# Gjerman/Orange3-Spark

Hardware: AMD Instinct MI355X
Metric: samples/sec LogisticRegression.fit on 1Bx256 synthetic at 1/2/4/8 MI355X (higher is better)
Workload: dtype bf16; 1 GPU; global_batch=1000000000, seq_len=256, features=256, parallelism=dp1, resident_rows=497795896, lineage_rows=502204104, device=cuda:0

## Files before the change

### orange3_spark_amd/models/glm.py

```python
from __future__ import annotations

import logging
import math
import os
import time
from dataclasses import dataclass, field

import numpy as np
import torch

from ..frame import column as C
from ..ops import _native as N
from ..ops import glm as G
from ..runtime.tracing import traced
from ..synthetic import LineageVectorColumn
from . import optim
from ..runtime import progress

log = logging.getLogger(__name__)

LOSS_ID = {"logistic": G.LOSS_LOGISTIC, "hinge": G.LOSS_HINGE, "squared": G.LOSS_SQUARED}


class GlmData:

    def __init__(self, comm, feat: C.Column, y: torch.Tensor, sw: torch.Tensor | None = None,
                 chunk_rows: int = 1 << 22):
        from ..frame.spill import SpilledVectorColumn
        self.comm = comm
        self.lineage = None
        self.spill = None
        if isinstance(feat, C.SparseVectorColumn):
            feat = C.VectorColumn(feat.to_dense(torch.float32), feat.size)
        if isinstance(feat, LineageVectorColumn):
            X = feat.data
            self.lineage = (feat.spec, feat.row0 + feat.resident_rows, feat.lineage_rows)
        elif isinstance(feat, SpilledVectorColumn):
            X = feat.data
            if feat.spilled_rows:
                self.spill = feat.streamer()
        else:
            X = feat.data
        self.d = int(feat.size)
        self.X = X
        self.device = X.device if X.numel() or X.is_cuda else y.device
        self.kernel = X.is_cuda and X.is_contiguous() and (
            X.dtype == torch.bfloat16 or (G.f32_rows(X) and not isinstance(feat, SpilledVectorColumn)))
        self.ld = int(X.shape[1])
        self.y = y.to(self.device, torch.float32).contiguous() if self.kernel else y.to(self.device)
        self.sw = None if sw is None else (sw.to(self.device, torch.float32).contiguous() if self.kernel else sw.to(self.device))
        self.nres = int(X.shape[0])
        self.n_local = self.nres + (self.lineage[2] if self.lineage else 0) + \
            (int(self.spill.host.shape[0]) if self.spill is not None else 0)
        self.n = int(comm.sum_scalar(self.n_local))
        self.chunk = chunk_rows
        self.ws = G.GlmWorkspace(self.device, self.ld) if self.kernel else None
        self.passes = 0
        self.overlap = None
        self.mixed = self.kernel and os.environ.get("O3S_GLM_MIXED", "1") == "1" \
            and (self.sw is None or self.sw.shape[0] == self.y.shape[0])
        self._row0 = int(feat.row0) if isinstance(feat, LineageVectorColumn) else None
        if self.spill is not None and self.kernel:
            self.mixed = True
        self._setup_workspace()
        self.ws_stream = G.GlmWorkspace(self.device, self.ld) if (self.spill is not None and self.kernel) else None

    def _res(self, t):
        return None if t is None else (t if self.spill is None else t[: self.nres])

    def _chunk_rows(self, t, off, rows):
        return None if t is None else t[self.nres + off: self.nres + off + rows]

    @property
    def mode(self) -> str:
        if self.lineage:
            return "resident+lineage" if self.nres else "lineage"
        if self.spill is not None:
            return "resident+streamed" if self.nres else "streamed"
        return "resident"

    def _setup_workspace(self):
        if self.mixed:
            cus = N.num_cus(self.device)
            tiles = -(-int(self.X.shape[0]) // 16) + -(-int(self.lineage[2] if self.lineage else 0) // 16)
            if self.spill is not None:
                tiles = max(tiles, -(-int(self.spill.chunk_rows) // 16))
            grid = max(1, min(cus * 32, -(-tiles // 4)))
            self.ws = G.GlmWorkspace(self.device, self.ld,
                                     grid=int(os.environ.get("O3S_GLM_GRID_MIX", str(grid))))
        elif self.kernel and self.lineage and self.X.shape[0] and os.environ.get("O3S_GLM_OVERLAP", "1") == "1":
            cus = N.num_cus(self.device)
            res_grid = int(os.environ.get("O3S_GLM_GRID_RES", str(cus * 8)))
            lin_grid = int(os.environ.get("O3S_GLM_GRID_LIN", str(cus)))
            self.ws = G.GlmWorkspace(self.device, self.ld, grid=res_grid)
            self.overlap = (torch.cuda.Stream(self.device), G.GlmWorkspace(self.device, self.ld, grid=lin_grid))

    def global_row0(self) -> int:
        if self._row0 is None:
            counts = self.comm.all_gather_object(int(self.n_local))
            self._row0 = int(sum(counts[: self.comm.rank]))
        return self._row0

    def require_mixed(self) -> None:
        if self.kernel and not self.mixed:
            self.mixed, self.overlap = True, None
            self._setup_workspace()

    def stats(self):
        spec, r0, nl = self.lineage if self.lineage else (None, 0, 0)
        if self.kernel:
            if not self.mixed:
                return None
            st = G.glm_stats_mixed(self.X, self._res(self.y), self._res(self.sw), nl, spec.d if spec else self.d,
                                   spec.seed if spec else 0, r0)
            if st is None:
                return None
            dpad = self.ws.dpad
        else:
            st = G.glm_stats_torch(self.X, self._res(self.y), self._res(self.sw), nl, spec.d if spec else self.d,
                                   spec.seed if spec else 0, r0).to(self.device)
            dpad = G.layout(self.ld)[0]
        if self.spill is not None:
            acc = st

            def chunk(Xc, off):
                yc, wc = self._chunk_rows(self.y, off, Xc.shape[0]), self._chunk_rows(self.sw, off, Xc.shape[0])
                if self.kernel:
                    acc.add_(G.glm_stats_mixed(Xc, yc, wc, 0, self.d, 0, 0))
                else:
                    acc.add_(G.glm_stats_torch(Xc, yc, wc, 0, self.d, 0, 0).to(self.device))
            self.spill.run(chunk)
        self.comm.all_reduce(st)
        h = st.cpu().numpy()
        d = self.d
        self.passes += 1
        return (h[:d], h[dpad:dpad + d], h[2 * dpad:2 * dpad + d], float(h[3 * dpad]), float(h[3 * dpad + 1]),
                float(h[3 * dpad + 2]))

    def moments(self):
        d = self.d
        def torch_stats(Xc, swc):
            Xd = Xc.to(torch.float64)
            w = torch.ones(Xd.shape[0], dtype=torch.float64, device=Xd.device) if swc is None \
                else swc.to(torch.float64)
            return torch.cat([w @ Xd, w @ (Xd * Xd), w.sum().reshape(1)])
        if self.kernel:
            parts = [G.glm_colstats(self.X, self._res(self.sw))] if self.X.shape[0] else []
            if self.lineage:
                spec, r0, nl = self.lineage
                parts.append(G.glm_colstats_synth(nl, self.ld, spec.d, spec.seed, r0, self.device))
            if parts:
                st = torch.stack(parts).sum(0)
            else:
                st = torch.zeros(2 * self.ld + 1, dtype=torch.float64, device=self.device)
        else:
            st = torch_stats(self.X, self._res(self.sw))
        if self.spill is not None:
            def chunk(Xc, off):
                wc = self._chunk_rows(self.sw, off, Xc.shape[0])
                st.add_(G.glm_colstats(Xc, wc) if self.kernel else torch_stats(Xc, wc).to(st.device))
            self.spill.run(chunk)
        ld = self.ld
        yw = self.y.to(torch.float64) * (1.0 if self.sw is None else self.sw.to(torch.float64))
        ystats = torch.stack([yw.sum(), (yw * self.y.to(torch.float64)).sum()]).to(st.device)
        full = torch.cat([st, ystats]).contiguous()
        self.comm.all_reduce(full)
        full = full.cpu().numpy()
        s1, s2, W = full[:ld], full[ld:2 * ld], full[2 * ld]
        ys1, ys2 = full[2 * ld + 1], full[2 * ld + 2]
        if self.lineage:
            pass
        mean = s1 / max(W, 1e-300)
        var = (s2 - W * mean * mean) / max(W - 1.0, 1e-300)
        var = np.maximum(var, 0.0)
        ymean = ys1 / max(W, 1e-300)
        yvar = max((ys2 - W * ymean * ymean) / max(W - 1.0, 1e-300), 0.0)
        return mean[:self.d], var[:self.d], W, ymean, yvar

    def pass_device(self, coef_eff: torch.Tensor, intercept: float | None, loss: int,
                    t_dev: torch.Tensor | None = None, sample: tuple | None = None) -> torch.Tensor:
        ws = self.ws
        if sample is not None and sample[1] < 1.0:
            self.require_mixed()
            ws = self.ws
        if self.mixed:
            spec, r0, nl = self.lineage if self.lineage else (None, 0, 0)
            sseed, frac = sample if sample is not None else (0, 1.0)
            g0 = self.global_row0() if frac < 1.0 else 0
            if self.nres or nl:
                G.glm_grad_mixed(self.X, self._res(self.y), self._res(self.sw), nl, spec.d if spec else self.d,
                                 spec.seed if spec else 0, r0, coef_eff, intercept, loss, ws,
                                 res_row0=g0, t_dev=t_dev, sample_seed=sseed, fraction=frac)
            else:
                ws.out.zero_()
            if self.spill is not None:
                cf = G._coef_buf(coef_eff, ws.dpad, self.device, intercept=intercept)
                wss = self.ws_stream

                def chunk(Xc, off):
                    rows = Xc.shape[0]
                    G.glm_grad_mixed(Xc, self._chunk_rows(self.y, off, rows), self._chunk_rows(self.sw, off, rows),
                                     0, self.d, 0, 0, cf, None, loss, wss, res_row0=g0 + self.nres + off,
                                     t_dev=t_dev, sample_seed=sseed, fraction=frac)
                    ws.out.add_(wss.out)
                self.spill.run(chunk)
            self.passes += 1
            return ws.out
        if self.overlap is not None:
            return self._pass_overlapped(coef_eff, intercept, loss)
        filled = False
        if self.X.shape[0]:
            G.glm_grad(self.X, self.y, self.sw, coef_eff, intercept, loss, ws)
            filled = True
        if self.lineage:
            spec, r0, nl = self.lineage
            G.glm_grad_synth(nl, self.ld, spec.d, spec.seed, r0, spec.wtrue, spec.btrue, coef_eff,
                             intercept, loss, ws, accumulate=filled)
            filled = True
        if not filled:
            ws.out.zero_()
        self.passes += 1
        return ws.out

    def _pass_overlapped(self, coef_eff, intercept, loss):
        side, ws_l = self.overlap
        ws = self.ws
        main = torch.cuda.current_stream(self.device)
        cf = G._coef_buf(coef_eff, ws.dpad, self.device, intercept=intercept)
        side.wait_stream(main)
        spec, r0, nl = self.lineage
        with torch.cuda.stream(side):
            G.glm_grad_synth(nl, self.ld, spec.d, spec.seed, r0, spec.wtrue, spec.btrue, cf, None, loss, ws_l)
        G.glm_grad(self.X, self.y, self.sw, cf, None, loss, ws)
        main.wait_stream(side)
        ws.out += ws_l.out
        self.passes += 1
        return ws.out

    def pass_torch(self, coef_eff: torch.Tensor, intercept: float, loss: int, it: int = 1,
                   sample: tuple | None = None) -> torch.Tensor:
        dpad = self.ld
        acc = torch.zeros(dpad + 3, dtype=torch.float64, device=self.device)
        c = coef_eff.to(self.device, torch.float64)[: self.ld]
        sampled = sample is not None and sample[1] < 1.0
        g0 = self.global_row0() if sampled else 0

        def block(X, base):
            n = X.shape[0]
            for a in range(0, n, self.chunk):
                b = min(n, a + self.chunk)
                Xc = X[a:b].to(self.device, torch.float64)
                yc = self.y[base + a:base + b].to(torch.float64)
                wc = None if self.sw is None else self.sw[base + a:base + b].to(torch.float64)
                if sampled:
                    keep = G.sample_mask(sample[0], it, torch.arange(g0 + base + a, g0 + base + b),
                                         sample[1]).to(self.device)
                    wc = keep.to(torch.float64) if wc is None else wc * keep
                acc.add_(G.glm_grad_torch(Xc, yc, wc, c, intercept, loss))
        block(self.X, 0)
        if self.spill is not None:
            self.spill.run(lambda Xc, off: block(Xc, self.nres + off))
        self.passes += 1
        return acc

    @traced("glm.pass")
    def loss_grad(self, coef_eff: np.ndarray, intercept: float, loss: int):
        ct = torch.from_numpy(np.ascontiguousarray(coef_eff, dtype=np.float64))
        if self.kernel:
            cf = torch.zeros(self.ws.dpad, dtype=torch.float32)
            cf[: self.d] = ct.float()
            out = self.pass_device(cf.to(self.device), intercept, loss)
            dpad = self.ws.dpad
        else:
            cf = torch.zeros(self.ld, dtype=torch.float64)
            cf[: self.d] = ct
            out = self.pass_torch(cf, intercept, loss)
            dpad = self.ld
        self.comm.all_reduce(out)
        o = out.cpu().numpy()
        return float(o[dpad + 1]), o[: self.d].copy(), float(o[dpad]), float(o[dpad + 2])


class SparseGlmData:

    kernel = False
    lineage = None

    def __init__(self, comm, feat: C.SparseVectorColumn, y: torch.Tensor, sw: torch.Tensor | None = None):
        from ..ops.sparse import SparseRows
        self.comm = comm
        self.rows = SparseRows(feat.indptr, feat.indices, feat.values, feat.size)
        self.device = self.rows.device
        self.d = int(feat.size)
        self.y = y.to(self.device)
        self.sw = None if sw is None else sw.to(self.device)
        self.n_local = self.rows.n
        self.n = int(comm.sum_scalar(self.n_local))
        self.passes = 0

    def moments(self):
        w = None if self.sw is None else self.sw.to(torch.float32)
        s1 = self.rows.colsum(w)
        s2 = self.rows.colsum(w, square=True)
        wd = torch.ones(self.n_local, dtype=torch.float64, device=self.device) if self.sw is None \
            else self.sw.to(torch.float64)
        yd = self.y.to(torch.float64)
        full = torch.cat([s1, s2, torch.stack([wd.sum(), (wd * yd).sum(), (wd * yd * yd).sum()])]).contiguous()
        self.comm.all_reduce(full)
        full = full.cpu().numpy()
        d = self.d
        s1, s2, W, ys1, ys2 = full[:d], full[d:2 * d], full[2 * d], full[2 * d + 1], full[2 * d + 2]
        mean = s1 / max(W, 1e-300)
        var = np.maximum((s2 - W * mean * mean) / max(W - 1.0, 1e-300), 0.0)
        ymean = ys1 / max(W, 1e-300)
        yvar = max((ys2 - W * ymean * ymean) / max(W - 1.0, 1e-300), 0.0)
        return mean, var, W, ymean, yvar

    sample_state = None
    _row0 = None

    def global_row0(self) -> int:
        if self._row0 is None:
            counts = self.comm.all_gather_object(int(self.n_local))
            self._row0 = int(sum(counts[: self.comm.rank]))
        return self._row0

    @traced("glm.pass")
    def loss_grad(self, coef_eff: np.ndarray, intercept: float, loss: int):
        ct = torch.from_numpy(np.ascontiguousarray(coef_eff, dtype=np.float64))
        sw = self.sw
        st = self.sample_state
        if st is not None and st[1] < 1.0:
            g0 = self.global_row0()
            keep = G.sample_mask(st[0], st[2], torch.arange(g0, g0 + self.n_local), st[1]).to(self.device)
            sw = keep.to(torch.float64) if sw is None else sw.to(torch.float64) * keep
        out = self.rows.loss_grad(ct, intercept, loss, self.y, sw)
        self.comm.all_reduce(out)
        self.passes += 1
        o = out.cpu().numpy()
        d = self.d
        return float(o[d + 1]), o[:d].copy(), float(o[d]), float(o[d + 2])


def make_glm_data(comm, feat: C.Column, y: torch.Tensor, sw: torch.Tensor | None = None):
    if isinstance(feat, C.SparseVectorColumn):
        return SparseGlmData(comm, feat, y, sw)
    return GlmData(comm, feat, y, sw)


@dataclass
class GlmResult:
    coef: np.ndarray
    intercept: float
    history: list = field(default_factory=list)
    iterations: int = 0
    converged: bool = False
    seconds: float = 0.0
    passes: int = 0
    setup_seconds: float = 0.0


class GlmObjective:

    def __init__(self, data: GlmData, loss: str, reg: float, alpha: float, fit_intercept: bool,
                 standardization: bool, std: np.ndarray):
        self.data, self.loss = data, LOSS_ID[loss]
        self.reg, self.alpha = float(reg), float(alpha)
        self.fi, self.stdz = fit_intercept, standardization
        self.std = std
        self.inv_std = np.where(std > 0, 1.0 / np.where(std > 0, std, 1.0), 0.0)
        self.W = None
        d = data.d
        self.l2 = self.reg * (1.0 - self.alpha)
        if self.stdz:
            self.pen2 = np.full(d, self.l2)
            self.pen1 = np.full(d, self.reg * self.alpha)
        else:
            self.pen2 = self.l2 * self.inv_std ** 2
            self.pen1 = self.reg * self.alpha * self.inv_std

    def split(self, x):
        d = self.data.d
        return x[:d], (x[d] if self.fi else 0.0)

    def smooth(self, x):
        bt, b = self.split(x)
        ls, g, gb, W = self.data.loss_grad(bt * self.inv_std, b, self.loss)
        self.W = W
        f = ls / W + 0.5 * float(np.sum(self.pen2 * bt * bt))
        gx = g * self.inv_std / W + self.pen2 * bt
        if self.fi:
            return f, np.concatenate([gx, [gb / W]])
        return f, gx


def _initial_intercept(loss: str, fit_intercept: bool, ymean: float, init_intercept=None) -> float:
    if not fit_intercept:
        return 0.0
    if init_intercept is not None:
        return float(init_intercept)
    if loss == "logistic" and 0 < ymean < 1:
        return math.log(ymean / (1 - ymean))
    if loss == "squared":
        return float(ymean)
    return 0.0


def _first_step_out(loss: str, b0: float, s1, syx, W: float, wy: float, wyy: float):
    if loss == "logistic":
        p = 1.0 / (1.0 + math.exp(-b0))
        sp = max(b0, 0.0) + math.log1p(math.exp(-abs(b0)))
        return p * s1 - syx, p * W - wy, sp * W - b0 * wy
    if loss == "hinge":
        if abs(b0) >= 1.0:
            return None
        return s1 - 2.0 * syx, W - 2.0 * wy, W - b0 * (2.0 * wy - W)
    return b0 * s1 - syx, b0 * W - wy, 0.5 * (b0 * b0 * W - 2.0 * b0 * wy + wyy)


def fit_sgd(data: GlmData, loss: str, reg=0.0, alpha=0.0, fit_intercept=True, standardization=True,
            max_iter=100, tol=1e-6, step_size=1.0, mini_batch_fraction=1.0, seed=0, init_intercept=None,
            ckpt=None, check_every: int = 10) -> GlmResult:
    t0 = time.time()
    frac = float(mini_batch_fraction)
    G.sample_threshold(frac)
    last = ckpt.latest() if ckpt is not None else None
    st = data.stats() if (frac >= 1.0 and last is None and max_iter > 0) else None
    if st is not None:
        s1, s2, syx, W, wy, wyy = st
        mean = s1 / max(W, 1e-300)
        var = np.maximum((s2 - W * mean * mean) / max(W - 1.0, 1e-300), 0.0)
        ymean = wy / max(W, 1e-300)
    else:
        mean, var, W, ymean, _ = data.moments()
    std = np.sqrt(var)
    b0 = float(init_intercept) if (fit_intercept and init_intercept is not None) else 0.0
    sgd = DeviceSGD(data, loss, reg, fit_intercept, step_size, standardization, std, elastic_net=alpha,
                    mini_batch_fraction=frac, seed=seed, init_intercept=b0)
    setup_s = time.time() - t0
    done = 0
    if last is not None and last[1]["x"].shape[0] == data.d + (1 if fit_intercept else 0):
        done = int(last[0])
        sgd.set_state(last[1]["x"], done)
    elif st is not None:
        first = _first_step_out(loss, b0, s1, syx, W, wy, wyy)
        if first is not None:
            sgd.apply_first_step(*first, W)
    converged = False
    while sgd.t < max_iter:
        progress.iteration(sgd.t, max_iter)
        sgd.step()
        if (tol > 0 or ckpt is not None) and sgd.t % check_every == 0:
            h = sgd.loss_hist[max(0, sgd.t - 2):sgd.t].cpu().numpy()
            if ckpt is not None and ckpt.due(sgd.t):
                ckpt.save(sgd.t, {"x": sgd.state()})
            if tol > 0 and len(h) == 2 and abs(h[0] - h[1]) / max(abs(h[1]), 1e-12) < tol:
                converged = True
                break
    if ckpt is not None:
        ckpt.clear()
    res = sgd.result()
    res.converged = converged
    res.seconds = time.time() - t0
    res.setup_seconds = setup_s
    res.passes = data.passes
    return res


def fit_glm(data: GlmData, loss: str, reg=0.0, alpha=0.0, fit_intercept=True, standardization=True,
            max_iter=100, tol=1e-6, solver="auto", step_size=1.0, mini_batch_fraction=1.0, seed=0,
            init_intercept=None, ckpt=None) -> GlmResult:
    if solver in ("sgd", "gd") and isinstance(data, GlmData):
        return fit_sgd(data, loss, reg, alpha, fit_intercept, standardization, max_iter, tol, step_size,
                       mini_batch_fraction, seed, init_intercept, ckpt)
    t0 = time.time()
    mean, var, W, ymean, yvar = data.moments()
    std = np.sqrt(var)
    obj = GlmObjective(data, loss, reg, alpha, fit_intercept, standardization, std)
    d = data.d
    x0 = np.zeros(d + (1 if fit_intercept else 0))
    if fit_intercept:
        if init_intercept is not None:
            x0[-1] = init_intercept
        elif loss == "logistic" and 0 < ymean < 1:
            x0[-1] = math.log(ymean / (1 - ymean))
        elif loss == "squared":
            x0[-1] = ymean
    done = 0
    last = ckpt.latest() if ckpt is not None else None
    if last is not None and last[1]["x"].shape == x0.shape:
        done, x0 = last[0], last[1]["x"]

    def save(it, x, f):
        if ckpt is not None and ckpt.due(done + it):
            ckpt.save(done + it, {"x": np.asarray(x)})
    left = max(max_iter - done, 0)
    if solver in ("sgd", "gd"):
        res = _sgd(obj, x0, left, step_size, mini_batch_fraction, seed, tol)
    elif reg * alpha > 0:
        l1 = np.concatenate([obj.pen1, [0.0]]) if fit_intercept else obj.pen1
        r = optim.owlqn(obj.smooth, x0, l1, max_iter=left, tol=tol, callback=save)
        res = GlmResult(r.x, 0.0, r.history, done + r.iterations, r.converged)
    else:
        f32 = isinstance(data, GlmData) and data.kernel and data.X.dtype == torch.float32
        r = optim.lbfgs(obj.smooth, x0, max_iter=left, tol=tol, callback=save, f_noise=2.0 ** -24 if f32 else 0.0)
        res = GlmResult(r.x, 0.0, r.history, done + r.iterations, r.converged)
    if ckpt is not None:
        ckpt.clear()
    bt, b = obj.split(res.coef)
    res.coef = bt * obj.inv_std
    res.intercept = float(b)
    res.seconds = time.time() - t0
    res.passes = data.passes
    return res


def _sgd(obj: GlmObjective, x0, max_iter, step, frac, seed, tol) -> GlmResult:
    x = x0.copy()
    hist = []
    for t in range(1, max_iter + 1):
        progress.iteration(t - 1, max_iter)
        obj.data.sample_state = (int(seed), float(frac), t)
        f, g = obj.smooth(x)
        hist.append(f)
        x = x - (step / math.sqrt(t)) * g
        if len(hist) > 1 and abs(hist[-2] - hist[-1]) / max(abs(hist[-1]), 1e-12) < tol * 1e-3:
            break
    obj.data.sample_state = None
    return GlmResult(x, 0.0, hist, len(hist), False)


class DeviceSGD:

    def __init__(self, data: GlmData, loss: str = "logistic", reg: float = 0.0, fit_intercept=True,
                 step_size: float = 1.0, standardization: bool = True, std: np.ndarray | None = None,
                 elastic_net: float = 0.0, mini_batch_fraction: float = 1.0, seed: int = 0,
                 init_intercept: float = 0.0):
        self.data, self.loss = data, LOSS_ID[loss]
        dev = data.device
        dpad = data.ws.dpad if data.kernel else data.ld
        self.dpad = dpad
        inv = np.ones(data.d) if std is None else np.where(std > 0, 1.0 / np.where(std > 0, std, 1.0), 0.0)
        self.inv_std = torch.zeros(dpad, dtype=torch.float64, device=dev)
        self.inv_std[: data.d] = torch.from_numpy(inv).to(dev)
        a = float(elastic_net)
        l2, l1 = float(reg) * (1.0 - a), float(reg) * a
        self.l2 = l2 if standardization else 0.0
        self.l2v = (l2 * self.inv_std ** 2) if not standardization else None
        self.l1 = l1 if standardization else 0.0
        self.l1v = (l1 * self.inv_std) if (not standardization and l1 > 0) else None
        self.bt = torch.zeros(dpad, dtype=torch.float64, device=dev)
        self.b = torch.full((1,), float(init_intercept) if fit_intercept else 0.0, dtype=torch.float64, device=dev)
        self.coef_eff = torch.zeros(dpad + 1, dtype=torch.float32, device=dev)
        self.coef_eff[dpad] = float(self.b[0])
        self.fi = fit_intercept
        self.step_size = float(step_size)
        self.fraction = float(mini_batch_fraction)
        G.sample_threshold(self.fraction)
        self.sample = (int(seed), self.fraction) if self.fraction < 1.0 else None
        self.t = 0
        self.loss_hist = torch.zeros(1024, dtype=torch.float64, device=dev)
        self.t_dev = torch.zeros(1, dtype=torch.int64, device=dev)
        self._graphs = None
        self._graph_failed = False
        self._eager_steps = 0
        self._first_buf = None
        self.passes = 0

    def state(self) -> np.ndarray:
        x = self.bt[: self.data.d].cpu().numpy()
        return np.concatenate([x, self.b.cpu().numpy()]) if self.fi else x

    def set_state(self, x: np.ndarray, t: int) -> None:
        d = self.data.d
        self.bt.zero_()
        self.bt[:d] = torch.from_numpy(np.asarray(x[:d], dtype=np.float64)).to(self.bt.device)
        if self.fi:
            self.b.fill_(float(x[d]))
        self.coef_eff[: self.dpad].copy_((self.bt * self.inv_std).to(torch.float32))
        self.coef_eff[self.dpad:].copy_(self.b.to(torch.float32))
        self.t = int(t)
        self.t_dev.fill_(int(t))
        self._ensure_hist()
        self._graphs = None

    def _ensure_hist(self):
        if self.t > self.loss_hist.shape[0]:
            n = self.loss_hist.shape[0]
            while n < self.t:
                n *= 2
            self.loss_hist = torch.cat([self.loss_hist, torch.zeros(n - self.loss_hist.shape[0],
                                                                     dtype=torch.float64, device=self.loss_hist.device)])
            self._graphs = None

    def apply_first_step(self, grad: np.ndarray, sum_r: float, loss_sum: float, W: float) -> None:
        out = torch.zeros(self.dpad + 3, dtype=torch.float64)
        out[: self.data.d] = torch.from_numpy(np.asarray(grad, dtype=np.float64))
        out[self.dpad:] = torch.tensor([sum_r, loss_sum, W], dtype=torch.float64)
        self._first_buf = out.to(self.bt.device)
        self.t += 1
        self._ensure_hist()
        self._update(self._first_buf)

    @traced("sgd.step")
    def step(self):
        self.t += 1
        self._ensure_hist()
        d = self.data
        self.passes += 1
        if d.kernel and self._graphs is not None:
            gp, gu = self._graphs
            gp.replay()
            if gu is not None:
                d.comm.all_reduce(self.data.ws.out)
                gu.replay()
            d.passes += 1
            return
        out = self._pass()
        d.comm.all_reduce(out)
        self._update(out)
        if d.kernel:
            self._eager_steps += 1
            self._maybe_capture()

    def _pass(self):
        if self.data.kernel:
            return self.data.pass_device(self.coef_eff, None, self.loss, t_dev=self.t_dev, sample=self.sample)
        return self.data.pass_torch(self.coef_eff[: self.dpad], float(self.b.item()), self.loss, it=self.t,
                                    sample=self.sample)

    def _update(self, out: torch.Tensor):
        if self.data.kernel:
            N.check(N.kernels().o3s_glm_sgd_update_dev(
                out.data_ptr(), self.dpad, self.bt.data_ptr(), self.b.data_ptr(), self.inv_std.data_ptr(),
                N.ptr(self.l2v), self.l2, N.ptr(self.l1v), self.l1, self.step_size, int(self.fi),
                self.coef_eff.data_ptr(), self.loss_hist.data_ptr(), int(self.loss_hist.shape[0]),
                self.t_dev.data_ptr(), torch.cuda.current_stream(self.data.device).cuda_stream), "glm_sgd_update")
            return
        eta = self.step_size / math.sqrt(self.t)
        W = out[self.dpad + 2]
        invW = torch.where(W > 0, 1.0 / W, torch.zeros_like(W))
        g = out[: self.dpad] * self.inv_std * invW
        g = g + (self.l2v if self.l2v is not None else self.l2) * self.bt
        v = self.bt - eta * g
        if self.l1v is not None or self.l1 > 0:
            sh = eta * (self.l1v if self.l1v is not None else self.l1)
            v = torch.sign(v) * torch.clamp(v.abs() - sh, min=0.0)
        self.bt.copy_(v)
        if self.fi:
            self.b -= eta * out[self.dpad] * invW
        self.coef_eff[: self.dpad].copy_((self.bt * self.inv_std).to(torch.float32))
        self.coef_eff[self.dpad:].copy_(self.b.to(torch.float32))
        self.loss_hist[self.t - 1:self.t].copy_(out[self.dpad + 1:self.dpad + 2] * invW)
        self.t_dev.fill_(self.t)

    GRAPH_MAX_BYTES = int(os.environ.get("O3S_SGD_GRAPH_MAX_BYTES", str(256 << 20)))

    def _maybe_capture(self):
        from ..runtime import faults
        mode = os.environ.get("O3S_SGD_GRAPH", "1")
        if self._graphs is not None or self._graph_failed or mode == "0" or self._eager_steps < 2:
            return
        if faults.launch_blocking():
            return
        d = self.data
        if d.spill is not None:
            return
        if mode != "force" and d.n_local * d.ld * d.X.element_size() > self.GRAPH_MAX_BYTES:
            return
        if d.comm.world_size > 1 and mode != "all":
            return
        try:
            if d.comm.world_size == 1:
                g = torch.cuda.CUDAGraph()
                with torch.cuda.graph(g):
                    out = self._pass()
                    self._update(out)
                self._graphs = (g, None)
            else:
                gp, gu = torch.cuda.CUDAGraph(), torch.cuda.CUDAGraph()
                with torch.cuda.graph(gp):
                    out = self._pass()
                with torch.cuda.graph(gu):
                    self._update(out)
                self._graphs = (gp, gu)
            d.passes -= 1
        except Exception as e:
            log.warning("SGD step graph capture failed (%s); continuing eagerly", e)
            self._graph_failed = True
            self._graphs = None

    def result(self) -> GlmResult:
        coef = (self.bt * self.inv_std)[: self.data.d].cpu().numpy()
        hist = [float(x) for x in self.loss_hist[: self.t].cpu()]
        return GlmResult(coef, float(self.b.item()), hist, self.t, False, 0.0, self.data.passes)


def _class_weights(yl: torch.Tensor, w: torch.Tensor | None, K: int) -> torch.Tensor:
    if w is None:
        return torch.bincount(yl, minlength=K)[:K].to(torch.float64)
    w64 = w.to(torch.float64)
    if K <= 64:
        return torch.stack([torch.where(yl == k, w64, 0.0).sum() for k in range(K)])
    return torch.zeros(K, dtype=torch.float64, device=yl.device).index_add_(0, yl, w64)


def fit_multinomial(comm, X: torch.Tensor, y: torch.Tensor, sw, num_classes: int, reg=0.0, alpha=0.0,
                    fit_intercept=True, standardization=True, max_iter=100, tol=1e-6, chunk=1 << 21):
    dev = X.device
    n, D = X.shape
    K = num_classes
    Xf_dtype = torch.float32 if X.is_cuda else torch.float64
    yl = y.to(dev).long()
    w = torch.ones(n, dtype=Xf_dtype, device=dev) if sw is None else sw.to(dev, Xf_dtype)
    fused = G.softmax_kernel_ok(X, K) and os.environ.get("O3S_SOFTMAX_KERNEL", "1") == "1"
    f32_kernel = fused and X.dtype == torch.float32
    if X.is_cuda and X.dtype in (torch.bfloat16, torch.float32) and X.stride(1) == 1 and X.stride(0) % 8 == 0:
        base = torch.as_strided(X, (n, X.stride(0)), (X.stride(0), 1))
        cs = G.glm_colstats(base, None if sw is None else w.float().contiguous())
        ldp = X.stride(0)
        s1, s2 = cs[:D], cs[ldp:ldp + D]
    else:
        s1 = torch.zeros(D, dtype=torch.float64, device=dev)
        s2 = torch.zeros(D, dtype=torch.float64, device=dev)
        for a in range(0, n, chunk):
            Xc = X[a:a + chunk].to(torch.float64)
            wc = w[a:a + chunk].to(torch.float64)
            s1 += wc @ Xc
            s2 += wc @ (Xc * Xc)
    cnt = _class_weights(yl, None if sw is None else w, K)
    st = torch.cat([s1, s2, cnt])
    comm.all_reduce(st)
    st = st.cpu().numpy()
    W = st[2 * D:].sum()
    mean = st[:D] / W
    var = np.maximum((st[D:2 * D] - W * mean ** 2) / max(W - 1, 1e-300), 0)
    std = np.sqrt(var)
    inv = np.where(std > 0, 1.0 / np.where(std > 0, std, 1.0), 0.0)
    inv_t = torch.from_numpy(inv).to(dev, Xf_dtype)
    l2 = reg * (1 - alpha)
    pen2 = np.full(D, l2) if standardization else l2 * inv ** 2
    pen1 = np.full(D, reg * alpha) if standardization else reg * alpha * inv
    prior = st[2 * D:] / W

    y32 = yl.to(torch.int32).contiguous() if fused else None
    sw32 = None if (sw is None or not fused) else w.float().contiguous()

    def fg(x):
        Bt = x[: D * K].reshape(K, D)
        b = x[D * K:] if fit_intercept else np.zeros(K)
        if fused:
            Gk, gbk, lk = G.softmax_pass(X, y32, sw32, torch.from_numpy(Bt * inv[None, :]).to(dev, torch.float32),
                                         torch.from_numpy(b).to(dev, torch.float32))
            buf = torch.cat([Gk.T.reshape(-1), gbk, lk.reshape(1)])
            return _mn_finish(buf, Bt)
        Weff = torch.from_numpy(Bt.T * inv[:, None]).to(dev, Xf_dtype)
        bt = torch.from_numpy(b).to(dev, Xf_dtype)
        G_ = torch.zeros((D, K), dtype=torch.float64, device=dev)
        gb = torch.zeros(K, dtype=torch.float64, device=dev)
        loss = torch.zeros(1, dtype=torch.float64, device=dev)
        for a in range(0, n, chunk):
            Xc = X[a:a + chunk].to(Xf_dtype)
            M = Xc @ Weff + bt
            lse = torch.logsumexp(M, dim=1)
            yc = yl[a:a + chunk]
            wc = w[a:a + chunk]
            loss += (wc * (lse - M.gather(1, yc[:, None]).squeeze(1))).to(torch.float64).sum()
            P = torch.softmax(M, dim=1)
            P[torch.arange(P.shape[0], device=dev), yc] -= 1.0
            R = P * wc[:, None]
            G_ += (Xc.T @ R).to(torch.float64)
            gb += R.sum(0).to(torch.float64)
        return _mn_finish(torch.cat([G_.reshape(-1), gb, loss]), Bt)

    def _mn_finish(buf, Bt):
        comm.all_reduce(buf)
        buf = buf.cpu().numpy()
        Gm = buf[: D * K].reshape(D, K).T * inv[None, :] / W
        gbm = buf[D * K:D * K + K] / W
        if f32_kernel:
            Gm = Gm - Gm.mean(0, keepdims=True)
            gbm = gbm - gbm.mean()
        f = buf[-1] / W + 0.5 * float(np.sum(pen2[None, :] * Bt * Bt))
        Gm = Gm + pen2[None, :] * Bt
        g = Gm.reshape(-1)
        if fit_intercept:
            g = np.concatenate([g, gbm])
        return f, g

    f_noise = 2.0 ** -24 if f32_kernel else 0.0
    x0 = np.zeros(D * K + (K if fit_intercept else 0))
    if fit_intercept:
        lp = np.log(np.maximum(prior, 1e-300))
        x0[D * K:] = lp - lp.mean()
    if reg * alpha > 0:
        l1 = np.concatenate([np.tile(pen1, K), np.zeros(K if fit_intercept else 0)])
        r = optim.owlqn(fg, x0, l1, max_iter=max_iter, tol=tol, f_noise=f_noise)
    else:
        r = optim.lbfgs(fg, x0, max_iter=max_iter, tol=tol, f_noise=f_noise)
    Bt = r.x[: D * K].reshape(K, D)
    B = Bt * inv[None, :]
    b = r.x[D * K:] if fit_intercept else np.zeros(K)
    if fit_intercept:
        b = b - b.mean()
    if reg == 0:
        B = B - B.mean(0, keepdims=True)
    return B, b, r
```

### orange3_spark_amd/ops/_native.py

```python
from __future__ import annotations

import ctypes as C
import os
import threading
from pathlib import Path

import torch

from ..runtime.faults import O3SError
from . import build as _build

_LOCK = threading.Lock()
_LIB = None
_HOST = None

c_i64, c_i32, c_u32, c_f32, c_f64 = C.c_int64, C.c_int, C.c_uint32, C.c_float, C.c_double
c_vp = C.c_void_p

_SIGS: dict[str, list] = {
    "o3s_glm_layout": [c_i64, C.POINTER(c_i32), C.POINTER(c_i32)],
    "o3s_glm_grad": [c_i32, c_i32, c_vp, c_i64, c_i64, c_vp, c_vp, c_vp, c_u32, c_i64,
                     c_vp, c_f32, c_vp, c_i32, c_vp, c_i32, c_vp],
    "o3s_glm_grad_mixed": [c_i32, c_vp, c_i64, c_i64, c_vp, c_vp, c_vp, c_u32, c_i64, c_i64,
                           c_vp, c_i32, c_vp, c_i32, c_i64, c_vp, c_u32, c_u32, c_i32, c_i32, c_i32, c_vp],
    "o3s_glm_stats_mixed": [c_vp, c_i64, c_i64, c_vp, c_vp, c_u32, c_i64, c_i64, c_vp, c_i32, c_vp, c_i32, c_i32,
                            c_vp],
    "o3s_glm_grad_f32": [c_i32, c_vp, c_i64, c_i64, c_vp, c_vp, c_vp, c_i64, c_vp, c_i32, c_vp, c_i32, c_i64, c_vp,
                         c_u32, c_u32, c_i32, c_vp],
    "o3s_glm_stats_f32": [c_vp, c_i64, c_i64, c_vp, c_vp, c_i64, c_vp, c_i32, c_vp, c_vp],
    "o3s_glm_margin_f32": [c_vp, c_i64, c_i64, c_vp, c_f32, c_vp, c_i32, c_vp],
    "o3s_glm_colstats_f32": [c_vp, c_i64, c_i64, c_vp, c_vp, c_i32, c_vp, c_vp],
    "o3s_bin_features": [c_vp, c_i64, c_i64, c_i32, c_vp, c_i32, c_vp, c_vp],
    "o3s_u8_transpose": [c_vp, c_i64, c_i32, c_vp, c_vp],
    "o3s_slab_range_sum": [c_vp, c_i32, c_i64, c_vp, c_vp, c_i32, c_vp, c_vp],
    "o3s_tree_leaf_apply": [c_vp, c_vp, c_vp, c_vp, c_i32, c_vp, c_vp],
    "o3s_ftf": [c_vp, c_i64, c_i64, c_i32, c_i64, c_vp, c_vp, c_vp],
    "o3s_als_gram": [c_vp, c_vp, c_vp, c_vp, c_vp, c_i32, c_vp, c_vp, c_i64, c_i64, c_vp, c_vp, c_vp],
    "o3s_csr_glm": [c_i32, c_vp, c_vp, c_vp, c_i64, c_vp, c_f32, c_vp, c_vp, c_vp, c_vp, c_i32, c_vp],
    "o3s_csc_colsum": [c_vp, c_vp, c_i64, c_vp, c_i64, c_vp, c_vp, c_vp, c_i32, c_vp, c_vp, c_vp],
    "o3s_csc_piece": [],
    "o3s_tokenize": [c_i32, c_vp, c_vp, c_i64, c_vp, c_vp, c_vp, c_vp, c_vp, c_vp],
    "o3s_murmur3_spans": [c_vp, c_vp, c_vp, c_i64, c_u32, c_i64, c_vp, c_vp],
    "o3s_tree_partition": [c_vp, c_i64, c_i64, c_vp, c_vp, c_vp, c_vp, c_vp, c_vp, c_vp, c_vp, c_vp, c_vp, c_i32, c_i32,
                           c_vp, c_vp, c_vp, c_vp, c_vp],
    "o3s_glm_sgd_update": [c_vp, c_i32, c_vp, c_vp, c_vp, c_vp, c_f64, c_f64, c_i32, c_vp, c_vp, c_vp],
    "o3s_glm_sgd_update_dev": [c_vp, c_i32, c_vp, c_vp, c_vp, c_vp, c_f64, c_vp, c_f64, c_f64, c_i32, c_vp, c_vp,
                               c_i64, c_vp, c_vp],
    "o3s_synth_glm": [c_vp, c_i64, c_i64, c_vp, c_u32, c_i64, c_vp, c_f32, c_i32, c_vp],
    "o3s_glm_margin": [c_vp, c_i64, c_i64, c_vp, c_f32, c_vp, c_i32, c_vp],
    "o3s_glm_colstats": [c_i32, c_vp, c_i64, c_i64, c_vp, c_u32, c_i64, c_vp, c_i32, c_vp, c_vp],
    "o3s_bin_sums": [c_vp, c_i32, c_i64, c_i64, c_i32, c_vp, c_i64, c_vp, c_i32, c_vp, c_i32, c_vp, c_vp],
    "o3s_glm_softmax": [c_vp, c_i64, c_i64, c_i32, c_vp, c_vp, c_vp, c_vp, c_i32, c_vp, c_i32, c_vp, c_vp],
    "o3s_glm_softmax_f32": [c_vp, c_i64, c_i64, c_i32, c_vp, c_vp, c_vp, c_vp, c_i32, c_vp, c_i32, c_vp, c_vp],
    "o3s_kmeans_assign": [c_vp, c_i64, c_i64, c_i32, c_vp, c_vp, c_vp, c_i32, c_vp, c_vp, c_vp, c_vp],
    "o3s_kmeans_screen2": [c_vp, c_i64, c_i64, c_i32, c_vp, c_vp, c_vp, c_i32, c_i32, C.c_float, C.c_float,
                           C.c_float, C.c_float, C.c_float, c_vp, c_vp, c_vp, c_vp, c_i32, c_i32, c_vp, c_vp, c_vp,
                           c_vp, c_vp],
    "o3s_kmeans_presplit": [c_vp, c_i64, c_i64, c_i32, C.c_float, c_vp, c_vp, c_vp],
    "o3s_kmeans_moments": [c_vp, c_i64, c_i64, c_i32, c_vp, c_i32, c_vp, c_vp],
    "o3s_kmeans_cost": [c_vp, c_i64, c_i64, c_i32, c_vp, c_vp, c_i32, c_i32, c_vp, c_vp],
    "o3s_kmeans_bounds": [c_vp, c_vp, c_i64, c_vp, C.c_float, c_i32, c_vp, c_vp, c_vp, c_i32, c_vp],
    "o3s_kmeans_update_ws": [c_i32, c_i32, c_i32, C.POINTER(c_i64), C.POINTER(c_i64), C.POINTER(c_i32)],
    "o3s_kmeans_screen_lds": [c_i32, c_i32, C.POINTER(c_i32)],
    "o3s_murmur3_terms": [c_vp, c_vp, c_i64, c_u32, c_i64, c_vp, c_vp, c_vp],
    "o3s_als_init": [c_i64, c_i64, c_i32, c_u32, c_i32, c_vp, c_vp],
    "o3s_als_cg": [c_i32, c_i64, c_i32, c_vp, c_vp, c_vp, c_vp, c_vp, c_vp, c_vp, c_vp, c_vp],
    "o3s_als_pass": [c_i32, c_vp, c_vp, c_vp, c_i64, c_vp, c_i32, c_vp, c_vp, c_vp, c_vp, c_vp],
    "o3s_tree_hist_lds": [c_i32, c_i32, c_i32, c_i32],
    "o3s_hash_uniform": [c_vp, c_i64, c_i64, c_u32, c_u32, c_i32, c_f64, c_vp, c_vp, c_vp],
    "o3s_tree_final_level": [c_vp, c_i64, c_i64, c_vp, c_vp, c_vp, c_vp, c_vp, c_vp, c_vp, c_vp, c_vp, c_vp, c_vp,
                             c_i32, c_vp],
    "o3s_forest_weights": [c_vp, c_i64, c_vp, c_i32, c_vp, c_i32, c_f32, c_vp, c_vp, c_vp],
    "o3s_tree_sibling": [c_vp, c_vp, c_vp, c_i64, c_i32, c_i32, c_i32, c_vp, c_vp],
    "o3s_tree_part_dest": [c_vp, c_vp, c_vp, c_vp, c_vp, c_i32, c_vp, c_vp, c_vp, c_vp],
    "o3s_gbt_grad_loss": [c_vp, c_vp, c_vp, c_vp, c_i64, c_i32, c_vp, c_vp, c_i32, c_vp],
    "o3s_gbt_leaf_pass": [c_vp, c_i64, c_i32, c_vp, c_i32, c_vp, c_i32, c_vp, c_vp, c_vp, c_vp, c_vp, c_i32, c_i32,
                          c_vp, c_vp, c_vp, c_i32, c_vp],
    "o3s_tree_split": [c_vp, c_i32, c_i32, c_i32, c_i32, c_i32, c_vp, c_vp, c_f64, c_f64, c_f64, c_vp, c_vp, c_vp],
    "o3s_tree_hist": [c_vp, c_i64, c_i32, c_i32, c_i32, c_i32, c_vp, c_vp, c_vp, c_vp, c_vp, c_i32, c_vp, c_i32,
                      c_vp],
    "o3s_eval_grid": [c_i64],
    "o3s_regression_stats": [c_vp, c_i32, c_vp, c_i32, c_vp, c_i32, c_i64, c_vp, c_vp, c_vp],
    "o3s_confusion": [c_vp, c_i32, c_vp, c_i32, c_vp, c_i32, c_i64, c_i32, c_vp, c_vp, c_vp],
    "o3s_score_hist": [c_vp, c_i32, c_i64, c_vp, c_i32, c_vp, c_i32, c_i64, c_f64, c_f64, c_i32, c_vp, c_vp],
    "o3s_als_wood_kn": [c_i32, c_i32, c_vp, c_vp, c_vp, c_vp, c_vp, c_vp, c_vp, c_vp, c_i64, c_vp, c_vp],
    "o3s_als_wood_timed": [c_i32, c_vp, c_vp, c_vp, c_vp, c_vp, c_vp, c_vp, c_vp, c_i64, c_vp, c_vp, c_vp],
    "o3s_hashing_tf": [c_i32, c_vp, c_vp, c_vp, c_vp, c_vp, c_i64, c_u32, c_i64, c_vp, c_vp, c_vp, c_vp, c_i32,
                       c_vp, c_vp, c_vp],
    "o3s_als_dense_wave_dbg": [c_i32, c_i32, c_vp, c_vp, c_vp, c_vp, c_vp, c_vp, c_i64, c_vp, c_i32, c_vp, c_vp],
    "o3s_bin_features2": [c_vp, c_i32, c_i64, c_i64, c_i32, c_vp, c_i32, c_vp, c_vp, c_i64, c_vp],
    "o3s_kmeanspp": [c_vp, c_vp, c_vp, c_i32, c_i32, c_i32, c_i32, c_vp, c_vp, c_vp, c_vp, c_vp, c_vp, c_vp, c_vp],
    "o3s_als_dense_wave_timed": [c_vp, c_vp, c_vp, c_vp, c_vp, c_vp, c_i64, c_vp, c_i32, c_vp, c_vp],
    "o3s_als_dense_wave": [c_i32, c_i32, c_vp, c_vp, c_vp, c_vp, c_vp, c_vp, c_i64, c_vp, c_i32, c_vp],
    "o3s_als_dense_wave_gd": [c_i32, c_vp, c_vp, c_vp, c_vp, c_vp, c_vp, c_i64, c_vp, c_i32, c_vp],
    "o3s_als_exact_max_small": [],
    "o3s_als_rotate": [c_i32, c_vp, c_vp, c_i64, c_vp, c_i32, c_vp],
    "o3s_als_rotate_to": [c_i32, c_vp, c_vp, c_i64, c_vp, c_vp, c_i32, c_vp],
    "o3s_assemble": [c_vp, c_i32, c_vp, c_i32, c_i32, c_i64, c_vp, c_i32, c_vp, c_vp, c_i32, c_vp],
    "o3s_assemble_src_size": [],
    "o3s_assemble_cols": [c_vp, c_i32, c_i32, c_i32, c_i64, c_vp, c_i32, c_vp, c_vp, c_i32, c_vp],
    "o3s_kmeans_update": [c_vp, c_i64, c_i64, c_i32, c_vp, c_i32, c_vp, c_vp, c_i32, c_vp, c_vp, c_vp],
    "o3s_gather_probe": [c_vp, c_i32, c_vp, c_i64, c_i32, c_vp, c_vp],
    "o3s_gram_layout": [c_i32, C.POINTER(c_i32), C.POINTER(c_i32), C.POINTER(c_i32)],
    "o3s_gram": [c_vp, c_i32, c_i64, c_i64, c_i32, c_vp, c_vp, c_vp, c_vp, c_i32, c_vp, c_vp],
    "o3s_gmm_layout": [c_i32, c_i32, C.POINTER(c_i32), C.POINTER(c_i32), C.POINTER(c_i64), C.POINTER(c_i32)],
    "o3s_gmm_estep": [c_vp, c_i32, c_i64, c_i64, c_i32, c_i32, c_vp, c_vp, c_vp, c_vp, c_vp, c_vp, c_vp, c_i32, c_vp],
}


class NativeError(O3SError):
    """A native kernel launch was rejected (bad shape/arguments) or failed."""


def lib_path() -> Path:
    alt = os.environ.get("O3S_KERNEL_LIB")
    return Path(alt) if alt else _build.KERNEL_LIB


def _load():
    global _LIB
    path = lib_path()
    if not path.exists() and os.environ.get("O3S_AUTOBUILD", "1") == "1":
        _build.build()
    if not path.exists():
        raise NativeError(f"kernel library missing: {path} (run python -m orange3_spark_amd.ops.build)")
    lib = C.CDLL(str(path), mode=C.RTLD_GLOBAL)
    for name, argt in _SIGS.items():
        fn = getattr(lib, name, None)
        if fn is None:
            continue
        fn.argtypes = argt
        fn.restype = C.c_int
    _LIB = lib
    return lib


def kernels():
    if _LIB is not None:
        return _LIB
    with _LOCK:
        if _LIB is not None:
            return _LIB
        return _load()


_HOST_SIGS: dict[str, list] = {
    "o3s_host_murmur3": [c_vp, c_vp, c_i64, c_u32, c_i64, c_vp, c_vp],
    "o3s_host_tokenize": [c_vp, c_vp, c_i64, c_vp, c_vp, c_vp, c_i64, c_vp],
    "o3s_host_pav": [c_vp, c_vp, c_vp, c_vp, c_i64, c_vp, c_vp, c_vp, c_vp],
    "o3s_host_ascii_lengths": [c_vp, c_i64, c_vp, c_vp],
    "o3s_host_ascii_pack": [c_vp, c_i64, c_vp, c_vp, c_i32],
}
_HOST_RET = {"o3s_host_tokenize": C.c_int64, "o3s_host_pav": C.c_int64, "o3s_host_ascii_lengths": C.c_int64}


def host():
    global _HOST
    if _HOST is not None:
        return _HOST
    with _LOCK:
        if _HOST is None:
            path = _build.HOST_LIB
            if not path.exists():
                _build.build()
            lib = C.CDLL(str(path))
            for name, argt in _HOST_SIGS.items():
                fn = getattr(lib, name)
                fn.argtypes = argt
                fn.restype = _HOST_RET.get(name)
            _HOST = lib
    return _HOST


PRELOAD_TAGS = ("glm", "trees", "kmeans", "als", "als_dense", "als_exact", "assemble", "binsum", "eval",
                "sampling", "sparse", "text", "probe", "gram", "gmm")


def preload(tags=PRELOAD_TAGS) -> dict:
    import time
    lib = kernels()
    out = {}
    for tag in tags:
        fn = getattr(lib, f"o3s_preload_{tag}", None)
        if fn is None:
            continue
        fn.restype = C.c_int
        t = time.perf_counter()
        rc = fn()
        if rc != 0:
            raise NativeError(f"o3s_preload_{tag}: hipError {rc}")
        out[tag] = round(time.perf_counter() - t, 5)
    return out


def available() -> bool:
    try:
        kernels()
        return True
    except Exception:
        return False


def ptr(t: torch.Tensor | None) -> int | None:
    if t is None:
        return None
    return t.data_ptr()


def upload(arr, dev) -> torch.Tensor:
    import numpy as np
    t = torch.from_numpy(np.ascontiguousarray(arr))
    dev = torch.device(dev)
    if dev.type != "cuda":
        return t.to(dev)
    p = torch.empty(t.shape, dtype=t.dtype, pin_memory=True)
    p.copy_(t)
    return p.to(dev, non_blocking=True)


def upload_many(dev, *arrays) -> list:
    import numpy as np
    arrs = [np.ascontiguousarray(a) for a in arrays]
    offs, total = [], 0
    for a in arrs:
        offs.append(total)
        total += (a.nbytes + 7) // 8 * 8
    buf = np.zeros(max(total, 8), dtype=np.uint8)
    for a, o in zip(arrs, offs):
        buf[o:o + a.nbytes] = a.view(np.uint8).reshape(-1)
    d = upload(buf, dev)
    out = []
    for a, o in zip(arrs, offs):
        dt = torch.from_numpy(np.zeros(0, dtype=a.dtype)).dtype
        out.append(d[o:o + a.nbytes].view(dt).view(a.shape))
    return out


def stream_of(t: torch.Tensor) -> int:
    return torch.cuda.current_stream(t.device).cuda_stream


def check(rc: int, what: str) -> None:
    from ..runtime import faults
    faults.INJECTOR.hit("kernel")
    if rc != 0:
        raise NativeError(f"{what} failed with code {rc}")
    if faults.launch_blocking() and torch.cuda.is_available():
        try:
            torch.cuda.synchronize()
        except Exception as e:
            raise faults.DeviceError(what, e) from e


def num_cus(device: torch.device) -> int:
    try:
        return torch.cuda.get_device_properties(device).multi_processor_count
    except Exception:
        return 256


def grid_for(device: torch.device, work_items: int, per_block: int, blocks_per_cu: int = 8) -> int:
    need = max(1, (work_items + per_block - 1) // per_block)
    return int(max(1, min(need, num_cus(device) * blocks_per_cu)))
```

### orange3_spark_amd/ops/csrc/glm.hip

```cpp
#include <type_traits>

#include "common.h"

using namespace o3s;

namespace {

enum { LOSS_LOGISTIC = 0, LOSS_HINGE = 1, LOSS_SQUARED = 2 };

constexpr int kBlock = 256;
constexpr int kWavesPerBlock = kBlock / kWave;

__host__ __device__ __forceinline__ uint32_t umad24(uint32_t a, uint32_t c, uint32_t add) {
#if defined(__HIP_DEVICE_COMPILE__)
  return __umul24(a, c) + add;
#else
  return (a & 0xFFFFFFu) * c + add;
#endif
}
__host__ __device__ __forceinline__ uint32_t mix24(uint32_t h) {
  h ^= h >> 16;
  h = umad24(h, 0xED5AD4u, h);
  h ^= h >> 15;
  return umad24(h, 0x2C1B3Cu, h);
}
__device__ __forceinline__ uint32_t feat_key(uint32_t seed, int64_t row) {
  const uint32_t lo = (uint32_t)(row & 0xffffffffll);
  const uint32_t hi = (uint32_t)((uint64_t)row >> 32);
  return mix24(mix24(lo + seed * 0x9E3779B1u) ^ umad24(hi, 0x7FEB35u, 0x165667u));
}
__device__ __forceinline__ uint32_t synth_word(uint32_t fk, int i) {
  return mix24(umad24((uint32_t)i, 0x9E3779u, fk));
}
__device__ __forceinline__ float synth_byte(uint32_t h, int q) {
  return (float)((h >> (8 * q)) & 0xffu);
}
constexpr float kSynthScale = 1.0f / 128.0f, kSynthShift = -255.0f / 256.0f;
__device__ __forceinline__ short8 synth_chunk(uint32_t fk, int ch) {
  short8 v;
#pragma unroll
  for (int p = 0; p < 2; ++p) {
    const uint32_t h = synth_word(fk, 2 * ch + p);
#pragma unroll
    for (int q = 0; q < 4; ++q)
      v[4 * p + q] = (short)f32_to_bf16(fmaf(synth_byte(h, q), kSynthScale, kSynthShift));
  }
  return v;
}
__device__ __forceinline__ float synth_label(uint32_t rk, float margin_true) {
  const float u = (float)(fmix32(rk ^ 0xA511E9B3u) >> 8) * (1.0f / 16777216.0f);
  return u < sigmoidf(margin_true) ? 1.0f : 0.0f;
}

constexpr int ilog2(int x) { return x <= 1 ? 0 : 1 + ilog2(x / 2); }

template <int LPR, int U>
struct RowReduce {
  static constexpr int LL = ilog2(LPR), LU = ilog2(U);
  static constexpr int H = LL < LU ? LL : LU;
  static constexpr int NF = U >> H;
  __device__ static __forceinline__ int base(int c) {
    int b = 0;
#pragma unroll
    for (int s = 0; s < H; ++s) b += ((c >> (LL - 1 - s)) & 1) * (U >> (s + 1));
    return b;
  }
  __host__ __device__ static constexpr int owner(int u) {
    int c = 0;
    for (int s = 0; s < H; ++s) c += (((u - u % NF) >> (LU - 1 - s)) & 1) << (LL - 1 - s);
    return c;
  }
  __device__ static __forceinline__ bool representative(int c) {
    return (c & ((1 << (LL - H)) - 1)) == 0;
  }
  __device__ static __forceinline__ void run(float (&v)[U], int c) {
    int n = U;
#pragma unroll
    for (int s = 0; s < LL; ++s) {
      const int off = LPR >> (s + 1);
      if (s < H) {
        const bool up = (c & off) != 0;
        n >>= 1;
#pragma unroll
        for (int j = 0; j < U / 2; ++j) {
          if (j < n) {
            const float keep = up ? v[j + n] : v[j];
            const float send = up ? v[j] : v[j + n];
            v[j] = keep + __shfl_xor(send, off, kWave);
          }
        }
      } else {
#pragma unroll
        for (int j = 0; j < NF; ++j) v[j] += __shfl_xor(v[j], off, kWave);
      }
    }
  }
};

struct MemoryRows {
  static constexpr bool kLineage = false;
  __device__ static __forceinline__ float dot(float d, float) { return d; }
  __device__ static __forceinline__ float resid(float r, float&) { return r; }
};
struct RowsBf16 : MemoryRows {
  using elem = uint16_t;
  using chunk = short8;
  __device__ static __forceinline__ void load(const elem* __restrict__ X, int64_t ld, int64_t rowc, int chc,
                                              chunk& v) {
    v = __builtin_nontemporal_load(reinterpret_cast<const short8*>(X + rowc * ld + 8 * chc));
  }
  __device__ static __forceinline__ void mask(chunk& v, bool keep) {
    v = keep ? v : short8{0, 0, 0, 0, 0, 0, 0, 0};
  }
  __device__ static __forceinline__ void load_if(const elem* __restrict__ X, int64_t ld, int64_t row, int ch,
                                                 bool ok, chunk& v) {
    v = ok ? *reinterpret_cast<const short8*>(X + row * ld + 8 * ch) : short8{0, 0, 0, 0, 0, 0, 0, 0};
  }
  __device__ static __forceinline__ void unpack(const chunk& v, float (&x)[8]) { unpack8(v, x); }
  __device__ static __forceinline__ void pin(chunk& v) { asm volatile("" : "+v"(v)); }
};
struct RowsF32 : MemoryRows {
  using elem = float;
  struct chunk { float4_ lo, hi; };
  __device__ static __forceinline__ void load(const elem* __restrict__ X, int64_t ld, int64_t rowc, int chc,
                                              chunk& v) {
    const float4_* p = reinterpret_cast<const float4_*>(X + rowc * ld + 8 * chc);
    v.lo = __builtin_nontemporal_load(p);
    v.hi = __builtin_nontemporal_load(p + 1);
  }
  __device__ static __forceinline__ void mask(chunk& v, bool keep) {
    v.lo = keep ? v.lo : float4_{0.f, 0.f, 0.f, 0.f};
    v.hi = keep ? v.hi : float4_{0.f, 0.f, 0.f, 0.f};
  }
  __device__ static __forceinline__ void load_if(const elem* __restrict__ X, int64_t ld, int64_t row, int ch,
                                                 bool ok, chunk& v) {
    const float4_* p = reinterpret_cast<const float4_*>(X + row * ld + 8 * ch);
    v.lo = ok ? p[0] : float4_{0.f, 0.f, 0.f, 0.f};
    v.hi = ok ? p[1] : float4_{0.f, 0.f, 0.f, 0.f};
  }
  __device__ static __forceinline__ void unpack(const chunk& v, float (&x)[8]) {
#pragma unroll
    for (int j = 0; j < 4; ++j) {
      x[j] = v.lo[j];
      x[4 + j] = v.hi[j];
    }
  }
  __device__ static __forceinline__ void pin(chunk&) {}
};
struct RowsLineage {
  using elem = uint16_t;
  static constexpr bool kLineage = true;
  struct chunk { float b[8]; };
  __device__ static __forceinline__ void load(uint32_t fk, int ch, chunk& v) {
    decode(synth_word(fk, 2 * ch), synth_word(fk, 2 * ch + 1), v);
  }
  __device__ static __forceinline__ void decode(uint32_t h0, uint32_t h1, chunk& v) {
#pragma unroll
    for (int j = 0; j < 4; ++j) {
      v.b[j] = synth_byte(h0, j);
      v.b[4 + j] = synth_byte(h1, j);
    }
  }
  __device__ static __forceinline__ void unpack(const chunk& v, float (&x)[8]) {
#pragma unroll
    for (int j = 0; j < 8; ++j) x[j] = v.b[j];
  }
  __device__ static __forceinline__ void values(const chunk& v, float (&x)[8]) {
#pragma unroll
    for (int j = 0; j < 8; ++j) x[j] = fmaf(v.b[j], kSynthScale, kSynthShift);
  }
  __device__ static __forceinline__ void pin(chunk& v) {
#pragma unroll
    for (int j = 0; j < 8; ++j) asm volatile("" : "+v"(v.b[j]));
  }
  __device__ static __forceinline__ float dot(float d, float wshift) { return fmaf(d, kSynthScale, wshift); }
  __device__ static __forceinline__ float resid(float r, float& rs) {
    rs += r;
    return r * kSynthScale;
  }
};

template <int LOSS>
__device__ __forceinline__ void loss_terms(float m, float yv, float wv, float& r, float& l) {
  if (LOSS == LOSS_LOGISTIC) {
    const float e = __expf(-fabsf(m));
    const float inv = __builtin_amdgcn_rcpf(1.0f + e);
    const float p = m >= 0.f ? inv : e * inv;
    r = (p - yv) * wv;
    l = wv * (fmaxf(m, 0.f) + __logf(1.0f + e) - yv * m);
  } else if (LOSS == LOSS_HINGE) {
    const float s = 2.f * yv - 1.f;
    const float mg = 1.f - s * m;
    r = mg > 0.f ? -s * wv : 0.f;
    l = mg > 0.f ? wv * mg : 0.f;
  } else {
    const float e = m - yv;
    r = e * wv;
    l = 0.5f * wv * e * e;
  }
}

template <int LPR, int CPL>
__device__ __forceinline__ void load_coef(const float* __restrict__ coef, int64_t ld, int c, float (&w)[CPL][8]) {
#pragma unroll
  for (int k = 0; k < CPL; ++k)
#pragma unroll
    for (int j = 0; j < 8; ++j) {
      const int col = 8 * (c + k * LPR) + j;
      w[k][j] = col < ld ? coef[col] : 0.f;
    }
}
template <class T, int A, int B>
__device__ __forceinline__ void zero(T (&a)[A][B]) {
#pragma unroll
  for (int k = 0; k < A; ++k)
#pragma unroll
    for (int j = 0; j < B; ++j) a[k][j] = T{};
}

template <int LPR, int CPL>
__device__ __forceinline__ void grad_epilogue(float (&acc)[CPL][8], float acc_r, float acc_loss, float acc_w,
                                              float* __restrict__ partial, int pstride, int pacc, int lane, int wid,
                                              int c) {
  constexpr int DP = LPR * CPL * 8;
#pragma unroll
  for (int k = 0; k < CPL; ++k)
#pragma unroll
    for (int j = 0; j < 8; ++j) {
      float v = acc[k][j];
#pragma unroll
      for (int off = LPR; off < kWave; off <<= 1) v += __shfl_xor(v, off, kWave);
      acc[k][j] = v;
    }
  acc_r = wave_sum(acc_r);
  acc_loss = wave_sum(acc_loss);
  acc_w = wave_sum(acc_w);
  __shared__ float red[kWavesPerBlock][DP + 4];
  if (lane < LPR) {
#pragma unroll
    for (int k = 0; k < CPL; ++k)
#pragma unroll
      for (int j = 0; j < 8; ++j) red[wid][8 * (c + k * LPR) + j] = acc[k][j];
  }
  if (lane == 0) {
    red[wid][DP] = acc_r;
    red[wid][DP + 1] = acc_loss;
    red[wid][DP + 2] = acc_w;
  }
  __syncthreads();
  for (int i = threadIdx.x; i < DP + 3; i += kBlock) {
    float s = 0.f;
#pragma unroll
    for (int q = 0; q < kWavesPerBlock; ++q) s += red[q][i];
    float* const pp = partial + (int64_t)blockIdx.x * pstride + i;
    *pp = pacc ? *pp + s : s;
  }
}

template <int LPR, int CPL, int UNROLL, int LOSS, int SRC>
__global__ __launch_bounds__(kBlock) void glm_grad_kernel(
    const uint16_t* __restrict__ X, int64_t ld, int64_t n, const float* __restrict__ y,
    const float* __restrict__ sw, const float* __restrict__ coef, const float* __restrict__ bptr,
    uint32_t seed, int64_t row0, const float* __restrict__ wtrue, float btrue,
    float* __restrict__ partial, int pstride) {
  constexpr int G = kWave / LPR;
  constexpr int RT = G * UNROLL;
  using RR = RowReduce<LPR, UNROLL>;
  constexpr int NF = RR::NF;
  const int lane = threadIdx.x & (kWave - 1);
  const int wid = threadIdx.x / kWave;
  const int g = lane / LPR, c = lane % LPR;
  const int nch = (int)(ld / 8);
  const int ubase = RR::base(c);
  const bool rep = RR::representative(c);
  const float intercept = *bptr;

  float w[CPL][8], wt[CPL][8], acc[CPL][8];
  float wshift = 0.f, wtshift = 0.f, rs = 0.f;
#pragma unroll
  for (int k = 0; k < CPL; ++k)
#pragma unroll
    for (int j = 0; j < 8; ++j) {
      const int col = 8 * (c + k * LPR) + j;
      const float wv = col < ld ? coef[col] : 0.f;
      const float wtv = (SRC == 1 && col < ld) ? wtrue[col] : 0.f;
      w[k][j] = SRC == 1 ? wv * kSynthScale : wv;
      wt[k][j] = wtv * kSynthScale;
      wshift += wv;
      wtshift += wtv;
      acc[k][j] = 0.f;
    }
  wshift *= kSynthShift;
  wtshift *= kSynthShift;
  float acc_r = 0.f, acc_loss = 0.f, acc_w = 0.f;

  const int64_t ntiles = (n + RT - 1) / RT;
  const int64_t gw = (int64_t)blockIdx.x * kWavesPerBlock + wid;
  const int64_t nw = (int64_t)gridDim.x * kWavesPerBlock;
  for (int64_t t = gw; t < ntiles; t += nw) {
    const int64_t base = t * RT;
    short8 xv[UNROLL][CPL];
    float xf[UNROLL][CPL][8];
#pragma unroll
    for (int u = 0; u < UNROLL; ++u) {
      const int64_t row = base + u * G + g;
      const bool ok = row < n;
      const int64_t rowc = ok ? row : n - 1;
      const uint32_t rk = SRC == 1 ? feat_key(seed, row0 + row) : 0u;
#pragma unroll
      for (int k = 0; k < CPL; ++k) {
        const int ch = c + k * LPR;
        if (SRC == 0) {
          const bool okc = ok && ch < nch;
          const int chc = ch < nch ? ch : nch - 1;
          short8 v = __builtin_nontemporal_load(reinterpret_cast<const short8*>(X + rowc * ld + 8 * chc));
          xv[u][k] = okc ? v : short8{0, 0, 0, 0, 0, 0, 0, 0};
        } else {
          const uint32_t h0 = synth_word(rk, 2 * ch), h1 = synth_word(rk, 2 * ch + 1);
#pragma unroll
          for (int j = 0; j < 4; ++j) {
            xf[u][k][j] = synth_byte(h0, j);
            xf[u][k][4 + j] = synth_byte(h1, j);
          }
        }
      }
    }
    float yy[NF], ww[NF];
#pragma unroll
    for (int j = 0; j < NF; ++j) {
      const int64_t row = base + (ubase + j) * G + g;
      const bool ok = row < n;
      const int64_t rowc = ok ? row : n - 1;
      if (SRC == 0) {
        const float yv = y[rowc];
        const float wv = sw ? sw[rowc] : 1.f;
        yy[j] = ok ? yv : 0.f;
        ww[j] = ok ? wv : 0.f;
      } else {
        ww[j] = ok ? 1.f : 0.f;
      }
    }
    float dot[UNROLL], dtrue[UNROLL];
#pragma unroll
    for (int u = 0; u < UNROLL; ++u) {
      float d = SRC == 1 ? wshift : 0.f, dt = wtshift;
#pragma unroll
      for (int k = 0; k < CPL; ++k) {
        float x[8];
        if (SRC == 0) {
          unpack8(xv[u][k], x);
        } else {
#pragma unroll
          for (int j = 0; j < 8; ++j) x[j] = xf[u][k][j];
        }
#pragma unroll
        for (int j = 0; j < 8; ++j) {
          d = fmaf(x[j], w[k][j], d);
          if (SRC == 1) dt = fmaf(x[j], wt[k][j], dt);
        }
      }
      dot[u] = d;
      dtrue[u] = dt;
    }
    RR::run(dot, c);
    if (SRC == 1) {
      RR::run(dtrue, c);
#pragma unroll
      for (int j = 0; j < NF; ++j) {
        const int64_t row = base + (ubase + j) * G + g;
        yy[j] = synth_label(row_key(seed, row0 + row), dtrue[j] + btrue);
      }
    }
    float res[NF];
#pragma unroll
    for (int j = 0; j < NF; ++j) {
      float r, l;
      loss_terms<LOSS>(dot[j] + intercept, yy[j], ww[j], r, l);
      res[j] = r;
      if (rep) { acc_r += r; acc_loss += l; acc_w += ww[j]; }
    }
#pragma unroll
    for (int u = 0; u < UNROLL; ++u)
#pragma unroll
      for (int k = 0; k < CPL; ++k) {
        if (SRC == 0) asm volatile("" : "+v"(xv[u][k]));
        else {
#pragma unroll
          for (int j = 0; j < 8; ++j) asm volatile("" : "+v"(xf[u][k][j]));
        }
      }
#pragma unroll
    for (int u = 0; u < UNROLL; ++u) {
      float r = __shfl(res[u % NF], g * LPR + RR::owner(u), kWave);
      if (SRC == 1) { rs += r; r *= kSynthScale; }
#pragma unroll
      for (int k = 0; k < CPL; ++k) {
        float x[8];
        if (SRC == 0) {
          unpack8(xv[u][k], x);
        } else {
#pragma unroll
          for (int j = 0; j < 8; ++j) x[j] = xf[u][k][j];
        }
#pragma unroll
        for (int j = 0; j < 8; ++j) acc[k][j] = fmaf(r, x[j], acc[k][j]);
      }
    }
  }

  if (SRC == 1) {
#pragma unroll
    for (int k = 0; k < CPL; ++k)
#pragma unroll
      for (int j = 0; j < 8; ++j) acc[k][j] = fmaf(rs, kSynthShift, acc[k][j]);
  }
  grad_epilogue<LPR, CPL>(acc, acc_r, acc_loss, acc_w, partial, pstride, 0, lane, wid, c);
}


template <int CTRL>
__device__ __forceinline__ float dpp_f(float v) {
  return __builtin_bit_cast(float, __builtin_amdgcn_update_dpp(0, __builtin_bit_cast(int, v), CTRL, 0xF, 0xF,
                                                               false));
}
constexpr int kDppXor1 = 0xB1, kDppXor2 = 0x4E, kDppHalfMirror = 0x141;
__device__ __forceinline__ void row_reduce_8x2(float (&v)[2], int c) {
  v[0] += dpp_f<kDppXor1>(v[0]);
  v[1] += dpp_f<kDppXor1>(v[1]);
  v[0] += dpp_f<kDppXor2>(v[0]);
  v[1] += dpp_f<kDppXor2>(v[1]);
  const bool up = (c & 4) != 0;
  const float keep = up ? v[1] : v[0], send = up ? v[0] : v[1];
  v[0] = keep + dpp_f<kDppHalfMirror>(send);
}

struct RowSampler {
  uint32_t key, thr;
  int64_t grow0;
  __device__ __forceinline__ bool on() const { return thr < (1u << 24); }
  __device__ __forceinline__ bool keep(int64_t row) const { return (row_key(key, grow0 + row) >> 8) < thr; }
};
__host__ __device__ __forceinline__ uint32_t sample_key(uint32_t seed, uint32_t iter) {
  return fmix32(seed ^ fmix32(iter * 0x9E3779B1u + 0x7F4A7C15u));
}

typedef __bf16 sm_bf16x2 __attribute__((ext_vector_type(2)));
__device__ __forceinline__ uint32_t pk_bf16(float a, float b) {
  float2_ v;
  v[0] = a;
  v[1] = b;
  return __builtin_bit_cast(uint32_t, __builtin_convertvector(v, sm_bf16x2));
}

constexpr int kStgTileBytes = 8 * 1024, kStgLabelBytes = kWave * 4;
constexpr int kStgWaveBytes = kStgTileBytes + 2 * kStgLabelBytes;
constexpr int kStgFragBytes = 8 * 1024;
constexpr int kStgLd = 256;
constexpr unsigned kAuxNt = 2;
struct TileStage {
  static constexpr int LPR = 8, CPL = 4, UNROLL = 2, G = kWave / LPR, kTileOps = 1 + UNROLL * CPL;
  unsigned char* slot;
  uint32_t sbase;
  uint32_t fbase;
  const unsigned char* xs;
  const float* yrs;
  const float* yls;
  int64_t tstep;
  uint32_t r_ahead, l_ahead;
  bool lab_younger;

  __device__ static __forceinline__ uint32_t fresh(int v) {
    asm volatile("" : "+v"(v));
    return (uint32_t)v;
  }
  __device__ static __forceinline__ uint32_t label_off(uint32_t g, uint32_t c) { return ((c >> 2) * G + g) * 4; }

  __device__ __forceinline__ void issue_tile(int lane) {
    const uint32_t ln = fresh(lane);
    __builtin_amdgcn_global_load_lds(reinterpret_cast<const unsigned char*>(yrs) + (ln & 15) * 4,
                                     slot + kStgTileBytes, 4, 0, 0);
    const uint32_t xoff = (ln >> 3) * (kStgLd * 2) + ((ln ^ (ln >> 4)) & 7) * 16;
#pragma unroll
    for (int u = 0; u < UNROLL; ++u)
#pragma unroll
      for (int k = 0; k < CPL; ++k)
        __builtin_amdgcn_global_load_lds(xs + (u * G * kStgLd * 2 + k * LPR * 16) + xoff, slot + (u * CPL + k) * 1024,
                                         16, 0, kAuxNt);
    xs += tstep * (kStgLd * 2);
    yrs += tstep;
    --r_ahead;
    lab_younger = false;
  }
  __device__ __forceinline__ void issue_label(int g, int c) {
    __builtin_amdgcn_global_load_lds(reinterpret_cast<const unsigned char*>(yls) + label_off(fresh(g), fresh(c)),
                                     slot + kStgTileBytes + kStgLabelBytes, 4, 0, 0);
    yls += tstep;
    --l_ahead;
    lab_younger = true;
  }
  __device__ __forceinline__ void take_tile(int lane, short8 (&xb)[8], short8 (&xv)[UNROLL][CPL], float& yv,
                                            short8 (&fa)[3]) {
    if (lab_younger) asm volatile("s_waitcnt vmcnt(1)" ::: "memory");
    else asm volatile("s_waitcnt vmcnt(0)" ::: "memory");
    const uint32_t ln = fresh(lane);
    const uint32_t b0 = sbase + ((ln & 8) << 9) + ((ln >> 4) << 10) + ((ln & 7) << 7) + (((ln >> 1) & 3) << 4);
    asm volatile(
        "ds_read_b128 %17, %26\n\t"
        "ds_read_b128 %18, %26 offset:1024\n\t"
        "ds_read_b128 %19, %26 offset:2048\n\t"
        "ds_read_b128 %0, %20\n\t"
        "ds_read_b128 %1, %21\n\t"
        "ds_read_b128 %2, %22\n\t"
        "ds_read_b128 %3, %23\n\t"
        "ds_read_b128 %4, %20 offset:64\n\t"
        "ds_read_b128 %5, %21 offset:64\n\t"
        "ds_read_b128 %6, %22 offset:64\n\t"
        "ds_read_b128 %7, %23 offset:64\n\t"
        "ds_read_b128 %8, %24\n\t"
        "ds_read_b128 %9, %24 offset:1024\n\t"
        "ds_read_b128 %10, %24 offset:2048\n\t"
        "ds_read_b128 %11, %24 offset:3072\n\t"
        "ds_read_b128 %12, %24 offset:4096\n\t"
        "ds_read_b128 %13, %24 offset:5120\n\t"
        "ds_read_b128 %14, %24 offset:6144\n\t"
        "ds_read_b128 %15, %24 offset:7168\n\t"
        "ds_read_b32 %16, %25 offset:8192\n\t"
        "s_waitcnt lgkmcnt(0)"
        : "=&v"(xb[0]), "=&v"(xb[1]), "=&v"(xb[2]), "=&v"(xb[3]), "=&v"(xb[4]), "=&v"(xb[5]), "=&v"(xb[6]),
          "=&v"(xb[7]), "=&v"(xv[0][0]), "=&v"(xv[0][1]), "=&v"(xv[0][2]), "=&v"(xv[0][3]), "=&v"(xv[1][0]),
          "=&v"(xv[1][1]), "=&v"(xv[1][2]), "=&v"(xv[1][3]), "=&v"(yv), "=&v"(fa[0]), "=&v"(fa[1]), "=&v"(fa[2])
        : "v"(b0), "v"(b0 ^ 16u), "v"(b0 ^ 32u), "v"(b0 ^ 48u), "v"(sbase + ((ln ^ (ln >> 4)) << 4)),
          "v"(sbase + ln * 4), "v"(fbase + ln * 16)
        : "memory");
    if (r_ahead > 0) issue_tile(lane);
    __builtin_amdgcn_sched_barrier(0);
  }
  __device__ __forceinline__ float4_ dot(int lane, const short8 (&xb)[8], short8 (&fa)[3]) {
    float4_ d;
    asm volatile(
        "v_mfma_f32_16x16x32_bf16 %0, %1, %5, 0\n\t"
        "s_nop 7\n\t"
        "ds_read_b128 %1, %4 offset:3072\n\t"
        "v_mfma_f32_16x16x32_bf16 %0, %2, %6, %0\n\t"
        "s_nop 7\n\t"
        "ds_read_b128 %2, %4 offset:4096\n\t"
        "v_mfma_f32_16x16x32_bf16 %0, %3, %7, %0\n\t"
        "s_nop 7\n\t"
        "ds_read_b128 %3, %4 offset:5120\n\t"
        "s_waitcnt lgkmcnt(2)\n\t"
        "v_mfma_f32_16x16x32_bf16 %0, %1, %8, %0\n\t"
        "s_nop 7\n\t"
        "ds_read_b128 %1, %4 offset:6144\n\t"
        "s_waitcnt lgkmcnt(2)\n\t"
        "v_mfma_f32_16x16x32_bf16 %0, %2, %9, %0\n\t"
        "s_nop 7\n\t"
        "ds_read_b128 %2, %4 offset:7168\n\t"
        "s_waitcnt lgkmcnt(2)\n\t"
        "v_mfma_f32_16x16x32_bf16 %0, %3, %10, %0\n\t"
        "s_nop 7\n\t"
        "s_waitcnt lgkmcnt(1)\n\t"
        "v_mfma_f32_16x16x32_bf16 %0, %1, %11, %0\n\t"
        "s_nop 7\n\t"
        "s_waitcnt lgkmcnt(0)\n\t"
        "v_mfma_f32_16x16x32_bf16 %0, %2, %12, %0\n\t"
        "s_nop 7\n\t"
        "s_nop 3"
        : "=&v"(d), "+v"(fa[0]), "+v"(fa[1]), "+v"(fa[2])
        : "v"(fbase + fresh(lane) * 16), "v"(xb[0]), "v"(xb[1]), "v"(xb[2]), "v"(xb[3]), "v"(xb[4]), "v"(xb[5]),
          "v"(xb[6]), "v"(xb[7])
        : "memory");
    return d;
  }
  __device__ __forceinline__ void take_label(int g, int c, float& yv) {
    if (lab_younger) asm volatile("s_waitcnt vmcnt(0)" ::: "memory");
    else asm volatile("s_waitcnt vmcnt(%0)" ::"n"(kTileOps) : "memory");
    const uint32_t a4 = sbase + (fresh(g) * LPR + fresh(c)) * 4;
    asm volatile("ds_read_b32 %0, %1 offset:8448\n\ts_waitcnt lgkmcnt(0)" : "=v"(yv) : "v"(a4) : "memory");
    lab_younger = false;
    if (l_ahead > 0) issue_label(g, c);
  }
};
static_assert(kStgTileBytes == 8192 && kStgLabelBytes == 256, "the asm offsets in TileStage");

template <class SRC, int LPR, int CPL, int UNROLL, int LOSS, bool SMP, bool FULL = false, bool STAGED = false>
__device__ __forceinline__ void grad_tile(
    int64_t base, int64_t n, const typename SRC::elem* __restrict__ X, int64_t ld, int nch,
    const float* __restrict__ y, const float* __restrict__ sw, uint32_t seed, int64_t row0, const float (&w)[CPL][8],
    float wshift, float intercept, int g, int c, const RowSampler smp, float (&acc)[CPL][8], float& rs, float& acc_r,
    float& acc_loss, float& acc_w, TileStage* stg = nullptr) {
  constexpr int G = kWave / LPR;
  using RR = RowReduce<LPR, UNROLL>;
  constexpr int NF = RR::NF;
  static_assert(!STAGED || (SRC::kLineage && FULL && NF == 1 && LPR == TileStage::LPR && CPL == TileStage::CPL &&
                            UNROLL == TileStage::UNROLL),
                "the staged slot holds the labels of one (8, 4, 2) lineage tile");
  const int ubase = RR::base(c);
  const bool rep = RR::representative(c);
  typename SRC::chunk xv[UNROLL][CPL];
#pragma unroll
  for (int u = 0; u < UNROLL; ++u) {
    const int64_t row = base + u * G + (STAGED ? (int)TileStage::fresh(g) : g);
    const bool ok = row < n;
    const int64_t rowc = ok ? row : n - 1;
    const uint32_t fk = SRC::kLineage ? feat_key(seed, row0 + row) : 0u;
#pragma unroll
    for (int k = 0; k < CPL; ++k) {
      const int ch = c + k * LPR;
      if constexpr (SRC::kLineage) {
        SRC::decode(synth_word(fk, 2 * ch), synth_word(fk, 2 * ch + 1), xv[u][k]);
      } else if constexpr (FULL) {
        SRC::load(X, ld, row, ch, xv[u][k]);
      } else {
        const int chc = ch < nch ? ch : nch - 1;
        SRC::load(X, ld, rowc, chc, xv[u][k]);
        SRC::mask(xv[u][k], ok && ch < nch);
      }
    }
  }
  float yy[NF], ww[NF];
#pragma unroll
  for (int j = 0; j < NF; ++j) {
    const int64_t row = base + (ubase + j) * G + g;
    const bool ok = row < n;
    const int64_t rowc = ok ? row : n - 1;
    if constexpr (STAGED) {
      ww[j] = 1.f;
    } else if constexpr (FULL) {
      yy[j] = y[row];
      ww[j] = sw ? sw[row] : 1.f;
    } else {
      const float yv = y[rowc];
      const float wv = sw ? sw[rowc] : 1.f;
      yy[j] = ok ? yv : 0.f;
      ww[j] = ok ? wv : 0.f;
    }
    if constexpr (SMP && !STAGED) {
      if (!smp.keep(row)) ww[j] = 0.f;
    }
  }
  float dot[UNROLL];
#pragma unroll
  for (int u = 0; u < UNROLL; ++u) {
    float2_ d2 = {0.f, 0.f};
#pragma unroll
    for (int k = 0; k < CPL; ++k) {
      float x[8];
      SRC::unpack(xv[u][k], x);
#pragma unroll
      for (int j = 0; j < 8; j += 2) {
        const float2_ xx = {x[j], x[j + 1]}, ww2 = {w[k][j], w[k][j + 1]};
        d2 = __builtin_elementwise_fma(xx, ww2, d2);
      }
    }
    dot[u] = SRC::dot(d2.x + d2.y, wshift);
  }
  constexpr bool kDpp = LPR == 8 && UNROLL == 2;
  if constexpr (kDpp) row_reduce_8x2(dot, c);
  else RR::run(dot, c);
  if constexpr (STAGED && SRC::kLineage) stg->take_label(g, c, yy[0]);
  if constexpr (STAGED && SMP) {
    if (!smp.keep(base + (int64_t)TileStage::fresh(ubase * G + g))) ww[0] = 0.f;
  }
  float res[NF];
#pragma unroll
  for (int j = 0; j < NF; ++j) {
    float r, l;
    loss_terms<LOSS>(dot[j] + intercept, yy[j], ww[j], r, l);
    res[j] = r;
    if (rep) { acc_r += r; acc_loss += l; acc_w += ww[j]; }
  }
#pragma unroll
  for (int u = 0; u < UNROLL; ++u)
#pragma unroll
    for (int k = 0; k < CPL; ++k) SRC::pin(xv[u][k]);
  float other = 0.f;
  if constexpr (kDpp) other = dpp_f<kDppHalfMirror>(res[0]);
#pragma unroll
  for (int u = 0; u < UNROLL; ++u) {
    float r;
    if constexpr (kDpp) r = ((c & 4) != 0) == (u == 0) ? other : res[0];
    else r = __shfl(res[u % NF], g * LPR + RR::owner(u), kWave);
    r = SRC::resid(r, rs);
#pragma unroll
    for (int k = 0; k < CPL; ++k) {
      float x[8];
      SRC::unpack(xv[u][k], x);
#pragma unroll
      for (int j = 0; j < 8; ++j) acc[k][j] = fmaf(r, x[j], acc[k][j]);
    }
  }
}

template <int LOSS, bool SMP>
__device__ __forceinline__ void staged_resident_tile(int64_t base, float intercept, int lane, const RowSampler smp,
                                                     float (&acc)[TileStage::CPL][8], float& acc_r, float& acc_loss,
                                                     float& acc_w, TileStage* stg) {
  constexpr int CPL = TileStage::CPL, UNROLL = TileStage::UNROLL;
  short8 xb[8], xv[UNROLL][CPL];
  float yv;
  short8 fa[3];
  stg->take_tile(lane, xb, xv, yv, fa);
  const float4_ d = stg->dot(lane, xb, fa);
  float wv = 1.f;
  if constexpr (SMP) {
    if (!smp.keep(base + (int64_t)(TileStage::fresh(lane) & 15u))) wv = 0.f;
  }
  float r, l;
  loss_terms<LOSS>(((d[2] + d[1]) + d[0]) + intercept, yv, wv, r, l);
  if (lane < 16) { acc_r += r; acc_loss += l; acc_w += wv; }
#pragma unroll
  for (int u = 0; u < UNROLL; ++u)
#pragma unroll
    for (int k = 0; k < CPL; ++k) RowsBf16::pin(xv[u][k]);
  const int src = (int)(TileStage::fresh(lane) >> 3) * 4;
  const float rr[UNROLL] = {
      __builtin_bit_cast(float, __builtin_amdgcn_ds_bpermute(src, __builtin_bit_cast(int, r))),
      __builtin_bit_cast(float, __builtin_amdgcn_ds_bpermute(src + 32, __builtin_bit_cast(int, r)))};
#pragma unroll
  for (int u = 0; u < UNROLL; ++u)
#pragma unroll
    for (int k = 0; k < CPL; ++k) {
      float x[8];
      unpack8(xv[u][k], x);
#pragma unroll
      for (int j = 0; j < 8; ++j) acc[k][j] = fmaf(rr[u], x[j], acc[k][j]);
    }
}

template <int LPR, int CPL, int UNROLL, int LOSS, int MW, bool SMP, bool FULL = false>
__global__ __launch_bounds__(kBlock, MW) void glm_grad_mixed_kernel(
    const uint16_t* __restrict__ X, int64_t ld, int64_t n_res, const float* __restrict__ y,
    const float* __restrict__ sw, const float* __restrict__ y_lin, const float* __restrict__ sw_lin,
    const float* __restrict__ coef, const float* __restrict__ bptr, uint32_t seed, int64_t row0, int64_t n_lin,
    float* __restrict__ partial, int pstride, int64_t res_row0, const int64_t* __restrict__ t_dev, uint32_t sseed,
    uint32_t sthr, int pacc) {
  constexpr int G = kWave / LPR;
  constexpr int RT = G * UNROLL;
  const int lane = threadIdx.x & (kWave - 1);
  const int wid = threadIdx.x / kWave;
  const int g = lane / LPR, c = lane % LPR;
  const int nch = (int)(ld / 8);
  const float intercept = *bptr;
  const uint32_t skey = SMP ? sample_key(sseed, (uint32_t)((t_dev ? t_dev[0] : 0) + 1)) : 0u;
  const RowSampler smp_res{skey, sthr, res_row0}, smp_lin{skey, sthr, row0};

  float w[CPL][8], acc[CPL][8];
  float wshift = 0.f;
#pragma unroll
  for (int k = 0; k < CPL; ++k)
#pragma unroll
    for (int j = 0; j < 8; ++j) {
      const int col = 8 * (c + k * LPR) + j;
      w[k][j] = col < ld ? coef[col] : 0.f;
      wshift += w[k][j];
      acc[k][j] = 0.f;
    }
  wshift *= kSynthShift;
  float rs = 0.f;
  float acc_r = 0.f, acc_loss = 0.f, acc_w = 0.f;

  const int64_t Tr = (n_res + RT - 1) / RT, Tl = (n_lin + RT - 1) / RT, S = Tr + Tl;
  const int64_t gw = (int64_t)blockIdx.x * kWavesPerBlock + wid;
  const int64_t nw = (int64_t)gridDim.x * kWavesPerBlock;
  if (gw < S) {
    int64_t L = gw * Tl / S, rem = gw * Tl - L * S;
    const int64_t q0 = nw * Tl / S, r0 = nw * Tl - q0 * S;
    for (int64_t s = gw; s < S; s += nw) {
      if (rem + Tl >= S)
        grad_tile<RowsLineage, LPR, CPL, UNROLL, LOSS, SMP, FULL>(L * RT, n_lin, X, ld, nch, y_lin, sw_lin, seed, row0, w,
                                                                  wshift, intercept, g, c, smp_lin, acc, rs, acc_r, acc_loss,
                                                                  acc_w);
      else
        grad_tile<RowsBf16, LPR, CPL, UNROLL, LOSS, SMP, FULL>((s - L) * RT, n_res, X, ld, nch, y, sw, seed, row0, w, wshift,
                                                               intercept, g, c, smp_res, acc, rs, acc_r, acc_loss, acc_w);
      rem += r0;
      L += q0;
      if (rem >= S) { rem -= S; ++L; }
    }
  }
#pragma unroll
  for (int k = 0; k < CPL; ++k)
#pragma unroll
    for (int j = 0; j < 8; ++j) acc[k][j] = fmaf(rs, kSynthShift, acc[k][j]);
  grad_epilogue<LPR, CPL>(acc, acc_r, acc_loss, acc_w, partial, pstride, pacc, lane, wid, c);
}

template <int LOSS, bool SMP>
__global__ __launch_bounds__(kBlock, 3) void glm_grad_staged_kernel(
    const uint16_t* __restrict__ X, int64_t n_res, const float* __restrict__ y, const float* __restrict__ y_lin,
    const float* __restrict__ coef, const float* __restrict__ bptr, uint32_t seed, int64_t row0, int64_t n_lin,
    float* __restrict__ partial, int pstride, int64_t res_row0, const int64_t* __restrict__ t_dev, uint32_t sseed,
    uint32_t sthr, int pacc) {
  constexpr int LPR = TileStage::LPR, CPL = TileStage::CPL, UNROLL = TileStage::UNROLL, G = TileStage::G;
  constexpr int RT = G * UNROLL;
  constexpr int64_t ld = kStgLd;
  __shared__ __attribute__((aligned(256))) unsigned char slots[kWavesPerBlock * kStgWaveBytes];
  __shared__ __attribute__((aligned(256))) unsigned char frags[kStgFragBytes];
  static_assert(kStgWaveBytes % 256 == 0, "TileStage: a slot starts on a bank row");
  const int lane = threadIdx.x & (kWave - 1);
  const int wid = __builtin_amdgcn_readfirstlane(threadIdx.x / kWave);
  const int g = lane / LPR, c = lane % LPR;
  const float intercept = *bptr;
  const uint32_t skey = SMP ? sample_key(sseed, (uint32_t)((t_dev ? t_dev[0] : 0) + 1)) : 0u;
  const RowSampler smp_res{skey, sthr, res_row0}, smp_lin{skey, sthr, row0};

  float w[CPL][8], acc[CPL][8];
  float wshift = 0.f;
#pragma unroll
  for (int k = 0; k < CPL; ++k)
#pragma unroll
    for (int j = 0; j < 8; ++j) {
      w[k][j] = coef[8 * (c + k * LPR) + j];
      wshift += w[k][j];
      acc[k][j] = 0.f;
    }
  wshift *= kSynthShift;
  float rs = 0.f;
  float acc_r = 0.f, acc_loss = 0.f, acc_w = 0.f;

  const uint32_t Tr = (uint32_t)(n_res / RT), Tl = (uint32_t)(n_lin / RT);
  const uint32_t gw = blockIdx.x * kWavesPerBlock + wid, nw = gridDim.x * kWavesPerBlock;
  const uint32_t nr = gw < Tr ? (Tr - gw + nw - 1) / nw : 0u;
  const uint32_t nl = gw < Tl ? (Tl - gw + nw - 1) / nw : 0u;
  const uint32_t S = nr + nl;
  int64_t br = (int64_t)gw * RT, bl = br;
  using lds_byte = __attribute__((address_space(3))) unsigned char;
  for (int e = threadIdx.x; e < kStgFragBytes / 16; e += kBlock) {
    const int s = e >> 6, term = e & 15, q = (e & 63) >> 4;
    uint32_t p[4] = {0u, 0u, 0u, 0u};
    if (term < 3) {
      const float* cw = coef + 8 * (8 * q + s);
#pragma unroll
      for (int j = 0; j < 4; ++j) {
        const float x0 = cw[2 * j], x1 = cw[2 * j + 1];
        const uint32_t ph = pk_bf16(x0, x1);
        const float r0 = x0 - __uint_as_float(ph << 16), r1 = x1 - __uint_as_float(ph & 0xffff0000u);
        const uint32_t pm = pk_bf16(r0, r1);
        const uint32_t pl = pk_bf16(r0 - __uint_as_float(pm << 16), r1 - __uint_as_float(pm & 0xffff0000u));
        p[j] = term == 0 ? ph : term == 1 ? pm : pl;
      }
    }
    uint32_t* const dst = reinterpret_cast<uint32_t*>(frags + e * 16);
#pragma unroll
    for (int j = 0; j < 4; ++j) dst[j] = p[j];
  }
  __syncthreads();
  TileStage st{slots + wid * kStgWaveBytes,
               (uint32_t)(uintptr_t)(lds_byte*)slots + wid * kStgWaveBytes,
               (uint32_t)(uintptr_t)(lds_byte*)frags,
               reinterpret_cast<const unsigned char*>(X + br * ld),
               y + br,
               y_lin + bl,
               (int64_t)nw * RT,
               nr,
               nl,
               false};
  static_assert(RowReduce<LPR, UNROLL>::NF == 1, "TileStage::label_off: one label per lane");
  if (nl > 0) st.issue_label(g, c);
  if (nr > 0) st.issue_tile(lane);
  uint32_t rem = 0;
  for (uint32_t s = 0; s < S; ++s) {
    rem += nl;
    if (rem >= S) {
      rem -= S;
      grad_tile<RowsLineage, LPR, CPL, UNROLL, LOSS, SMP, true, true>(bl, n_lin, X, ld, CPL * LPR, y_lin, nullptr, seed, row0,
                                                                      w, wshift, intercept, g, c, smp_lin, acc, rs, acc_r,
                                                                      acc_loss, acc_w, &st);
      bl += st.tstep;
    } else {
      staged_resident_tile<LOSS, SMP>(br, intercept, lane, smp_res, acc, acc_r, acc_loss, acc_w, &st);
      br += st.tstep;
    }
  }
#pragma unroll
  for (int k = 0; k < CPL; ++k)
#pragma unroll
    for (int j = 0; j < 8; ++j) acc[k][j] = fmaf(rs, kSynthShift, acc[k][j]);
  grad_epilogue<LPR, CPL>(acc, acc_r, acc_loss, acc_w, partial, pstride, pacc, lane, wid, c);
}

template <class SRC, int LPR, int CPL, int U, bool UNW, bool FULL = false>
__device__ __forceinline__ void stats_tile(int64_t base, int64_t n, const typename SRC::elem* __restrict__ X,
                                           int64_t ld, int nch, const float* __restrict__ y,
                                           const float* __restrict__ sw, uint32_t seed, int64_t row0, int g, int c,
                                           float2_ (&s1)[CPL][4], float2_ (&s2)[CPL][4], float2_ (&syx)[CPL][4],
                                           float (&rsum)[3]) {
  constexpr int G = kWave / LPR;
  typename SRC::chunk xv[U][CPL];
  uint32_t fk[U];
  float yv[U], wv[U];
#pragma unroll
  for (int u = 0; u < U; ++u) {
    const int64_t row = base + u * G + g;
    const bool ok = row < n;
    const int64_t rowc = FULL ? row : (ok ? row : n - 1);
    yv[u] = y[rowc];
    if (UNW) {
      wv[u] = 1.f;
    } else if constexpr (FULL) {
      wv[u] = sw[row];
    } else {
      const float w0 = sw ? sw[rowc] : 1.f;
      wv[u] = ok ? w0 : 0.f;
    }
    if constexpr (SRC::kLineage) {
      fk[u] = feat_key(seed, row0 + rowc);
    } else {
#pragma unroll
      for (int k = 0; k < CPL; ++k) {
        const int ch = c + k * LPR;
        if constexpr (FULL) {
          SRC::load(X, ld, row, ch, xv[u][k]);
        } else {
          SRC::load(X, ld, rowc, ch < nch ? ch : nch - 1, xv[u][k]);
          SRC::mask(xv[u][k], ch < nch);
        }
      }
    }
  }
#pragma unroll
  for (int u = 0; u < U; ++u) {
    const float2_ w2 = {wv[u], wv[u]};
    const float wy = wv[u] * yv[u];
    const float2_ wy2 = {wy, wy};
#pragma unroll
    for (int k = 0; k < CPL; ++k) {
      float x[8];
      if constexpr (SRC::kLineage) {
        SRC::load(fk[u], c + k * LPR, xv[u][k]);
        SRC::values(xv[u][k], x);
      } else {
        SRC::unpack(xv[u][k], x);
      }
#pragma unroll
      for (int j = 0; j < 4; ++j) {
        const float2_ xx = {x[2 * j], x[2 * j + 1]};
        const float2_ wx = UNW ? xx : w2 * xx;
        s1[k][j] += wx;
        s2[k][j] = __builtin_elementwise_fma(wx, xx, s2[k][j]);
        syx[k][j] = __builtin_elementwise_fma(wy2, xx, syx[k][j]);
      }
    }
    if (c == 0) {
      rsum[0] += wv[u];
      rsum[1] += wy;
      rsum[2] = fmaf(wy, yv[u], rsum[2]);
    }
  }
}
template <int LPR, int CPL>
__device__ __forceinline__ void stats_epilogue(const float2_ (&s1)[CPL][4], const float2_ (&s2)[CPL][4],
                                               const float2_ (&syx)[CPL][4], const float (&rsum)[3],
                                               float* __restrict__ partial, int pstride, int lane, int wid, int c) {
  constexpr int DP = LPR * CPL * 8;
  __shared__ float red[kWavesPerBlock][3 * DP + 4];
#pragma unroll
  for (int k = 0; k < CPL; ++k)
#pragma unroll
    for (int j = 0; j < 4; ++j)
#pragma unroll
      for (int h = 0; h < 2; ++h) {
        float a = s1[k][j][h], b = s2[k][j][h], e = syx[k][j][h];
#pragma unroll
        for (int off = LPR; off < kWave; off <<= 1) {
          a += __shfl_xor(a, off, kWave);
          b += __shfl_xor(b, off, kWave);
          e += __shfl_xor(e, off, kWave);
        }
        const int col = 8 * (c + k * LPR) + 2 * j + h;
        if (lane < LPR) {
          red[wid][col] = a;
          red[wid][DP + col] = b;
          red[wid][2 * DP + col] = e;
        }
      }
#pragma unroll
  for (int q = 0; q < 3; ++q) {
    const float v = wave_sum(rsum[q]);
    if (lane == 0) red[wid][3 * DP + q] = v;
  }
  __syncthreads();
  for (int i = threadIdx.x; i < 3 * DP + 3; i += kBlock) {
    float s = 0.f;
#pragma unroll
    for (int q = 0; q < kWavesPerBlock; ++q) s += red[q][i];
    partial[(int64_t)blockIdx.x * pstride + i] = s;
  }
}

template <int LPR, int CPL, int MW, int FULL = 0>
__global__ __launch_bounds__(kBlock, MW) void glm_stats_mixed_kernel(
    const uint16_t* __restrict__ X, int64_t ld, int64_t n_res, const float* __restrict__ y,
    const float* __restrict__ sw, const float* __restrict__ y_lin, const float* __restrict__ sw_lin, uint32_t seed,
    int64_t row0, int64_t n_lin, float* __restrict__ partial, int pstride) {
  constexpr int G = kWave / LPR;
  constexpr int U = CPL >= 8 ? 1 : 8 / CPL;
  constexpr int RT = G * U;
  const int lane = threadIdx.x & (kWave - 1);
  const int wid = threadIdx.x / kWave;
  const int g = lane / LPR, c = lane % LPR;
  const int nch = (int)(ld / 8);
  float2_ s1[CPL][4], s2[CPL][4], syx[CPL][4];
#pragma unroll
  for (int k = 0; k < CPL; ++k)
#pragma unroll
    for (int j = 0; j < 4; ++j) s1[k][j] = s2[k][j] = syx[k][j] = float2_{0.f, 0.f};
  float rsum[3] = {0.f, 0.f, 0.f};
  const int64_t Tr = (n_res + RT - 1) / RT, Tl = (n_lin + RT - 1) / RT, S = Tr + Tl;
  const int64_t gw = (int64_t)blockIdx.x * kWavesPerBlock + wid;
  const int64_t nw = (int64_t)gridDim.x * kWavesPerBlock;
  if (gw < S) {
    int64_t L = gw * Tl / S, rem = gw * Tl - L * S;
    const int64_t q0 = nw * Tl / S, r0 = nw * Tl - q0 * S;
    for (int64_t s = gw; s < S; s += nw) {
      if constexpr (FULL != 0) {
        if (rem + Tl >= S)
          stats_tile<RowsLineage, LPR, CPL, U, FULL == 1, true>(L * RT, n_lin, X, ld, nch, y_lin, sw_lin, seed, row0, g, c,
                                                               s1, s2, syx, rsum);
        else
          stats_tile<RowsBf16, LPR, CPL, U, FULL == 1, true>((s - L) * RT, n_res, X, ld, nch, y, sw, seed, row0, g, c, s1,
                                                            s2, syx, rsum);
      } else if (rem + Tl >= S) {
        const int64_t base = L * RT;
        if (sw == nullptr && base + RT <= n_lin)
          stats_tile<RowsLineage, LPR, CPL, U, true>(base, n_lin, X, ld, nch, y_lin, sw_lin, seed, row0, g, c, s1,
                                                     s2, syx, rsum);
        else
          stats_tile<RowsLineage, LPR, CPL, U, false>(base, n_lin, X, ld, nch, y_lin, sw_lin, seed, row0, g, c, s1,
                                                      s2, syx, rsum);
      } else {
        const int64_t base = (s - L) * RT;
        if (sw == nullptr && base + RT <= n_res)
          stats_tile<RowsBf16, LPR, CPL, U, true>(base, n_res, X, ld, nch, y, sw, seed, row0, g, c, s1, s2, syx, rsum);
        else
          stats_tile<RowsBf16, LPR, CPL, U, false>(base, n_res, X, ld, nch, y, sw, seed, row0, g, c, s1, s2, syx, rsum);
      }
      rem += r0;
      L += q0;
      if (rem >= S) { rem -= S; ++L; }
    }
  }
  stats_epilogue<LPR, CPL>(s1, s2, syx, rsum, partial, pstride, lane, wid, c);
}

template <int LPR, int CPL>
__global__ __launch_bounds__(kBlock) void synth_glm_kernel(
    uint16_t* __restrict__ X, int64_t ld, int64_t n, float* __restrict__ y, uint32_t seed,
    int64_t row0, const float* __restrict__ wtrue, float btrue) {
  constexpr int G = kWave / LPR;
  const int lane = threadIdx.x & (kWave - 1);
  const int g = lane / LPR, c = lane % LPR;
  float wt[CPL][8];
#pragma unroll
  for (int k = 0; k < CPL; ++k)
#pragma unroll
    for (int j = 0; j < 8; ++j) {
      const int col = 8 * (c + k * LPR) + j;
      wt[k][j] = col < ld ? wtrue[col] : 0.f;
    }
  const int64_t gw = ((int64_t)blockIdx.x * blockDim.x + threadIdx.x) / kWave;
  const int64_t nw = ((int64_t)gridDim.x * blockDim.x) / kWave;
  const int64_t ntiles = (n + G - 1) / G;
  for (int64_t t = gw; t < ntiles; t += nw) {
    const int64_t row = t * G + g;
    const bool ok = row < n;
    const uint32_t rk = row_key(seed, row0 + row), fk = feat_key(seed, row0 + row);
    float dt = 0.f;
#pragma unroll
    for (int k = 0; k < CPL; ++k) {
      const int ch = c + k * LPR;
      if (8 * ch < ld) {
        short8 v = synth_chunk(fk, ch);
        float x[8];
        unpack8(v, x);
#pragma unroll
        for (int j = 0; j < 8; ++j) dt = fmaf(x[j], wt[k][j], dt);
        if (ok) *reinterpret_cast<short8*>(X + row * ld + 8 * ch) = v;
      }
    }
    dt = group_sum<LPR>(dt);
    if (ok && c == 0) y[row] = synth_label(rk, dt + btrue);
  }
}

template <class SRC, int LPR, int CPL, int U>
__device__ __forceinline__ void margin_body(const typename SRC::elem* __restrict__ X, int64_t ld, int64_t n,
                                            const float* __restrict__ coef, float intercept,
                                            float* __restrict__ out) {
  constexpr int G = kWave / LPR;
  const int lane = threadIdx.x & (kWave - 1);
  const int g = lane / LPR, c = lane % LPR;
  const int nch = (int)(ld / 8);
  float w[CPL][8];
  load_coef<LPR, CPL>(coef, ld, c, w);
  const int64_t gw = ((int64_t)blockIdx.x * blockDim.x + threadIdx.x) / kWave;
  const int64_t nw = ((int64_t)gridDim.x * blockDim.x) / kWave;
  const int64_t RT = (int64_t)G * U;
  const int64_t ntiles = (n + RT - 1) / RT;
  for (int64_t t = gw; t < ntiles; t += nw) {
    typename SRC::chunk xv[U][CPL];
#pragma unroll
    for (int u = 0; u < U; ++u) {
      const int64_t row = t * RT + u * G + g;
#pragma unroll
      for (int k = 0; k < CPL; ++k) {
        const int ch = c + k * LPR;
        SRC::load_if(X, ld, row, ch, row < n && ch < nch, xv[u][k]);
      }
    }
#pragma unroll
    for (int u = 0; u < U; ++u) {
      const int64_t row = t * RT + u * G + g;
      float d = 0.f;
#pragma unroll
      for (int k = 0; k < CPL; ++k) {
        float x[8];
        SRC::unpack(xv[u][k], x);
#pragma unroll
        for (int j = 0; j < 8; ++j) d = fmaf(x[j], w[k][j], d);
      }
      d = group_sum<LPR>(d);
      if (row < n && c == 0) out[row] = d + intercept;
    }
  }
}
template <int LPR, int CPL>
__global__ __launch_bounds__(kBlock) void glm_margin_kernel(
    const uint16_t* __restrict__ X, int64_t ld, int64_t n, const float* __restrict__ coef,
    float intercept, float* __restrict__ out) {
  margin_body<RowsBf16, LPR, CPL, (CPL >= 8 ? 1 : 8 / CPL)>(X, ld, n, coef, intercept, out);
}

template <class SRC, int LPR, int CPL>
__device__ __forceinline__ void colstats_body(const typename SRC::elem* __restrict__ X, int64_t ld, int64_t n,
                                              const float* __restrict__ sw, uint32_t seed, int64_t row0,
                                              float* __restrict__ partial, int pstride) {
  constexpr int G = kWave / LPR;
  constexpr int UNROLL = CPL >= 4 ? 1 : 4 / CPL;
  constexpr int DP = LPR * CPL * 8;
  const int lane = threadIdx.x & (kWave - 1);
  const int wid = threadIdx.x / kWave;
  const int g = lane / LPR, c = lane % LPR;
  const int nch = (int)(ld / 8);
  float s1[CPL][8], s2[CPL][8];
  zero(s1);
  zero(s2);
  float sw_acc = 0.f;
  const int64_t RT = (int64_t)G * UNROLL;
  const int64_t ntiles = (n + RT - 1) / RT;
  const int64_t gw = (int64_t)blockIdx.x * kWavesPerBlock + wid;
  const int64_t nw = (int64_t)gridDim.x * kWavesPerBlock;
  for (int64_t t = gw; t < ntiles; t += nw) {
#pragma unroll
    for (int u = 0; u < UNROLL; ++u) {
      const int64_t row = t * RT + u * G + g;
      const bool ok = row < n;
      const int64_t rowc = ok ? row : n - 1;
      const float wv = sw ? sw[rowc] : 1.f;
      const float w = ok ? wv : 0.f;
#pragma unroll
      for (int k = 0; k < CPL; ++k) {
        const int ch = c + k * LPR;
        const int chc = ch < nch ? ch : nch - 1;
        const float wk = ch < nch ? w : 0.f;
        float x[8];
        if constexpr (SRC::kLineage) {
          unpack8(synth_chunk(feat_key(seed, row0 + rowc), chc), x);
        } else {
          typename SRC::chunk v;
          SRC::load(X, ld, rowc, chc, v);
          SRC::unpack(v, x);
        }
#pragma unroll
        for (int j = 0; j < 8; ++j) {
          const float wx = wk * x[j];
          s1[k][j] += wx;
          s2[k][j] = fmaf(wx, x[j], s2[k][j]);
        }
      }
      if (c == 0) sw_acc += w;
    }
  }
#pragma unroll
  for (int k = 0; k < CPL; ++k)
#pragma unroll
    for (int j = 0; j < 8; ++j) {
      float a = s1[k][j], b = s2[k][j];
#pragma unroll
      for (int off = LPR; off < kWave; off <<= 1) {
        a += __shfl_xor(a, off, kWave);
        b += __shfl_xor(b, off, kWave);
      }
      s1[k][j] = a;
      s2[k][j] = b;
    }
  sw_acc = wave_sum(sw_acc);
  __shared__ float red[2 * DP + 2];
  for (int q = 0; q < kWavesPerBlock; ++q) {
    if (wid == q) {
      if (lane < LPR) {
#pragma unroll
        for (int k = 0; k < CPL; ++k)
#pragma unroll
          for (int j = 0; j < 8; ++j) {
            const int i1 = 8 * (c + k * LPR) + j;
            red[i1] = (q == 0 ? 0.f : red[i1]) + s1[k][j];
            red[DP + i1] = (q == 0 ? 0.f : red[DP + i1]) + s2[k][j];
          }
      }
      if (lane == 0) red[2 * DP] = (q == 0 ? 0.f : red[2 * DP]) + sw_acc;
    }
    __syncthreads();
  }
  for (int i = threadIdx.x; i < 2 * DP + 1; i += kBlock) partial[(int64_t)blockIdx.x * pstride + i] = red[i];
}
template <int LPR, int CPL, int SRC>
__global__ __launch_bounds__(kBlock) void glm_colstats_kernel(
    const uint16_t* __restrict__ X, int64_t ld, int64_t n, const float* __restrict__ sw,
    uint32_t seed, int64_t row0, float* __restrict__ partial, int pstride) {
  colstats_body<std::conditional_t<SRC == 0, RowsBf16, RowsLineage>, LPR, CPL>(X, ld, n, sw, seed, row0, partial,
                                                                               pstride);
}

__global__ __launch_bounds__(1024) void glm_finish_kernel(const float* __restrict__ partial, int nblocks,
                                                          int pstride, int ncols, double* __restrict__ out,
                                                          int accumulate) {
  __shared__ double red[32][33];
  const int cx = threadIdx.x & 31, gy = threadIdx.x >> 5;
  const int i = blockIdx.x * 32 + cx;
  double s = 0.0;
  if (i < ncols)
    for (int b = gy; b < nblocks; b += 32) s += (double)partial[(int64_t)b * pstride + i];
  red[gy][cx] = s;
  __syncthreads();
  if (gy == 0 && i < ncols) {
    double t = 0.0;
#pragma unroll 8
    for (int q = 0; q < 32; ++q) t += red[q][cx];
    out[i] = accumulate ? out[i] + t : t;
  }
}

__global__ __launch_bounds__(256) void glm_sgd_update_kernel(
    const double* __restrict__ out, int dpad, double* __restrict__ bt, double* __restrict__ b,
    const double* __restrict__ inv_std, const double* __restrict__ l2v, double l2, double eta,
    int fit_intercept, float* __restrict__ coef_eff, double* __restrict__ loss_slot) {
  const double W = out[dpad + 2];
  const double invW = W > 0.0 ? 1.0 / W : 0.0;
  for (int i = threadIdx.x; i < dpad; i += blockDim.x) {
    const double inv = inv_std[i];
    const double reg = l2v ? l2v[i] : l2;
    const double v = bt[i] - eta * (out[i] * inv * invW + reg * bt[i]);
    bt[i] = v;
    coef_eff[i] = (float)(v * inv);
  }
  if (threadIdx.x == 0) {
    double bv = b[0];
    if (fit_intercept) bv -= eta * out[dpad] * invW;
    b[0] = bv;
    coef_eff[dpad] = (float)bv;
    if (loss_slot) loss_slot[0] = out[dpad + 1] * invW;
  }
}

__global__ __launch_bounds__(256) void glm_sgd_update_dev_kernel(
    const double* __restrict__ out, int dpad, double* __restrict__ bt, double* __restrict__ b,
    const double* __restrict__ inv_std, const double* __restrict__ l2v, double l2, const double* __restrict__ l1v,
    double l1, double step_size, int fit_intercept, float* __restrict__ coef_eff, double* __restrict__ loss_hist,
    int64_t cap, int64_t* __restrict__ t_dev) {
  const int64_t t = t_dev[0] + 1;
  const double eta = step_size / sqrt((double)t);
  const double W = out[dpad + 2];
  const double invW = W > 0.0 ? 1.0 / W : 0.0;
  const bool prox = l1v != nullptr || l1 > 0.0;
  for (int i = threadIdx.x; i < dpad; i += blockDim.x) {
    const double inv = inv_std[i];
    const double reg = l2v ? l2v[i] : l2;
    double v = bt[i] - eta * (out[i] * inv * invW + reg * bt[i]);
    if (prox) {
      const double sh = eta * (l1v ? l1v[i] : l1);
      v = v > sh ? v - sh : (v < -sh ? v + sh : 0.0);
    }
    bt[i] = v;
    coef_eff[i] = (float)(v * inv);
  }
  __syncthreads();
  if (threadIdx.x == 0) {
    double bv = b[0];
    if (fit_intercept) bv -= eta * out[dpad] * invW;
    b[0] = bv;
    coef_eff[dpad] = (float)bv;
    if (t <= cap) loss_hist[t - 1] = out[dpad + 1] * invW;
    t_dev[0] = t;
  }
}

int pick_lpr(int nch) {
  int l = 4;
  while (l < nch && l < 64) l <<= 1;
  return l;
}
int pick_cpl(int nch) {
  if (nch <= 64) return 1;
  const int need = (nch + 63) / 64;
  int c = 2;
  while (c < need) c <<= 1;
  return c;
}

struct Layout { int lpr, cpl, lpr_s, cpl_s, dpad; };
bool resolve_layout(int64_t ld, Layout* l) {
  const int nch = (int)(ld / 8);
  const int lpr = pick_lpr(nch), cpl = pick_cpl(nch);
  if (ld % 8 != 0 || cpl > 16) return false;
  int lpr_s = lpr, cpl_s = cpl;
  if (cpl == 1 && lpr >= 16) { lpr_s = lpr / 4; cpl_s = 4; }
  else if (cpl == 2) { lpr_s = 32; cpl_s = 4; }
  *l = Layout{lpr, cpl, lpr_s, cpl_s, lpr * cpl * 8};
  return true;
}

#define O3S_NATURAL_LAYOUTS(M) M(4, 1) M(8, 1) M(16, 1) M(32, 1) M(64, 1) M(64, 2) M(64, 4) M(64, 8) M(64, 16)
#define O3S_REMAPPED_LAYOUTS(M) M(4, 1) M(8, 1) M(4, 4) M(8, 4) M(16, 4) M(32, 4) M(64, 4) M(64, 8) M(64, 16)

template <int V> using IC = std::integral_constant<int, V>;
#define O3S_LAYOUT_CASE(L, C) \
  if (lpr == L && cpl == C) return f(IC<L>{}, IC<C>{});
template <class F>
int with_natural_layout(const Layout& l, F&& f) {
  const int lpr = l.lpr, cpl = l.cpl;
  O3S_NATURAL_LAYOUTS(O3S_LAYOUT_CASE)
  return -1;
}
template <class F>
int with_remapped_layout(const Layout& l, F&& f) {
  const int lpr = l.lpr_s, cpl = l.cpl_s;
  O3S_REMAPPED_LAYOUTS(O3S_LAYOUT_CASE)
  return -1;
}
#undef O3S_LAYOUT_CASE
#undef O3S_NATURAL_LAYOUTS
#undef O3S_REMAPPED_LAYOUTS
template <class F>
int with_loss(int loss, F&& f) {
  if (loss == LOSS_LOGISTIC) return f(IC<LOSS_LOGISTIC>{});
  if (loss == LOSS_HINGE) return f(IC<LOSS_HINGE>{});
  return f(IC<LOSS_SQUARED>{});
}
template <class F>
int with_remapped_layout_and_loss(const Layout& l, int loss, F&& f) {
  return with_remapped_layout(l, [&](auto L, auto C) {
    return with_loss(loss, [&](auto LOSS) { return f(L, C, LOSS); });
  });
}

template <class... P, class... A>
void launch(void (*kernel)(P...), int grid, hipStream_t st, A... args) {
  hipLaunchKernelGGL(kernel, dim3(grid), dim3(kBlock), 0, st, static_cast<P>(args)...);
}
int launch_finish(const float* partial, int grid, int pstride, int ncols, double* out, int accumulate,
                  hipStream_t st) {
  O3S_CHECK_LAUNCH();
  hipLaunchKernelGGL(glm_finish_kernel, dim3((ncols + 31) / 32), dim3(1024), 0, st, partial, grid, pstride, ncols,
                     out, accumulate);
  O3S_CHECK_LAUNCH();
  return 0;
}

template <class F>
int for_row_slices(int splits, int64_t n_res, int64_t n_lin, F&& slice, int64_t unit = 1) {
  const int K = splits < 1 ? 1 : splits;
  const auto cut = [&](int64_t n, int k) { return n * k / K / unit * unit; };
  for (int k = 0; k < K; ++k) {
    const int64_t r_lo = cut(n_res, k), l_lo = cut(n_lin, k);
    const int rc = slice(r_lo, cut(n_res, k + 1) - r_lo, l_lo, cut(n_lin, k + 1) - l_lo, k > 0);
    if (rc != 0) return rc;
    O3S_CHECK_LAUNCH();
  }
  return 0;
}

}

O3S_API int o3s_glm_layout(int64_t ld, int* dpad, int* pstride) {
  Layout l;
  if (!resolve_layout(ld, &l)) return -1;
  *dpad = l.dpad;
  *pstride = l.dpad + 4;
  return 0;
}

O3S_API int o3s_glm_grad(int loss, int src, const void* X, int64_t ld, int64_t n, const float* y,
                         const float* sw, const float* coef, uint32_t seed,
                         int64_t row0, const float* wtrue, float btrue, float* partial,
                         int grid, double* out, int accumulate, hipStream_t st) {
  Layout l;
  if (!resolve_layout(ld, &l) || grid <= 0) return -1;
  const int pstride = l.dpad + 4;
  const uint16_t* Xh = (const uint16_t*)X;
  if (n > 0) {
    const int rc = with_loss(loss, [&](auto LOSS) {
      if (src == 0)
        return with_natural_layout(l, [&](auto L, auto C) {
          constexpr int U = C == 1 ? 8 : (C == 2 ? 2 : 1);
          launch(glm_grad_kernel<L, C, U, LOSS, 0>, grid, st, Xh, ld, n, y, sw, coef, coef + l.dpad, seed, row0,
                 wtrue, btrue, partial, pstride);
          return 0;
        });
      return with_remapped_layout(l, [&](auto L, auto C) {
        constexpr int U = C >= 8 ? 1 : 8 / C;
        launch(glm_grad_kernel<L, C, U, LOSS, 1>, grid, st, Xh, ld, n, y, sw, coef, coef + l.dpad, seed, row0,
               wtrue, btrue, partial, pstride);
        return 0;
      });
    });
    if (rc != 0) return rc;
  } else {
    if (accumulate) return 0;
    hipMemsetAsync(partial, 0, sizeof(float) * pstride * (size_t)grid, st);
  }
  return launch_finish(partial, grid, pstride, l.dpad + 3, out, accumulate, st);
}

O3S_API int o3s_glm_grad_mixed(int loss, const void* X, int64_t ld, int64_t n_res, const float* y,
                               const float* sw, const float* coef, uint32_t seed, int64_t row0,
                               int64_t n_lin, float* partial, int grid, double* out, int waves,
                               int64_t res_row0, const int64_t* t_dev, uint32_t sseed,
                               uint32_t sthr, int splits, int full_tiles, int staged, hipStream_t st) {
  Layout l;
  if (!resolve_layout(ld, &l) || grid <= 0 || n_res < 0 || n_lin < 0) return -1;
  const int pstride = l.dpad + 4;
  const uint16_t* Xh = (const uint16_t*)X;
  const bool smp = sthr < (1u << 24);
  const int rc = with_remapped_layout_and_loss(l, loss, [&](auto L, auto C, auto LOSS) {
    constexpr int U = C >= 8 ? 1 : 8 / C;
    constexpr int64_t RT = (kWave / L) * U;
    auto slice = [&](auto FULL, int g, int64_t r_lo, int64_t r_n, int64_t l_lo, int64_t l_n, int pacc) {
      if (FULL && (r_n % RT != 0 || l_n % RT != 0 || ld != 8 * L * C)) return -1;
      const float* y_lin = y + n_res + l_lo;
      const float* sw_lin = sw ? sw + n_res + l_lo : nullptr;
      if constexpr (decltype(FULL)::value && L == TileStage::LPR && C == TileStage::CPL) {
        static_assert(U == TileStage::UNROLL, "the staged kernel's tile");
        const bool wanted = staged >= 2 || (staged == 1 && r_n > 0 && l_n > 0);
        if (wanted && !sw && r_n / RT < (int64_t(1) << 31) && l_n / RT < (int64_t(1) << 31)) {
          auto go_staged = [&](auto SMP) {
            launch(glm_grad_staged_kernel<LOSS, SMP>, g, st, Xh + r_lo * ld, r_n, y + r_lo, y_lin, coef, coef + l.dpad,
                   seed, row0 + l_lo, l_n, partial, pstride, res_row0 + r_lo, t_dev, sseed, sthr, pacc);
          };
          if (smp) go_staged(std::true_type{});
          else go_staged(std::false_type{});
          return 0;
        }
      }
      auto go = [&](auto MW, auto SMP) {
        launch(glm_grad_mixed_kernel<L, C, U, LOSS, MW, SMP, FULL>, g, st, Xh + r_lo * ld, ld, r_n, y + r_lo,
               sw ? sw + r_lo : nullptr, y_lin, sw_lin, coef, coef + l.dpad, seed, row0 + l_lo, l_n, partial, pstride,
               res_row0 + r_lo, t_dev, sseed, sthr, pacc);
      };
      if (waves == 3 && smp) go(IC<3>{}, std::true_type{});
      else if (waves == 3) go(IC<3>{}, std::false_type{});
      else if (smp) go(IC<2>{}, std::true_type{});
      else go(IC<2>{}, std::false_type{});
      return 0;
    };
    constexpr bool kHasFull = !(L >= 32 && C == 4);
    const int64_t r_full = n_res / RT * RT, l_full = n_lin / RT * RT;
    if constexpr (kHasFull) {
      if (full_tiles && ld == 8 * L * C && r_full + l_full > 0) {
        const int rc = for_row_slices(
            splits, n_res, n_lin,
            [&](int64_t r_lo, int64_t r_n, int64_t l_lo, int64_t l_n, int pacc) {
              return slice(std::true_type{}, grid, r_lo, r_n, l_lo, l_n, pacc);
            },
            RT);
        if (rc != 0 || (r_full == n_res && l_full == n_lin)) return rc;
        const int rc2 = slice(std::false_type{}, 1, r_full, n_res - r_full, l_full, n_lin - l_full, 1);
        O3S_CHECK_LAUNCH();
        return rc2;
      }
    }
    return for_row_slices(splits, n_res, n_lin, [&](int64_t r_lo, int64_t r_n, int64_t l_lo, int64_t l_n, int pacc) {
      return slice(std::false_type{}, grid, r_lo, r_n, l_lo, l_n, pacc);
    });
  });
  if (rc != 0) return rc;
  return launch_finish(partial, grid, pstride, l.dpad + 3, out, 0, st);
}

O3S_API int o3s_synth_glm(void* X, int64_t ld, int64_t n, float* y, uint32_t seed, int64_t row0,
                          const float* wtrue, float btrue, int grid, hipStream_t st) {
  Layout l;
  if (!resolve_layout(ld, &l)) return -1;
  if (n <= 0) return 0;
  return with_natural_layout(l, [&](auto L, auto C) {
    launch(synth_glm_kernel<L, C>, grid, st, (uint16_t*)X, ld, n, y, seed, row0,
           wtrue, btrue);
    O3S_CHECK_LAUNCH();
    return 0;
  });
}

O3S_API int o3s_glm_margin(const void* X, int64_t ld, int64_t n, const float* coef,
                           float intercept, float* out, int grid, hipStream_t st) {
  Layout l;
  if (!resolve_layout(ld, &l)) return -1;
  if (n <= 0) return 0;
  return with_natural_layout(l, [&](auto L, auto C) {
    launch(glm_margin_kernel<L, C>, grid, st, (const uint16_t*)X, ld, n, coef,
           intercept, out);
    O3S_CHECK_LAUNCH();
    return 0;
  });
}

O3S_API int o3s_glm_colstats(int src, const void* X, int64_t ld, int64_t n, const float* sw,
                             uint32_t seed, int64_t row0, float* partial, int grid, double* out,
                             hipStream_t st) {
  Layout l;
  if (!resolve_layout(ld, &l) || grid <= 0) return -1;
  const int pstride = 2 * l.dpad + 2;
  const uint16_t* Xh = (const uint16_t*)X;
  if (n > 0) {
    const int rc = with_natural_layout(l, [&](auto L, auto C) {
      if (src == 0) launch(glm_colstats_kernel<L, C, 0>, grid, st, Xh, ld, n, sw, seed, row0, partial, pstride);
      else launch(glm_colstats_kernel<L, C, 1>, grid, st, Xh, ld, n, sw, seed, row0, partial, pstride);
      return 0;
    });
    if (rc != 0) return rc;
  } else {
    hipMemsetAsync(partial, 0, sizeof(float) * pstride * (size_t)grid, st);
  }
  return launch_finish(partial, grid, pstride, 2 * l.dpad + 1, out, 0, st);
}

O3S_API int o3s_glm_sgd_update(const double* out, int dpad, double* bt, double* b, const double* inv_std,
                               const double* l2v, double l2, double eta, int fit_intercept, float* coef_eff,
                               double* loss_slot, hipStream_t st) {
  hipLaunchKernelGGL(glm_sgd_update_kernel, dim3(1), dim3(256), 0, st, out, dpad, bt, b, inv_std, l2v, l2,
                     eta, fit_intercept, coef_eff, loss_slot);
  O3S_CHECK_LAUNCH();
  return 0;
}

O3S_API int o3s_glm_sgd_update_dev(const double* out, int dpad, double* bt, double* b, const double* inv_std,
                                   const double* l2v, double l2, const double* l1v, double l1, double step_size,
                                   int fit_intercept, float* coef_eff, double* loss_hist, int64_t cap,
                                   int64_t* t_dev, hipStream_t st) {
  hipLaunchKernelGGL(glm_sgd_update_dev_kernel, dim3(1), dim3(256), 0, st, out, dpad, bt, b, inv_std, l2v, l2,
                     l1v, l1, step_size, fit_intercept, coef_eff, loss_hist, cap, t_dev);
  O3S_CHECK_LAUNCH();
  return 0;
}

O3S_API int o3s_glm_stats_mixed(const void* X, int64_t ld, int64_t n_res, const float* y, const float* sw,
                                uint32_t seed, int64_t row0, int64_t n_lin, float* partial, int grid, double* out,
                                int waves, int full_tiles, hipStream_t st) {
  Layout l;
  if (!resolve_layout(ld, &l) || grid <= 0 || n_res < 0 || n_lin < 0) return -1;
  const int pstride = 3 * l.dpad + 4;
  const uint16_t* Xh = (const uint16_t*)X;
  int slab_rows = grid;
  const int rc = with_remapped_layout(l, [&](auto L, auto C) {
    if constexpr (C > 4) {
      return -2;
    } else {
      constexpr int64_t RT = (kWave / L) * (8 / C);
      auto pass = [&](auto FULL, int g, float* slab, int64_t r_lo, int64_t r_n, int64_t l_lo, int64_t l_n) {
        if (FULL != 0 && (r_n % RT != 0 || l_n % RT != 0 || ld != 8 * L * C || (FULL == 2) != (sw != nullptr)))
          return -1;
        auto go = [&](auto MW) {
          launch(glm_stats_mixed_kernel<L, C, MW, FULL>, g, st, Xh + r_lo * ld, ld, r_n, y + r_lo,
                 sw ? sw + r_lo : nullptr, y + n_res + l_lo, sw ? sw + n_res + l_lo : nullptr, seed, row0 + l_lo, l_n,
                 slab, pstride);
        };
        if constexpr (FULL == 0) {
          if (waves == 3) go(IC<3>{});
          else go(IC<2>{});
        } else {
          go(IC<2>{});
        }
        return 0;
      };
      if constexpr (L < 64) {
        const int64_t r_full = n_res / RT * RT, l_full = n_lin / RT * RT;
        if (full_tiles && ld == 8 * L * C && r_full + l_full > 0) {
          const int rc = sw ? pass(IC<2>{}, grid, partial, 0, r_full, 0, l_full)
                            : pass(IC<1>{}, grid, partial, 0, r_full, 0, l_full);
          if (rc != 0 || (r_full == n_res && l_full == n_lin)) return rc;
          O3S_CHECK_LAUNCH();
          slab_rows = grid + 1;
          return pass(IC<0>{}, 1, partial + (size_t)grid * pstride, r_full, n_res - r_full, l_full, n_lin - l_full);
        }
      }
      return pass(IC<0>{}, grid, partial, 0, n_res, 0, n_lin);
    }
  });
  if (rc != 0) return rc;
  return launch_finish(partial, slab_rows, pstride, 3 * l.dpad + 3, out, 0, st);
}

namespace {

typedef float sm_f32x16 __attribute__((ext_vector_type(16)));
typedef short sm_bf16x8 __attribute__((ext_vector_type(8)));
constexpr int kSmWaves = 4;
constexpr int kSmThreads = kSmWaves * kWave;

template <int NB>
struct SmLds {
  static constexpr int D = 32 * NB;
  static constexpr int WLD = D + 8;
  static constexpr int XLD = D + 8;
  static constexpr int RLD = 40;
  static constexpr int W_ELEMS = 3 * 32 * WLD;
  static constexpr int WAVE_ELEMS = 32 * XLD + 2 * 32 * RLD;
  static constexpr int ELEMS = W_ELEMS + kSmWaves * WAVE_ELEMS;
};

template <int NB>
__global__ __launch_bounds__(kSmThreads, 1) void glm_softmax_kernel(
    const uint16_t* __restrict__ X, int64_t n, int64_t ldx, const int32_t* __restrict__ y,
    const float* __restrict__ sw, const uint16_t* __restrict__ Wsp, const float* __restrict__ bias, int K,
    float* __restrict__ partial, int pstride) {
  using L = SmLds<NB>;
  constexpr int D = L::D, KS = 2 * NB, WLD = L::WLD, XLD = L::XLD, RLD = L::RLD;
  __shared__ __attribute__((aligned(16))) uint16_t smem[L::ELEMS];
  const int lane = threadIdx.x & 63, wid = threadIdx.x >> 6;
  const int r = lane & 31, h = lane >> 5;
  uint16_t* Ws = smem;
  uint16_t* Xs = smem + L::W_ELEMS + wid * L::WAVE_ELEMS;
  uint16_t* Rs = Xs + 32 * XLD;

  for (int p = threadIdx.x; p < 3 * 32 * (D / 8); p += kSmThreads) {
    const int row = p / (D / 8), k8 = p % (D / 8);
    *reinterpret_cast<sm_bf16x8*>(Ws + row * WLD + k8 * 8) =
        *reinterpret_cast<const sm_bf16x8*>(Wsp + (int64_t)row * D + k8 * 8);
  }
  float bl[16];
  int cls[16];
#pragma unroll
  for (int v = 0; v < 16; ++v) {
    cls[v] = 8 * (v >> 2) + 4 * h + (v & 3);
    bl[v] = cls[v] < K ? bias[cls[v]] : -INFINITY;
  }
  __syncthreads();

  sm_f32x16 G[NB];
#pragma unroll
  for (int b = 0; b < NB; ++b)
#pragma unroll
    for (int v = 0; v < 16; ++v) G[b][v] = 0.f;
  float gb[16];
#pragma unroll
  for (int v = 0; v < 16; ++v) gb[v] = 0.f;
  float lossacc = 0.f;

  const int64_t ntiles = (n + 31) / 32;
  const int64_t step = (int64_t)gridDim.x * kSmWaves;
  int64_t tile = (int64_t)blockIdx.x * kSmWaves + wid;
  sm_bf16x8 xb[KS], xn[KS];
  auto load = [&](int64_t t, sm_bf16x8 (&dst)[KS]) {
    int64_t row = t * 32 + r;
    row = row < n ? row : n - 1;
    const uint16_t* src = X + row * ldx;
#pragma unroll
    for (int ks = 0; ks < KS; ++ks) {
      const int col = ks * 16 + 8 * h;
      if (col < ldx) {
        dst[ks] = *reinterpret_cast<const sm_bf16x8*>(src + col);
      } else {
#pragma unroll
        for (int j = 0; j < 8; ++j) dst[ks][j] = 0;
      }
    }
  };
  if (tile < ntiles) load(tile, xb);
  for (; tile < ntiles; tile += step) {
    if (tile + step < ntiles) load(tile + step, xn);
    const int64_t row = tile * 32 + r;
    const bool valid = row < n;
    const int yl = valid ? y[row] : -1;
    const float wr = valid ? (sw ? sw[row] : 1.f) : 0.f;
    sm_f32x16 acc;
#pragma unroll
    for (int v = 0; v < 16; ++v) acc[v] = bl[v];
#pragma unroll
    for (int ks = 0; ks < KS; ++ks) {
#pragma unroll
      for (int s = 0; s < 3; ++s) {
        const sm_bf16x8 a = *reinterpret_cast<const sm_bf16x8*>(Ws + (s * 32 + r) * WLD + ks * 16 + 8 * h);
        acc = __builtin_amdgcn_mfma_f32_32x32x16_bf16(a, xb[ks], acc, 0, 0, 0);
      }
      *reinterpret_cast<sm_bf16x8*>(Xs + r * XLD + ks * 16 + 8 * h) = xb[ks];
    }
    float mx = -INFINITY;
#pragma unroll
    for (int v = 0; v < 16; ++v) mx = fmaxf(mx, acc[v]);
    mx = fmaxf(mx, __shfl_xor(mx, 32, 64));
    float se = 0.f;
#pragma unroll
    for (int v = 0; v < 16; ++v) se += __expf(acc[v] - mx);
    se += __shfl_xor(se, 32, 64);
    const float lse = mx + __logf(se);
#pragma unroll
    for (int v = 0; v < 16; ++v) {
      const bool hit = cls[v] == yl;
      const float p = __expf(acc[v] - lse);
      const float rv = wr * (p - (hit ? 1.f : 0.f));
      gb[v] += rv;
      if (hit) lossacc += wr * (lse - acc[v]);
      const uint16_t a0 = f32_to_bf16(rv);
      Rs[(0 * 32 + cls[v]) * RLD + r] = a0;
      Rs[(1 * 32 + cls[v]) * RLD + r] = f32_to_bf16(rv - bf16_to_f32(a0));
    }
    asm volatile("s_waitcnt lgkmcnt(0)" ::: "memory");
    __builtin_amdgcn_wave_barrier();
    sm_bf16x8 ar[2][2];
#pragma unroll
    for (int rs = 0; rs < 2; ++rs)
#pragma unroll
      for (int s = 0; s < 2; ++s)
        ar[rs][s] = *reinterpret_cast<const sm_bf16x8*>(Rs + (s * 32 + r) * RLD + rs * 16 + 8 * h);
#pragma unroll
    for (int b = 0; b < NB; ++b) {
#pragma unroll
      for (int rs = 0; rs < 2; ++rs) {
        sm_bf16x8 bx;
#pragma unroll
        for (int q = 0; q < 8; ++q) bx[q] = (short)Xs[(rs * 16 + 8 * h + q) * XLD + b * 32 + r];
#pragma unroll
        for (int s = 0; s < 2; ++s) G[b] = __builtin_amdgcn_mfma_f32_32x32x16_bf16(ar[rs][s], bx, G[b], 0, 0, 0);
      }
    }
    asm volatile("s_waitcnt lgkmcnt(0)" ::: "memory");
    __builtin_amdgcn_wave_barrier();
#pragma unroll
    for (int ks = 0; ks < KS; ++ks) xb[ks] = xn[ks];
  }
  float* out = partial + ((int64_t)blockIdx.x * kSmWaves + wid) * pstride;
#pragma unroll
  for (int b = 0; b < NB; ++b)
#pragma unroll
    for (int v = 0; v < 16; ++v) out[cls[v] * D + b * 32 + r] = G[b][v];
#pragma unroll
  for (int v = 0; v < 16; ++v) {
    float s = gb[v];
#pragma unroll
    for (int off = 16; off > 0; off >>= 1) s += __shfl_xor(s, off, 64);
    if (r == 0) out[32 * D + cls[v]] = s;
  }
  const float lt = wave_sum(lossacc);
  if (lane == 0) out[32 * D + 32] = lt;
}

}

O3S_API int o3s_glm_softmax(const void* X, int64_t n, int64_t ldx, int d, const int32_t* y, const float* sw,
                            const void* Wsp, const float* bias, int K, float* partial, int grid, double* out,
                            hipStream_t st) {
  const int nb = (d + 31) / 32;
  if (ldx % 8 != 0 || nb < 1 || nb > 8 || K < 1 || K > 32 || grid <= 0) return -1;
  const int D = 32 * nb, pstride = 32 * D + 33;
  const uint16_t* Xh = (const uint16_t*)X;
  const uint16_t* Wh = (const uint16_t*)Wsp;
  if (n > 0) {
    switch (nb) {
#define O3S_SM(NBV) \
  case NBV: hipLaunchKernelGGL((glm_softmax_kernel<NBV>), dim3(grid), dim3(kSmThreads), 0, st, Xh, n, ldx, y, sw, \
                               Wh, bias, K, partial, pstride); break;
      O3S_SM(1) O3S_SM(2) O3S_SM(3) O3S_SM(4) O3S_SM(5) O3S_SM(6) O3S_SM(7) O3S_SM(8)
#undef O3S_SM
      default: return -1;
    }
  } else {
    hipMemsetAsync(partial, 0, sizeof(float) * pstride * (size_t)grid * kSmWaves, st);
  }
  O3S_CHECK_LAUNCH();
  hipLaunchKernelGGL(glm_finish_kernel, dim3((pstride + 31) / 32), dim3(1024), 0, st, partial, grid * kSmWaves,
                     pstride, pstride, out, 0);
  O3S_CHECK_LAUNCH();
  return 0;
}

namespace {

template <int LPR, int CPL, int UNROLL, int LOSS, int MW, bool SMP>
__global__ __launch_bounds__(kBlock, MW) void glm_grad_f32_kernel(
    const float* __restrict__ X, int64_t ld, int64_t n, const float* __restrict__ y, const float* __restrict__ sw,
    const float* __restrict__ coef, const float* __restrict__ bptr, float* __restrict__ partial, int pstride,
    int64_t res_row0, const int64_t* __restrict__ t_dev, uint32_t sseed, uint32_t sthr, int pacc) {
  constexpr int G = kWave / LPR;
  constexpr int RT = G * UNROLL;
  using RR = RowReduce<LPR, UNROLL>;
  constexpr int NF = RR::NF;
  constexpr bool kDpp = LPR == 8 && UNROLL == 2;
  const int lane = threadIdx.x & (kWave - 1);
  const int wid = threadIdx.x / kWave;
  const int g = lane / LPR, c = lane % LPR;
  const int nch = (int)(ld / 8);
  const int ubase = RR::base(c);
  const bool rep = RR::representative(c);
  const float intercept = *bptr;
  const uint32_t skey = SMP ? sample_key(sseed, (uint32_t)((t_dev ? t_dev[0] : 0) + 1)) : 0u;
  const RowSampler smp{skey, sthr, res_row0};

  float w[CPL][8], acc[CPL][8];
#pragma unroll
  for (int k = 0; k < CPL; ++k)
#pragma unroll
    for (int j = 0; j < 8; ++j) {
      const int col = 8 * (c + k * LPR) + j;
      w[k][j] = col < ld ? coef[col] : 0.f;
      acc[k][j] = 0.f;
    }
  float acc_r = 0.f, acc_loss = 0.f, acc_w = 0.f;

  const int64_t ntiles = (n + RT - 1) / RT;
  const int64_t gw = (int64_t)blockIdx.x * kWavesPerBlock + wid;
  const int64_t nw = (int64_t)gridDim.x * kWavesPerBlock;
  for (int64_t t = gw; t < ntiles; t += nw) {
    const int64_t base = t * RT;
    float4_ xv[UNROLL][CPL][2];
#pragma unroll
    for (int u = 0; u < UNROLL; ++u) {
      const int64_t row = base + u * G + g;
      const bool ok = row < n;
      const int64_t rowc = ok ? row : n - 1;
#pragma unroll
      for (int k = 0; k < CPL; ++k) {
        const int ch = c + k * LPR;
        const int chc = ch < nch ? ch : nch - 1;
        RowsF32::chunk v;
        RowsF32::load(X, ld, rowc, chc, v);
        RowsF32::mask(v, ok && ch < nch);
        xv[u][k][0] = v.lo;
        xv[u][k][1] = v.hi;
      }
    }
    float yy[NF], ww[NF];
#pragma unroll
    for (int j = 0; j < NF; ++j) {
      const int64_t row = base + (ubase + j) * G + g;
      const bool ok = row < n;
      const int64_t rowc = ok ? row : n - 1;
      const float yv = y[rowc];
      const float wv = sw ? sw[rowc] : 1.f;
      yy[j] = ok ? yv : 0.f;
      ww[j] = ok ? wv : 0.f;
      if constexpr (SMP) {
        if (!smp.keep(row)) ww[j] = 0.f;
      }
    }
    float dot[UNROLL];
#pragma unroll
    for (int u = 0; u < UNROLL; ++u) {
      float2_ d2 = {0.f, 0.f};
#pragma unroll
      for (int k = 0; k < CPL; ++k)
#pragma unroll
        for (int h = 0; h < 2; ++h)
#pragma unroll
          for (int j = 0; j < 4; j += 2) {
            const float2_ xx = {xv[u][k][h][j], xv[u][k][h][j + 1]};
            const float2_ ww2 = {w[k][4 * h + j], w[k][4 * h + j + 1]};
            d2 = __builtin_elementwise_fma(xx, ww2, d2);
          }
      dot[u] = d2.x + d2.y;
    }
    if constexpr (kDpp) row_reduce_8x2(dot, c);
    else RR::run(dot, c);
    float res[NF];
#pragma unroll
    for (int j = 0; j < NF; ++j) {
      float r, l;
      loss_terms<LOSS>(dot[j] + intercept, yy[j], ww[j], r, l);
      res[j] = r;
      if (rep) { acc_r += r; acc_loss += l; acc_w += ww[j]; }
    }
    float other = 0.f;
    if constexpr (kDpp) other = dpp_f<kDppHalfMirror>(res[0]);
#pragma unroll
    for (int u = 0; u < UNROLL; ++u) {
      float r;
      if constexpr (kDpp) r = ((c & 4) != 0) == (u == 0) ? other : res[0];
      else r = __shfl(res[u % NF], g * LPR + RR::owner(u), kWave);
#pragma unroll
      for (int k = 0; k < CPL; ++k)
#pragma unroll
        for (int h = 0; h < 2; ++h)
#pragma unroll
          for (int j = 0; j < 4; ++j) acc[k][4 * h + j] = fmaf(r, xv[u][k][h][j], acc[k][4 * h + j]);
    }
  }

  grad_epilogue<LPR, CPL>(acc, acc_r, acc_loss, acc_w, partial, pstride, pacc, lane, wid, c);
}

template <int LPR, int CPL, int U, int MW>
__global__ __launch_bounds__(kBlock, MW) void glm_stats_f32_kernel(
    const float* __restrict__ X, int64_t ld, int64_t n, const float* __restrict__ y, const float* __restrict__ sw,
    float* __restrict__ partial, int pstride) {
  constexpr int RT = kWave / LPR * U;
  const int lane = threadIdx.x & (kWave - 1);
  const int wid = threadIdx.x / kWave;
  const int g = lane / LPR, c = lane % LPR;
  const int nch = (int)(ld / 8);
  float2_ s1[CPL][4], s2[CPL][4], syx[CPL][4];
#pragma unroll
  for (int k = 0; k < CPL; ++k)
#pragma unroll
    for (int j = 0; j < 4; ++j) s1[k][j] = s2[k][j] = syx[k][j] = float2_{0.f, 0.f};
  float rsum[3] = {0.f, 0.f, 0.f};
  const int64_t ntiles = (n + RT - 1) / RT;
  const int64_t gw = (int64_t)blockIdx.x * kWavesPerBlock + wid;
  const int64_t nw = (int64_t)gridDim.x * kWavesPerBlock;
  for (int64_t t = gw; t < ntiles; t += nw) {
    const int64_t base = t * RT;
    if (sw == nullptr && base + RT <= n)
      stats_tile<RowsF32, LPR, CPL, U, true>(base, n, X, ld, nch, y, sw, 0u, 0, g, c, s1, s2, syx, rsum);
    else
      stats_tile<RowsF32, LPR, CPL, U, false>(base, n, X, ld, nch, y, sw, 0u, 0, g, c, s1, s2, syx, rsum);
  }
  stats_epilogue<LPR, CPL>(s1, s2, syx, rsum, partial, pstride, lane, wid, c);
}

template <int LPR, int CPL>
__global__ __launch_bounds__(kBlock) void glm_margin_f32_kernel(
    const float* __restrict__ X, int64_t ld, int64_t n, const float* __restrict__ coef, float intercept,
    float* __restrict__ out) {
  margin_body<RowsF32, LPR, CPL, (CPL >= 4 ? 1 : 4 / CPL)>(X, ld, n, coef, intercept, out);
}

template <int LPR, int CPL>
__global__ __launch_bounds__(kBlock) void glm_colstats_f32_kernel(
    const float* __restrict__ X, int64_t ld, int64_t n, const float* __restrict__ sw, float* __restrict__ partial,
    int pstride) {
  colstats_body<RowsF32, LPR, CPL>(X, ld, n, sw, 0u, 0, partial, pstride);
}

template <int C> struct F32Cfg { static constexpr int U = C >= 8 ? 1 : 8 / C, MW = C >= 8 ? 1 : 2; };

}

O3S_API int o3s_glm_grad_f32(int loss, const void* X, int64_t ld, int64_t n, const float* y, const float* sw,
                             const float* coef, int64_t n_lin, float* partial, int grid, double* out,
                             int accumulate, int64_t res_row0, const int64_t* t_dev, uint32_t sseed, uint32_t sthr,
                             int splits, hipStream_t st) {
  Layout l;
  if (ld <= 0 || !resolve_layout(ld, &l) || grid <= 0 || n < 0 || n_lin != 0) return -1;
  const int pstride = l.dpad + 4;
  const float* Xf = (const float*)X;
  const bool smp = sthr < (1u << 24);
  const int rc = for_row_slices(splits, n, 0, [&](int64_t r_lo, int64_t r_n, int64_t, int64_t, int pacc) {
    return with_remapped_layout_and_loss(l, loss, [&](auto L, auto C, auto LOSS) {
      constexpr int U = F32Cfg<C>::U, MW = F32Cfg<C>::MW;
      auto go = [&](auto SMP) {
        launch(glm_grad_f32_kernel<L, C, U, LOSS, MW, SMP>, grid, st, Xf + r_lo * ld, ld, r_n, y + r_lo,
               sw ? sw + r_lo : nullptr, coef, coef + l.dpad, partial, pstride, res_row0 + r_lo, t_dev, sseed, sthr,
               pacc);
      };
      if (smp) go(std::true_type{});
      else go(std::false_type{});
      return 0;
    });
  });
  if (rc != 0) return rc;
  return launch_finish(partial, grid, pstride, l.dpad + 3, out, accumulate, st);
}

O3S_API int o3s_glm_stats_f32(const void* X, int64_t ld, int64_t n, const float* y, const float* sw, int64_t n_lin,
                              float* partial, int grid, double* out, hipStream_t st) {
  Layout l;
  if (ld <= 0 || !resolve_layout(ld, &l) || grid <= 0 || n < 0 || n_lin != 0) return -1;
  const int pstride = 3 * l.dpad + 4;
  const int rc = with_remapped_layout(l, [&](auto L, auto C) {
    if constexpr (C > 4) {
      return -2;
    } else {
      launch(glm_stats_f32_kernel<L, C, (C >= 4 ? 1 : 4 / C), 2>, grid, st, (const float*)X, ld, n, y, sw, partial,
             pstride);
      return 0;
    }
  });
  if (rc != 0) return rc;
  return launch_finish(partial, grid, pstride, 3 * l.dpad + 3, out, 0, st);
}

O3S_API int o3s_glm_margin_f32(const void* X, int64_t ld, int64_t n, const float* coef, float intercept, float* out,
                               int grid, hipStream_t st) {
  Layout l;
  if (ld <= 0 || !resolve_layout(ld, &l) || grid <= 0) return -1;
  if (n <= 0) return 0;
  return with_remapped_layout(l, [&](auto L, auto C) {
    launch(glm_margin_f32_kernel<L, C>, grid, st, (const float*)X, ld, n, coef,
           intercept, out);
    O3S_CHECK_LAUNCH();
    return 0;
  });
}

O3S_API int o3s_glm_colstats_f32(const void* X, int64_t ld, int64_t n, const float* sw, float* partial, int grid,
                                 double* out, hipStream_t st) {
  Layout l;
  if (ld <= 0 || !resolve_layout(ld, &l) || grid <= 0 || n < 0) return -1;
  const int pstride = 2 * l.dpad + 2;
  if (n > 0) {
    const int rc = with_remapped_layout(l, [&](auto L, auto C) {
      launch(glm_colstats_f32_kernel<L, C>, grid, st, (const float*)X, ld, n, sw,
             partial, pstride);
      return 0;
    });
    if (rc != 0) return rc;
  } else {
    hipMemsetAsync(partial, 0, sizeof(float) * pstride * (size_t)grid, st);
  }
  return launch_finish(partial, grid, pstride, 2 * l.dpad + 1, out, 0, st);
}

namespace {

typedef uint32_t sm_u32x4 __attribute__((ext_vector_type(4)));

__device__ __forceinline__ void split8(const float4_ a, const float4_ b, sm_bf16x8& hi, sm_bf16x8& mid,
                                       sm_bf16x8& lo) {
  sm_u32x4 ph, pm, pl;
#pragma unroll
  for (int j = 0; j < 4; ++j) {
    const float x0 = j < 2 ? a[2 * j] : b[2 * j - 4], x1 = j < 2 ? a[2 * j + 1] : b[2 * j - 3];
    ph[j] = pk_bf16(x0, x1);
    const float r0 = x0 - __uint_as_float(ph[j] << 16), r1 = x1 - __uint_as_float(ph[j] & 0xffff0000u);
    pm[j] = pk_bf16(r0, r1);
    pl[j] = pk_bf16(r0 - __uint_as_float(pm[j] << 16), r1 - __uint_as_float(pm[j] & 0xffff0000u));
  }
  hi = __builtin_bit_cast(sm_bf16x8, ph);
  mid = __builtin_bit_cast(sm_bf16x8, pm);
  lo = __builtin_bit_cast(sm_bf16x8, pl);
}

template <int NB>
__global__ __launch_bounds__(kSmThreads, 1) void glm_softmax_f32_kernel(
    const float* __restrict__ X, int64_t n, int64_t ldx, const int32_t* __restrict__ y,
    const float* __restrict__ sw, const uint16_t* __restrict__ Wsp, const float* __restrict__ bias, int K,
    float* __restrict__ partial, int pstride) {
  using L = SmLds<NB>;
  constexpr int D = L::D, KS = 2 * NB, WLD = L::WLD, XLD = L::XLD, RLD = L::RLD;
  __shared__ __attribute__((aligned(16))) uint16_t smem[L::ELEMS];
  __shared__ __attribute__((aligned(16))) float bs[32];
  const int lane = threadIdx.x & 63, wid = threadIdx.x >> 6;
  const int r = lane & 31, h = lane >> 5;
  uint16_t* Ws = smem;
  uint16_t* Xs = smem + L::W_ELEMS + wid * L::WAVE_ELEMS;
  uint16_t* Rs = Xs + 32 * XLD;

  for (int p = threadIdx.x; p < 3 * 32 * (D / 8); p += kSmThreads) {
    const int row = p / (D / 8), k8 = p % (D / 8);
    *reinterpret_cast<sm_bf16x8*>(Ws + row * WLD + k8 * 8) =
        *reinterpret_cast<const sm_bf16x8*>(Wsp + (int64_t)row * D + k8 * 8);
  }
  auto cv = [](int v) { return 8 * (v >> 2) + (v & 3); };
  if (threadIdx.x < 32) bs[threadIdx.x] = (int)threadIdx.x < K ? bias[threadIdx.x] : -INFINITY;
  uint16_t* Rw = Rs + 4 * h * RLD + r;
  __syncthreads();

  sm_f32x16 G[NB];
#pragma unroll
  for (int b = 0; b < NB; ++b)
#pragma unroll
    for (int v = 0; v < 16; ++v) G[b][v] = 0.f;
  float gb[16];
#pragma unroll
  for (int v = 0; v < 16; ++v) gb[v] = 0.f;
  float lossacc = 0.f;

  const int64_t ntiles = (n + 31) / 32;
  const int64_t step = (int64_t)gridDim.x * kSmWaves;
  int64_t tile = (int64_t)blockIdx.x * kSmWaves + wid;
  float4_ xf[KS][2], xn[KS][2];
  auto load = [&](int64_t t, float4_ (*dst)[2]) {
    int64_t row = t * 32 + r;
    row = row < n ? row : n - 1;
    const float* src = X + row * ldx;
#pragma unroll
    for (int ks = 0; ks < KS; ++ks) {
      const int col = ks * 16 + 8 * h;
      if (col < ldx) {
        dst[ks][0] = *reinterpret_cast<const float4_*>(src + col);
        dst[ks][1] = *reinterpret_cast<const float4_*>(src + col + 4);
      } else {
#pragma unroll
        for (int j = 0; j < 4; ++j) dst[ks][0][j] = dst[ks][1][j] = 0.f;
      }
    }
  };
  if (tile < ntiles) load(tile, xf);
  for (; tile < ntiles; tile += step) {
    if (tile + step < ntiles) load(tile + step, xn);
    const int64_t row = tile * 32 + r;
    const bool valid = row < n;
    const int ylh = (valid ? y[row] : -1) - 4 * h;
    const float wr = valid ? (sw ? sw[row] : 1.f) : 0.f;
    sm_f32x16 acc;
#pragma unroll
    for (int j = 0; j < 4; ++j) {
      const float4_ b4 = *reinterpret_cast<const float4_*>(bs + 8 * j + 4 * h);
#pragma unroll
      for (int u = 0; u < 4; ++u) acc[4 * j + u] = b4[u];
    }
    sm_bf16x8 xh[KS], xm[KS];
#pragma unroll
    for (int ks = 0; ks < KS; ++ks) {
      sm_bf16x8 xl;
      split8(xf[ks][0], xf[ks][1], xh[ks], xm[ks], xl);
      const uint16_t* wp = Ws + r * WLD + ks * 16 + 8 * h;
      const sm_bf16x8 a0 = *reinterpret_cast<const sm_bf16x8*>(wp);
      const sm_bf16x8 a1 = *reinterpret_cast<const sm_bf16x8*>(wp + 32 * WLD);
      const sm_bf16x8 a2 = *reinterpret_cast<const sm_bf16x8*>(wp + 64 * WLD);
      acc = __builtin_amdgcn_mfma_f32_32x32x16_bf16(a0, xl, acc, 0, 0, 0);
      acc = __builtin_amdgcn_mfma_f32_32x32x16_bf16(a2, xh[ks], acc, 0, 0, 0);
      acc = __builtin_amdgcn_mfma_f32_32x32x16_bf16(a1, xm[ks], acc, 0, 0, 0);
      acc = __builtin_amdgcn_mfma_f32_32x32x16_bf16(a0, xm[ks], acc, 0, 0, 0);
      acc = __builtin_amdgcn_mfma_f32_32x32x16_bf16(a1, xh[ks], acc, 0, 0, 0);
      acc = __builtin_amdgcn_mfma_f32_32x32x16_bf16(a0, xh[ks], acc, 0, 0, 0);
      __builtin_amdgcn_sched_barrier(0);
    }
    float mx = -INFINITY;
#pragma unroll
    for (int v = 0; v < 16; ++v) mx = fmaxf(mx, acc[v]);
    mx = fmaxf(mx, __shfl_xor(mx, 32, 64));
    float se = 0.f;
#pragma unroll
    for (int v = 0; v < 16; ++v) se += __expf(acc[v] - mx);
    se += __shfl_xor(se, 32, 64);
    const float lse = mx + __logf(se);
#pragma unroll
    for (int v = 0; v < 16; v += 2) {
      float rv[2];
#pragma unroll
      for (int u = 0; u < 2; ++u) {
        const bool hit = cv(v + u) == ylh;
        rv[u] = wr * (__expf(acc[v + u] - lse) - (hit ? 1.f : 0.f));
        gb[v + u] += rv[u];
        if (hit) lossacc += wr * (lse - acc[v + u]);
      }
      const uint32_t ph = pk_bf16(rv[0], rv[1]);
      const uint32_t pl = pk_bf16(rv[0] - __uint_as_float(ph << 16), rv[1] - __uint_as_float(ph & 0xffff0000u));
      Rw[cv(v) * RLD] = (uint16_t)ph;
      Rw[cv(v + 1) * RLD] = (uint16_t)(ph >> 16);
      Rw[(32 + cv(v)) * RLD] = (uint16_t)pl;
      Rw[(32 + cv(v + 1)) * RLD] = (uint16_t)(pl >> 16);
    }
    asm volatile("s_waitcnt lgkmcnt(0)" ::: "memory");
    __builtin_amdgcn_wave_barrier();
    sm_bf16x8 ar[2][2];
#pragma unroll
    for (int rs = 0; rs < 2; ++rs)
#pragma unroll
      for (int s = 0; s < 2; ++s)
        ar[rs][s] = *reinterpret_cast<const sm_bf16x8*>(Rs + (s * 32 + r) * RLD + rs * 16 + 8 * h);
#pragma unroll
    for (int rs = 0; rs < 2; ++rs) {
      if ((r >> 4) == rs) {
#pragma unroll
        for (int ks = 0; ks < KS; ++ks) {
          *reinterpret_cast<sm_bf16x8*>(Xs + (r & 15) * XLD + ks * 16 + 8 * h) = xh[ks];
          *reinterpret_cast<sm_bf16x8*>(Xs + (16 + (r & 15)) * XLD + ks * 16 + 8 * h) = xm[ks];
        }
      }
      asm volatile("s_waitcnt lgkmcnt(0)" ::: "memory");
      __builtin_amdgcn_wave_barrier();
#pragma unroll
      for (int b = 0; b < NB; ++b) {
        sm_bf16x8 bh, bm;
#pragma unroll
        for (int q = 0; q < 8; ++q) {
          bh[q] = (short)Xs[(8 * h + q) * XLD + b * 32 + r];
          bm[q] = (short)Xs[(16 + 8 * h + q) * XLD + b * 32 + r];
        }
        G[b] = __builtin_amdgcn_mfma_f32_32x32x16_bf16(ar[rs][1], bm, G[b], 0, 0, 0);
        G[b] = __builtin_amdgcn_mfma_f32_32x32x16_bf16(ar[rs][0], bm, G[b], 0, 0, 0);
        G[b] = __builtin_amdgcn_mfma_f32_32x32x16_bf16(ar[rs][1], bh, G[b], 0, 0, 0);
        G[b] = __builtin_amdgcn_mfma_f32_32x32x16_bf16(ar[rs][0], bh, G[b], 0, 0, 0);
        __builtin_amdgcn_sched_barrier(0);
      }
      asm volatile("s_waitcnt lgkmcnt(0)" ::: "memory");
      __builtin_amdgcn_wave_barrier();
    }
#pragma unroll
    for (int ks = 0; ks < KS; ++ks) {
      xf[ks][0] = xn[ks][0];
      xf[ks][1] = xn[ks][1];
    }
  }
  float* out = partial + ((int64_t)blockIdx.x * kSmWaves + wid) * pstride;
#pragma unroll
  for (int b = 0; b < NB; ++b)
#pragma unroll
    for (int v = 0; v < 16; ++v) out[(4 * h + cv(v)) * D + b * 32 + r] = G[b][v];
#pragma unroll
  for (int v = 0; v < 16; ++v) {
    float s = gb[v];
#pragma unroll
    for (int off = 16; off > 0; off >>= 1) s += __shfl_xor(s, off, 64);
    if (r == 0) out[32 * D + 4 * h + cv(v)] = s;
  }
  const float lt = wave_sum(lossacc);
  if (lane == 0) out[32 * D + 32] = lt;
}

}

O3S_API int o3s_glm_softmax_f32(const void* X, int64_t n, int64_t ldx, int d, const int32_t* y, const float* sw,
                                const void* Wsp, const float* bias, int K, float* partial, int grid, double* out,
                                hipStream_t st) {
  const int nb = (d + 31) / 32;
  if (ldx % 8 != 0 || nb < 1 || nb > 8 || K < 1 || K > 32 || grid <= 0) return -1;
  const int D = 32 * nb, pstride = 32 * D + 33;
  const float* Xf = (const float*)X;
  const uint16_t* Wh = (const uint16_t*)Wsp;
  if (n > 0) {
    switch (nb) {
#define O3S_SM(NBV) \
  case NBV: hipLaunchKernelGGL((glm_softmax_f32_kernel<NBV>), dim3(grid), dim3(kSmThreads), 0, st, Xf, n, ldx, y, \
                               sw, Wh, bias, K, partial, pstride); break;
      O3S_SM(1) O3S_SM(2) O3S_SM(3) O3S_SM(4) O3S_SM(5) O3S_SM(6) O3S_SM(7) O3S_SM(8)
#undef O3S_SM
      default: return -1;
    }
  } else {
    hipMemsetAsync(partial, 0, sizeof(float) * pstride * (size_t)grid * kSmWaves, st);
  }
  O3S_CHECK_LAUNCH();
  hipLaunchKernelGGL(glm_finish_kernel, dim3((pstride + 31) / 32), dim3(1024), 0, st, partial, grid * kSmWaves,
                     pstride, pstride, out, 0);
  O3S_CHECK_LAUNCH();
  return 0;
}

O3S_PRELOAD(glm)
```

### orange3_spark_amd/ops/glm.py

```python
from __future__ import annotations

import os

import numpy as np
import torch

from . import _native as N

LOSS_LOGISTIC, LOSS_HINGE, LOSS_SQUARED = 0, 1, 2
_MASK = 0xFFFFFFFF


def padded_width(d: int) -> int:
    return max(8, (d + 7) // 8 * 8)


def f32_rows(X: torch.Tensor) -> bool:
    return (X.is_cuda and X.dtype == torch.float32 and X.dim() == 2 and X.is_contiguous()
            and X.shape[1] > 0 and X.shape[1] % 8 == 0)


def kernel_rows(X: torch.Tensor) -> bool:
    return (X.is_cuda and X.dtype == torch.bfloat16 and X.is_contiguous()) or f32_rows(X)


def layout(ld: int) -> tuple[int, int]:
    nch = ld // 8
    lpr = 4
    while lpr < nch and lpr < 64:
        lpr <<= 1
    cpl = 1
    if nch > 64:
        need = (nch + 63) // 64
        cpl = 2
        while cpl < need:
            cpl <<= 1
    if cpl > 16:
        raise ValueError(f"feature dimension {ld} too large for the fused GLM kernel")
    dpad = lpr * cpl * 8
    return dpad, dpad + 4


def _fmix32(h: torch.Tensor) -> torch.Tensor:
    h = h ^ (h >> 16)
    h = (h * 0x85EBCA6B) & _MASK
    h = h ^ (h >> 13)
    h = (h * 0xC2B2AE35) & _MASK
    return h ^ (h >> 16)


def row_keys(seed: int, rows: torch.Tensor) -> torch.Tensor:
    lo = rows & _MASK
    hi = rows >> 32
    inner = (lo * 0x9E3779B1 + hi * 0x7FEB352D + 0x165667B1) & _MASK
    return _fmix32((seed & _MASK) ^ _fmix32(inner))


def _mix24(h: torch.Tensor) -> torch.Tensor:
    h = h ^ (h >> 16)
    h = ((h & 0xFFFFFF) * 0xED5AD4 + h) & _MASK
    h = h ^ (h >> 15)
    return ((h & 0xFFFFFF) * 0x2C1B3C + h) & _MASK


def feat_keys(seed: int, rows: torch.Tensor) -> torch.Tensor:
    lo = rows & _MASK
    hi = rows >> 32
    k = _mix24((lo + ((seed * 0x9E3779B1) & _MASK)) & _MASK)
    return _mix24(k ^ (((hi & 0xFFFFFF) * 0x7FEB35 + 0x165667) & _MASK))


def synth_features_torch(fk: torch.Tensor, ld: int, d: int) -> torch.Tensor:
    n = fk.shape[0]
    words = torch.arange(ld // 4, dtype=torch.int64, device=fk.device)
    h = _mix24((fk[:, None] + words[None, :] * 0x9E3779) & _MASK)
    shifts = torch.arange(4, dtype=torch.int64, device=fk.device) * 8
    b = (h[:, :, None] >> shifts) & 0xFF
    return ((2 * b - 255).to(torch.float32) * (1.0 / 256.0)).reshape(n, ld).to(torch.bfloat16)


def synth_labels_torch(rk: torch.Tensor, margin_true: torch.Tensor) -> torch.Tensor:
    u = (_fmix32(rk ^ 0xA511E9B3) >> 8).to(torch.float32) * (1.0 / 16777216.0)
    return (u < torch.sigmoid(margin_true.to(torch.float32))).to(torch.float32)


def synth_truth(seed: int, d: int, ld: int | None = None) -> tuple[torch.Tensor, float]:
    ld = ld or padded_width(d)
    rng = np.random.default_rng(seed ^ 0x5EED)
    w = np.zeros(ld, dtype=np.float32)
    w[:d] = rng.standard_normal(d).astype(np.float32) * np.float32(np.sqrt(12.0 / max(d, 1)))
    b = float(rng.standard_normal() * 0.25)
    return torch.from_numpy(w), b


def synth_glm(n: int, d: int, seed: int, row0: int = 0, device="cpu", ld: int | None = None,
              wtrue: torch.Tensor | None = None, btrue: float | None = None):
    ld = ld or padded_width(d)
    if wtrue is None:
        wtrue, btrue = synth_truth(seed, d, ld)
    device = torch.device(device)
    X = torch.empty((n, ld), dtype=torch.bfloat16, device=device)
    y = torch.empty((n,), dtype=torch.float32, device=device)
    if n == 0:
        return X, y
    if device.type == "cuda":
        lib = N.kernels()
        wt = wtrue.to(device=device, dtype=torch.float32).contiguous()
        grid = N.grid_for(device, n, 256)
        N.check(lib.o3s_synth_glm(X.data_ptr(), ld, n, y.data_ptr(), seed & _MASK, row0,
                                  wt.data_ptr(), float(btrue), grid, N.stream_of(X)), "synth_glm")
        return X, y
    step = 1 << 16
    for s in range(0, n, step):
        e = min(n, s + step)
        rows = torch.arange(row0 + s, row0 + e, dtype=torch.int64)
        rk = row_keys(seed, rows)
        xs = synth_features_torch(feat_keys(seed, rows), ld, d)
        X[s:e] = xs
        y[s:e] = synth_labels_torch(rk, xs.float() @ wtrue.float() + btrue)
    return X, y


def _loss_terms(m: torch.Tensor, y: torch.Tensor, w: torch.Tensor, loss: int):
    if loss == LOSS_LOGISTIC:
        r = (torch.sigmoid(m) - y) * w
        l = w * (torch.nn.functional.softplus(m) - y * m)
    elif loss == LOSS_HINGE:
        s = 2.0 * y - 1.0
        mg = 1.0 - s * m
        act = (mg > 0).to(m.dtype)
        r = -s * w * act
        l = w * mg * act
    else:
        e = m - y
        r = e * w
        l = 0.5 * w * e * e
    return r, l


def glm_grad_torch(X, y, sw, coef, intercept, loss: int) -> torch.Tensor:
    Xd = X.to(torch.float64)
    m = Xd @ coef.to(torch.float64)[: X.shape[1]] + float(intercept)
    yd = y.to(torch.float64)
    w = torch.ones_like(yd) if sw is None else sw.to(torch.float64)
    r, l = _loss_terms(m, yd, w, loss)
    g = Xd.T @ r
    return torch.cat([g, torch.stack([r.sum(), l.sum(), w.sum()])])


class GlmWorkspace:

    def __init__(self, device: torch.device, ld: int, grid: int | None = None):
        self.device = torch.device(device)
        self.ld = ld
        self.dpad, self.pstride = layout(ld)
        self.grid = grid or (N.num_cus(self.device) * 8 if self.device.type == "cuda" else 1)
        self.partial = torch.empty(self.grid * self.pstride, dtype=torch.float32, device=self.device)
        self.out = torch.empty(self.dpad + 3, dtype=torch.float64, device=self.device)


_ROWS_MSG = ("GPU GLM pass expects a contiguous bf16 feature matrix (or a contiguous fp32 one whose row "
             "stride is a multiple of 8)")


def glm_grad(X: torch.Tensor, y: torch.Tensor, sw: torch.Tensor | None, coef: torch.Tensor,
             intercept: float | None, loss: int, ws: GlmWorkspace | None = None,
             accumulate: bool = False) -> torch.Tensor:
    ld = X.shape[1]
    if X.is_cuda:
        if not kernel_rows(X):
            raise TypeError(_ROWS_MSG)
        ws = ws or GlmWorkspace(X.device, ld)
        cf = _coef_buf(coef, ws.dpad, X.device, intercept=intercept)
        lib = N.kernels()
        if X.dtype == torch.float32:
            N.check(lib.o3s_glm_grad_f32(loss, X.data_ptr(), ld, X.shape[0], y.data_ptr(), N.ptr(sw),
                                         cf.data_ptr(), 0, ws.partial.data_ptr(), ws.grid, ws.out.data_ptr(),
                                         int(accumulate), 0, None, 0, 1 << 24, 1, N.stream_of(X)), "glm_grad_f32")
            return ws.out
        N.check(lib.o3s_glm_grad(loss, 0, X.data_ptr(), ld, X.shape[0], y.data_ptr(),
                                 N.ptr(sw), cf.data_ptr(), 0, 0, None, 0.0,
                                 ws.partial.data_ptr(), ws.grid, ws.out.data_ptr(), int(accumulate),
                                 N.stream_of(X)), "glm_grad")
        return ws.out
    if intercept is None:
        intercept = float(coef[-1])
    dpad, _ = layout(ld)
    ref = glm_grad_torch(X, y, sw, coef.to(torch.float64)[:ld], intercept, loss)
    out = torch.zeros(dpad + 3, dtype=torch.float64)
    out[:ld] = ref[:ld]
    out[dpad:] = ref[ld:]
    return out


def glm_grad_synth(n: int, ld: int, d: int, seed: int, row0: int, wtrue: torch.Tensor,
                   btrue: float, coef: torch.Tensor, intercept: float | None, loss: int,
                   ws: GlmWorkspace, accumulate: bool = False) -> torch.Tensor:
    if ws.device.type == "cuda":
        cf = _coef_buf(coef, ws.dpad, ws.device, intercept=intercept)
        wt = _coef_buf(wtrue, ws.dpad, ws.device, slot=1, intercept=0.0)
        lib = N.kernels()
        N.check(lib.o3s_glm_grad(loss, 1, None, ld, n, None, None, cf.data_ptr(),
                                 seed & _MASK, row0, wt.data_ptr(), float(btrue),
                                 ws.partial.data_ptr(), ws.grid, ws.out.data_ptr(), int(accumulate),
                                 torch.cuda.current_stream(ws.device).cuda_stream), "glm_grad_synth")
        return ws.out
    X, y = synth_glm(n, d, seed, row0, "cpu", ld, wtrue, btrue)
    out = glm_grad(X, y, None, coef, intercept, loss)
    if accumulate and ws is not None and getattr(ws, "out", None) is not None:
        ws.out += out
        return ws.out
    return out


MIX_WAVES = int(os.environ.get("O3S_GLM_MIX_WAVES", "3"))
STATS_WAVES = int(os.environ.get("O3S_GLM_STATS_WAVES", "2"))
MIX_SLICE_ROWS = int(os.environ.get("O3S_GLM_MIX_SLICE_ROWS", str(64 << 20)))
MIX_FULL_TILES = int(os.environ.get("O3S_GLM_MIX_FULL", "1"))
MIX_STAGED = int(os.environ.get("O3S_GLM_MIX_STAGED", "1"))


def mix_splits(n_rows: int) -> int:
    return max(1, min(16, n_rows // max(1, MIX_SLICE_ROWS)))


def sample_threshold(fraction: float) -> int:
    f = float(fraction)
    if not 0.0 < f <= 1.0:
        raise ValueError(f"miniBatchFraction must be in (0, 1], got {fraction}")
    return 1 << 24 if f >= 1.0 else max(1, int(round(f * (1 << 24))))


def sample_key(seed: int, it: int) -> int:
    t = torch.tensor([(int(it) * 0x9E3779B1 + 0x7F4A7C15) & _MASK], dtype=torch.int64)
    return int(_fmix32((int(seed) & _MASK) ^ _fmix32(t))[0])


def sample_mask(seed: int, it: int, grows: torch.Tensor, fraction: float) -> torch.Tensor:
    thr = sample_threshold(fraction)
    if thr >= 1 << 24:
        return torch.ones(grows.shape[0], dtype=torch.bool, device=grows.device)
    return (row_keys(sample_key(seed, it), grows.to(torch.int64)) >> 8) < thr


def glm_grad_mixed(X: torch.Tensor, y: torch.Tensor, sw: torch.Tensor | None, n_lin: int, d: int,
                   seed: int, row0: int, coef: torch.Tensor, intercept: float | None, loss: int,
                   ws: GlmWorkspace, res_row0: int = 0, t_dev: torch.Tensor | None = None,
                   sample_seed: int = 0, fraction: float = 1.0) -> torch.Tensor:
    ld = X.shape[1]
    nr = X.shape[0]
    if y.shape[0] != nr + n_lin or (sw is not None and sw.shape[0] != nr + n_lin):
        raise ValueError("label / weight columns must cover the resident and lineage rows")
    thr = sample_threshold(fraction)
    if ws.device.type != "cuda":
        Xl, _ = synth_glm(n_lin, d, seed, row0, "cpu", ld, torch.zeros(ld), 0.0)
        w = sw
        if thr < 1 << 24:
            it = int(t_dev[0]) + 1 if t_dev is not None else 1
            grows = torch.cat([torch.arange(res_row0, res_row0 + nr), torch.arange(row0, row0 + n_lin)])
            keep = sample_mask(sample_seed, it, grows, fraction).to(torch.float64)
            w = keep if sw is None else sw.to(torch.float64) * keep
        return glm_grad(torch.cat([X, Xl]), y, w, coef, intercept, loss)
    if not kernel_rows(X) or not y.is_contiguous():
        raise TypeError(_ROWS_MSG)
    if X.dtype == torch.float32:
        if n_lin:
            raise ValueError("fp32 feature rows have no lineage rows (lineage storage is bf16)")
        cf = _coef_buf(coef, ws.dpad, ws.device, intercept=intercept)
        N.check(N.kernels().o3s_glm_grad_f32(loss, X.data_ptr(), ld, nr, y.data_ptr(), N.ptr(sw), cf.data_ptr(),
                                             0, ws.partial.data_ptr(), ws.grid, ws.out.data_ptr(), 0,
                                             int(res_row0), N.ptr(t_dev), int(sample_seed) & _MASK, thr,
                                             mix_splits(nr), N.stream_of(X)), "glm_grad_f32")
        return ws.out
    cf = _coef_buf(coef, ws.dpad, ws.device, intercept=intercept)
    N.check(N.kernels().o3s_glm_grad_mixed(loss, X.data_ptr(), ld, nr, y.data_ptr(), N.ptr(sw),
                                           cf.data_ptr(), seed & _MASK, row0, n_lin, ws.partial.data_ptr(),
                                           ws.grid, ws.out.data_ptr(), MIX_WAVES, int(res_row0),
                                           N.ptr(t_dev), int(sample_seed) & _MASK, thr, mix_splits(nr + n_lin),
                                           MIX_FULL_TILES, MIX_STAGED, N.stream_of(X)),
            "glm_grad_mixed")
    return ws.out


def glm_stats_mixed(X: torch.Tensor, y: torch.Tensor, sw: torch.Tensor | None, n_lin: int, d: int,
                    seed: int, row0: int, grid: int | None = None) -> torch.Tensor | None:
    ld = X.shape[1]
    nr = X.shape[0]
    dpad, _ = layout(ld)
    if y.shape[0] != nr + n_lin or (sw is not None and sw.shape[0] != nr + n_lin):
        raise ValueError("label / weight columns must cover the resident and lineage rows")
    if X.device.type != "cuda":
        return glm_stats_torch(X, y, sw, n_lin, d, seed, row0)
    grid = grid or N.num_cus(X.device) * 16
    pstride = 3 * dpad + 4
    partial = torch.empty((grid + 1) * pstride, dtype=torch.float32, device=X.device)
    out = torch.empty(3 * dpad + 3, dtype=torch.float64, device=X.device)
    if f32_rows(X):
        if n_lin:
            raise ValueError("fp32 feature rows have no lineage rows (lineage storage is bf16)")
        rc = N.kernels().o3s_glm_stats_f32(X.data_ptr(), ld, nr, y.data_ptr(), N.ptr(sw), 0, partial.data_ptr(),
                                           grid, out.data_ptr(), N.stream_of(X))
        if rc == -2:
            return None
        N.check(rc, "glm_stats_f32")
        return out
    rc = N.kernels().o3s_glm_stats_mixed(X.data_ptr(), ld, nr, y.data_ptr(), N.ptr(sw), seed & _MASK, row0,
                                         n_lin, partial.data_ptr(), grid, out.data_ptr(), STATS_WAVES, MIX_FULL_TILES,
                                         N.stream_of(X))
    if rc == -2:
        return None
    N.check(rc, "glm_stats_mixed")
    return out


def glm_stats_torch(X, y, sw, n_lin=0, d=None, seed=0, row0=0) -> torch.Tensor:
    ld = X.shape[1]
    dpad, _ = layout(ld)
    if n_lin:
        Xl, _ = synth_glm(n_lin, d or ld, seed, row0, "cpu", ld, torch.zeros(ld), 0.0)
        X = torch.cat([X.cpu(), Xl])
    Xd = X.to(torch.float64).cpu()
    yd = y.to(torch.float64).cpu()
    w = torch.ones_like(yd) if sw is None else sw.to(torch.float64).cpu()
    out = torch.zeros(3 * dpad + 3, dtype=torch.float64)
    out[:ld] = w @ Xd
    out[dpad:dpad + ld] = w @ (Xd * Xd)
    out[2 * dpad:2 * dpad + ld] = (w * yd) @ Xd
    out[3 * dpad:] = torch.stack([w.sum(), (w * yd).sum(), (w * yd * yd).sum()])
    return out


_COEF_CACHE: dict = {}


def _coef_buf(coef: torch.Tensor, dpad: int, device, slot: int = 0,
              intercept: float | None = 0.0) -> torch.Tensor:
    if intercept is None:
        if coef.shape[0] != dpad + 1 or coef.dtype != torch.float32 or coef.device != torch.device(device):
            raise ValueError("coef operand must be fp32 [dpad + 1] on the pass device")
        return coef
    key = (str(device), dpad, slot)
    buf = _COEF_CACHE.get(key)
    if buf is None:
        buf = torch.zeros(dpad + 1, dtype=torch.float32, device=device)
        _COEF_CACHE[key] = buf
    k = min(coef.shape[0], dpad)
    buf[:k].copy_(coef[:k], non_blocking=True)
    if k < dpad:
        buf[k:dpad].zero_()
    buf[dpad] = float(intercept)
    return buf


def glm_margin(X: torch.Tensor, coef: torch.Tensor, intercept: float) -> torch.Tensor:
    ld = X.shape[1]
    if kernel_rows(X):
        dpad, _ = layout(ld)
        cf = torch.zeros(dpad, dtype=torch.float32, device=X.device)
        k = min(coef.shape[0], dpad)
        cf[:k] = coef[:k].to(X.device, torch.float32)
        out = torch.empty(X.shape[0], dtype=torch.float32, device=X.device)
        lib = N.kernels()
        fn, what = ((lib.o3s_glm_margin_f32, "glm_margin_f32") if X.dtype == torch.float32
                    else (lib.o3s_glm_margin, "glm_margin"))
        grid = N.grid_for(X.device, X.shape[0], 64)
        N.check(fn(X.data_ptr(), ld, X.shape[0], cf.data_ptr(), float(intercept), out.data_ptr(), grid,
                   N.stream_of(X)), what)
        return out
    c = coef.to(X.device, torch.float64)[:ld]
    return (X.to(torch.float64) @ c + float(intercept)).to(torch.float32)


def softmax_kernel_ok(X: torch.Tensor, K: int) -> bool:
    return (X.is_cuda and X.dtype in (torch.bfloat16, torch.float32) and X.dim() == 2 and X.stride(1) == 1
            and X.stride(0) % 8 == 0 and 1 <= X.shape[1] <= 256 and 1 <= K <= 32)


def softmax_pass(X: torch.Tensor, y: torch.Tensor, sw: torch.Tensor | None, W: torch.Tensor, b: torch.Tensor):
    n, d = X.shape
    K = W.shape[0]
    dev = X.device
    D = 32 * (-(-d // 32))
    Wp = torch.zeros((32, D), dtype=torch.float32, device=dev)
    Wp[:K, :d] = W
    hi = Wp.to(torch.bfloat16)
    r1 = Wp - hi.float()
    mid = r1.to(torch.bfloat16)
    lo = (r1 - mid.float()).to(torch.bfloat16)
    Wsp = torch.stack([hi, mid, lo]).contiguous()
    bp = torch.zeros(32, dtype=torch.float32, device=dev)
    bp[:K] = b
    grid = N.num_cus(dev)
    pstride = 32 * D + 33
    partial = torch.empty(grid * 4 * pstride, dtype=torch.float32, device=dev)
    out = torch.empty(pstride, dtype=torch.float64, device=dev)
    yi = y if y.dtype == torch.int32 else y.to(torch.int32)
    lib = N.kernels()
    fn = lib.o3s_glm_softmax_f32 if X.dtype == torch.float32 else lib.o3s_glm_softmax
    N.check(fn(X.data_ptr(), n, X.stride(0), d, yi.contiguous().data_ptr(),
               N.ptr(None if sw is None else sw.float().contiguous()),
               Wsp.data_ptr(), bp.data_ptr(), K, partial.data_ptr(), grid,
               out.data_ptr(), N.stream_of(X)), "glm_softmax")
    return out[: 32 * D].view(32, D)[:K, :d], out[32 * D:32 * D + K], out[32 * D + 32]


def softmax_pass_torch(X, y, sw, W, b):
    Xd = X.to(torch.float64)
    M = Xd @ W.to(torch.float64).T + b.to(torch.float64)
    lse = torch.logsumexp(M, 1)
    w = torch.ones(X.shape[0], dtype=torch.float64, device=X.device) if sw is None else sw.to(torch.float64)
    yl = y.long()
    P = torch.exp(M - lse[:, None])
    P[torch.arange(X.shape[0], device=X.device), yl] -= 1.0
    R = P * w[:, None]
    return R.T @ Xd, R.sum(0), (w * (lse - M.gather(1, yl[:, None]).squeeze(1))).sum()


def _colstats_out(ld: int, device, grid: int):
    dpad, _ = layout(ld)
    partial = torch.empty(grid * (2 * dpad + 2), dtype=torch.float32, device=device)
    out = torch.empty(2 * dpad + 1, dtype=torch.float64, device=device)
    return dpad, partial, out


def glm_colstats(X: torch.Tensor, sw: torch.Tensor | None = None) -> torch.Tensor:
    ld = X.shape[1]
    if kernel_rows(X):
        grid = N.num_cus(X.device) * 4
        dpad, partial, out = _colstats_out(ld, X.device, grid)
        lib = N.kernels()
        if X.dtype == torch.float32:
            N.check(lib.o3s_glm_colstats_f32(X.data_ptr(), ld, X.shape[0], N.ptr(sw), partial.data_ptr(), grid,
                                             out.data_ptr(), N.stream_of(X)), "glm_colstats_f32")
        else:
            N.check(lib.o3s_glm_colstats(0, X.data_ptr(), ld, X.shape[0], N.ptr(sw), 0, 0, partial.data_ptr(), grid,
                                         out.data_ptr(), N.stream_of(X)), "glm_colstats")
        return torch.cat([out[:ld], out[dpad:dpad + ld], out[2 * dpad:]])
    Xd = X.to(torch.float64)
    w = torch.ones(X.shape[0], dtype=torch.float64, device=X.device) if sw is None else sw.to(torch.float64)
    return torch.cat([w @ Xd, w @ (Xd * Xd), w.sum().reshape(1)])


def glm_colstats_synth(n: int, ld: int, d: int, seed: int, row0: int, device) -> torch.Tensor:
    device = torch.device(device)
    if device.type == "cuda":
        grid = N.num_cus(device) * 4
        dpad, partial, out = _colstats_out(ld, device, grid)
        N.check(N.kernels().o3s_glm_colstats(1, None, ld, n, None, seed & _MASK, row0, partial.data_ptr(), grid,
                                             out.data_ptr(), torch.cuda.current_stream(device).cuda_stream),
                "glm_colstats_synth")
        return torch.cat([out[:ld], out[dpad:dpad + ld], out[2 * dpad:]])
    X, _ = synth_glm(n, d, seed, row0, "cpu", ld, torch.zeros(ld), 0.0)
    return glm_colstats(X)
```

Baseline: 25.18 billion samples/s.

## Add persistent work-stealing GLM gradient kernel with per-item partial slab

Adds a persistent kernel for the mixed resident+lineage staged gradient pass. Waves claim fixed-size work items through an atomic ticket and prefetch the next item's tiles and labels while finishing the current one. Each item writes its partial sums to a slab, and a two-stage fp64 reduction then replaces the sliced multi-launch scheme and its grid partials. The aim is to cut load imbalance, launch and slice overhead, and tail effects, at the cost of an extra slab allocation, atomics and a larger final reduction.

Measured after the change: 25.75 billion samples/s, median of 6. 2.3% higher.

```diff
diff --git a/orange3_spark_amd/models/glm.py b/orange3_spark_amd/models/glm.py
--- a/orange3_spark_amd/models/glm.py
+++ b/orange3_spark_amd/models/glm.py
@@ -88,6 +88,8 @@
             grid = max(1, min(cus * 32, -(-tiles // 4)))
             self.ws = G.GlmWorkspace(self.device, self.ld,
                                      grid=int(os.environ.get("O3S_GLM_GRID_MIX", str(grid))))
+            self.ws.reserve_items(int(self.X.shape[0]), int(self.lineage[2] if self.lineage else 0),
+                                  self.sw is not None)
         elif self.kernel and self.lineage and self.X.shape[0] and os.environ.get("O3S_GLM_OVERLAP", "1") == "1":
             cus = N.num_cus(self.device)
             res_grid = int(os.environ.get("O3S_GLM_GRID_RES", str(cus * 8)))
diff --git a/orange3_spark_amd/ops/_native.py b/orange3_spark_amd/ops/_native.py
--- a/orange3_spark_amd/ops/_native.py
+++ b/orange3_spark_amd/ops/_native.py
@@ -22,7 +22,10 @@
     "o3s_glm_grad": [c_i32, c_i32, c_vp, c_i64, c_i64, c_vp, c_vp, c_vp, c_u32, c_i64,
                      c_vp, c_f32, c_vp, c_i32, c_vp, c_i32, c_vp],
     "o3s_glm_grad_mixed": [c_i32, c_vp, c_i64, c_i64, c_vp, c_vp, c_vp, c_u32, c_i64, c_i64,
-                           c_vp, c_i32, c_vp, c_i32, c_i64, c_vp, c_u32, c_u32, c_i32, c_i32, c_i32, c_vp],
+                           c_vp, c_i32, c_vp, c_i32, c_i64, c_vp, c_u32, c_u32, c_i32, c_i32, c_i32, c_i32, c_i32,
+                           c_vp, c_i64, c_vp, c_i64, c_vp, c_i32, c_vp],
+    "o3s_glm_persist_plan": [c_i64, c_i64, c_i64, c_i32, c_i32, c_i32, c_i32, c_i32, C.POINTER(c_i64),
+                             C.POINTER(c_i64), C.POINTER(c_i64)],
     "o3s_glm_stats_mixed": [c_vp, c_i64, c_i64, c_vp, c_vp, c_u32, c_i64, c_i64, c_vp, c_i32, c_vp, c_i32, c_i32,
                             c_vp],
     "o3s_glm_grad_f32": [c_i32, c_vp, c_i64, c_i64, c_vp, c_vp, c_vp, c_i64, c_vp, c_i32, c_vp, c_i32, c_i64, c_vp,
diff --git a/orange3_spark_amd/ops/csrc/glm.hip b/orange3_spark_amd/ops/csrc/glm.hip
--- a/orange3_spark_amd/ops/csrc/glm.hip
+++ b/orange3_spark_amd/ops/csrc/glm.hip
@@ -1,6 +1,7 @@
 #include <type_traits>
 
 #include "common.h"
+#include "glm_items.h"
 
 using namespace o3s;
 
@@ -468,6 +469,11 @@
   int64_t tstep;
   uint32_t r_ahead, l_ahead;
   bool lab_younger;
+  const unsigned char* x0;
+  const float* yr0;
+  const float* yl0;
+  uint32_t nx_r0, nx_nr, nx_l0, nx_nl;
+  bool r_pre, l_pre;
 
   __device__ static __forceinline__ uint32_t fresh(int v) {
     asm volatile("" : "+v"(v));
@@ -498,6 +504,7 @@
     --l_ahead;
     lab_younger = true;
   }
+  template <bool PERSIST = false>
   __device__ __forceinline__ void take_tile(int lane, short8 (&xb)[8], short8 (&xv)[UNROLL][CPL], float& yv,
                                             short8 (&fa)[3]) {
     if (lab_younger) asm volatile("s_waitcnt vmcnt(1)" ::: "memory");
@@ -532,6 +539,15 @@
         : "v"(b0), "v"(b0 ^ 16u), "v"(b0 ^ 32u), "v"(b0 ^ 48u), "v"(sbase + ((ln ^ (ln >> 4)) << 4)),
           "v"(sbase + ln * 4), "v"(fbase + ln * 16)
         : "memory");
+    if constexpr (PERSIST) {
+      if (r_ahead == 0 && nx_nr > 0) {
+        xs = x0 + (uint64_t)nx_r0 * (UNROLL * G * kStgLd * 2);
+        yrs = yr0 + (uint64_t)nx_r0 * (UNROLL * G);
+        r_ahead = nx_nr;
+        nx_nr = 0;
+        r_pre = true;
+      }
+    }
     if (r_ahead > 0) issue_tile(lane);
     __builtin_amdgcn_sched_barrier(0);
   }
@@ -571,18 +587,28 @@
         : "memory");
     return d;
   }
+  template <bool PERSIST = false>
   __device__ __forceinline__ void take_label(int g, int c, float& yv) {
     if (lab_younger) asm volatile("s_waitcnt vmcnt(0)" ::: "memory");
     else asm volatile("s_waitcnt vmcnt(%0)" ::"n"(kTileOps) : "memory");
     const uint32_t a4 = sbase + (fresh(g) * LPR + fresh(c)) * 4;
     asm volatile("ds_read_b32 %0, %1 offset:8448\n\ts_waitcnt lgkmcnt(0)" : "=v"(yv) : "v"(a4) : "memory");
     lab_younger = false;
+    if constexpr (PERSIST) {
+      if (l_ahead == 0 && nx_nl > 0) {
+        yls = yl0 + (uint64_t)nx_l0 * (UNROLL * G);
+        l_ahead = nx_nl;
+        nx_nl = 0;
+        l_pre = true;
+      }
+    }
     if (l_ahead > 0) issue_label(g, c);
   }
 };
 static_assert(kStgTileBytes == 8192 && kStgLabelBytes == 256, "the asm offsets in TileStage");
 
-template <class SRC, int LPR, int CPL, int UNROLL, int LOSS, bool SMP, bool FULL = false, bool STAGED = false>
+template <class SRC, int LPR, int CPL, int UNROLL, int LOSS, bool SMP, bool FULL = false, bool STAGED = false,
+          bool PERSIST = false>
 __device__ __forceinline__ void grad_tile(
     int64_t base, int64_t n, const typename SRC::elem* __restrict__ X, int64_t ld, int nch,
     const float* __restrict__ y, const float* __restrict__ sw, uint32_t seed, int64_t row0, const float (&w)[CPL][8],
@@ -657,7 +683,7 @@
   constexpr bool kDpp = LPR == 8 && UNROLL == 2;
   if constexpr (kDpp) row_reduce_8x2(dot, c);
   else RR::run(dot, c);
-  if constexpr (STAGED && SRC::kLineage) stg->take_label(g, c, yy[0]);
+  if constexpr (STAGED && SRC::kLineage) stg->template take_label<PERSIST>(g, c, yy[0]);
   if constexpr (STAGED && SMP) {
     if (!smp.keep(base + (int64_t)TileStage::fresh(ubase * G + g))) ww[0] = 0.f;
   }
@@ -691,7 +717,7 @@
   }
 }
 
-template <int LOSS, bool SMP>
+template <int LOSS, bool SMP, bool PERSIST = false>
 __device__ __forceinline__ void staged_resident_tile(int64_t base, float intercept, int lane, const RowSampler smp,
                                                      float (&acc)[TileStage::CPL][8], float& acc_r, float& acc_loss,
                                                      float& acc_w, TileStage* stg) {
@@ -699,7 +725,7 @@
   short8 xb[8], xv[UNROLL][CPL];
   float yv;
   short8 fa[3];
-  stg->take_tile(lane, xb, xv, yv, fa);
+  stg->template take_tile<PERSIST>(lane, xb, xv, yv, fa);
   const float4_ d = stg->dot(lane, xb, fa);
   float wv = 1.f;
   if constexpr (SMP) {
@@ -783,6 +809,28 @@
 #pragma unroll
     for (int j = 0; j < 8; ++j) acc[k][j] = fmaf(rs, kSynthShift, acc[k][j]);
   grad_epilogue<LPR, CPL>(acc, acc_r, acc_loss, acc_w, partial, pstride, pacc, lane, wid, c);
+}
+
+__device__ __forceinline__ void build_coef_frags(unsigned char* __restrict__ frags, const float* __restrict__ coef) {
+  for (int e = threadIdx.x; e < kStgFragBytes / 16; e += kBlock) {
+    const int s = e >> 6, term = e & 15, q = (e & 63) >> 4;
+    uint32_t p[4] = {0u, 0u, 0u, 0u};
+    if (term < 3) {
+      const float* cw = coef + 8 * (8 * q + s);
+#pragma unroll
+      for (int j = 0; j < 4; ++j) {
+        const float x0 = cw[2 * j], x1 = cw[2 * j + 1];
+        const uint32_t ph = pk_bf16(x0, x1);
+        const float r0 = x0 - __uint_as_float(ph << 16), r1 = x1 - __uint_as_float(ph & 0xffff0000u);
+        const uint32_t pm = pk_bf16(r0, r1);
+        const uint32_t pl = pk_bf16(r0 - __uint_as_float(pm << 16), r1 - __uint_as_float(pm & 0xffff0000u));
+        p[j] = term == 0 ? ph : term == 1 ? pm : pl;
+      }
+    }
+    uint32_t* const dst = reinterpret_cast<uint32_t*>(frags + e * 16);
+#pragma unroll
+    for (int j = 0; j < 4; ++j) dst[j] = p[j];
+  }
 }
 
 template <int LOSS, bool SMP>
@@ -825,25 +873,7 @@
   const uint32_t S = nr + nl;
   int64_t br = (int64_t)gw * RT, bl = br;
   using lds_byte = __attribute__((address_space(3))) unsigned char;
-  for (int e = threadIdx.x; e < kStgFragBytes / 16; e += kBlock) {
-    const int s = e >> 6, term = e & 15, q = (e & 63) >> 4;
-    uint32_t p[4] = {0u, 0u, 0u, 0u};
-    if (term < 3) {
-      const float* cw = coef + 8 * (8 * q + s);
-#pragma unroll
-      for (int j = 0; j < 4; ++j) {
-        const float x0 = cw[2 * j], x1 = cw[2 * j + 1];
-        const uint32_t ph = pk_bf16(x0, x1);
-        const float r0 = x0 - __uint_as_float(ph << 16), r1 = x1 - __uint_as_float(ph & 0xffff0000u);
-        const uint32_t pm = pk_bf16(r0, r1);
-        const uint32_t pl = pk_bf16(r0 - __uint_as_float(pm << 16), r1 - __uint_as_float(pm & 0xffff0000u));
-        p[j] = term == 0 ? ph : term == 1 ? pm : pl;
-      }
-    }
-    uint32_t* const dst = reinterpret_cast<uint32_t*>(frags + e * 16);
-#pragma unroll
-    for (int j = 0; j < 4; ++j) dst[j] = p[j];
-  }
+  build_coef_frags(frags, coef);
   __syncthreads();
   TileStage st{slots + wid * kStgWaveBytes,
                (uint32_t)(uintptr_t)(lds_byte*)slots + wid * kStgWaveBytes,
@@ -877,6 +907,179 @@
 #pragma unroll
     for (int j = 0; j < 8; ++j) acc[k][j] = fmaf(rs, kSynthShift, acc[k][j]);
   grad_epilogue<LPR, CPL>(acc, acc_r, acc_loss, acc_w, partial, pstride, pacc, lane, wid, c);
+}
+
+__device__ __forceinline__ uint32_t claim_item(uint32_t* __restrict__ ticket, int lane) {
+  uint32_t t = 0;
+  if (lane == 0) t = atomicAdd(ticket, 1u);
+  return (uint32_t)__builtin_amdgcn_readfirstlane((int)t);
+}
+__device__ __forceinline__ GlmItem uniform_item(uint32_t i, uint32_t Tr, uint32_t Tl, uint32_t items, double inv) {
+  const GlmItem it = glm_item(i, Tr, Tl, items, inv);
+  return GlmItem{(uint32_t)__builtin_amdgcn_readfirstlane((int)it.r0), (uint32_t)__builtin_amdgcn_readfirstlane((int)it.nr),
+                 (uint32_t)__builtin_amdgcn_readfirstlane((int)it.l0), (uint32_t)__builtin_amdgcn_readfirstlane((int)it.nl)};
+}
+template <int LPR, int CPL>
+__device__ __forceinline__ void item_flush(float (&acc)[CPL][8], float& rs, float& acc_r, float& acc_loss,
+                                           float& acc_w, float* __restrict__ dst, int lane) {
+  static_assert(LPR == 8 && CPL == 4, "the halving below is written for the (8, 4) layout");
+  constexpr int DP = LPR * CPL * 8;
+  float a[16], b[8];
+  float4_ q;
+  const uint32_t ln = TileStage::fresh(lane);
+  const bool h2 = (ln & 32) != 0, h1 = (ln & 16) != 0, h0 = (ln & 8) != 0;
+  const auto xch = [&](float v, uint32_t bit) {
+    return __builtin_bit_cast(float, __builtin_amdgcn_ds_bpermute((int)((ln ^ bit) << 2), __builtin_bit_cast(int, v)));
+  };
+#pragma unroll
+  for (int t = 0; t < 16; ++t) {
+    const float lo = fmaf(rs, kSynthShift, acc[t >> 3][t & 7]), hi = fmaf(rs, kSynthShift, acc[2 + (t >> 3)][t & 7]);
+    a[t] = (h2 ? hi : lo) + xch(h2 ? lo : hi, 32u);
+  }
+#pragma unroll
+  for (int t = 0; t < 8; ++t)
+    b[t] = (h1 ? a[8 + t] : a[t]) + xch(h1 ? a[t] : a[8 + t], 16u);
+#pragma unroll
+  for (int t = 0; t < 4; ++t)
+    q[t] = (h0 ? b[4 + t] : b[t]) + xch(h0 ? b[t] : b[4 + t], 8u);
+  const float sr = wave_sum_dpp(acc_r), sl = wave_sum_dpp(acc_loss), sw = wave_sum_dpp(acc_w);
+  {
+    const uint32_t g = ln >> 3, cc = ln & (LPR - 1);
+    *reinterpret_cast<float4_*>(dst + (8 * (cc + ((g >> 1) & 3) * LPR) + 4 * (g & 1))) = q;
+  }
+  if (ln == 0) {
+    dst[DP] = sr;
+    dst[DP + 1] = sl;
+    dst[DP + 2] = sw;
+  }
+  zero(acc);
+  rs = acc_r = acc_loss = acc_w = 0.f;
+}
+
+template <int LOSS, bool SMP>
+__global__ __launch_bounds__(kBlock, 3) void glm_grad_persist_kernel(
+    const uint16_t* __restrict__ X, int64_t n_res, const float* __restrict__ y, const float* __restrict__ y_lin,
+    const float* __restrict__ coef, const float* __restrict__ bptr, uint32_t seed, int64_t row0, int64_t n_lin,
+    float* __restrict__ islab, int pstride, int64_t res_row0, const int64_t* __restrict__ t_dev, uint32_t sseed,
+    uint32_t sthr, uint32_t* __restrict__ ticket, uint32_t items, double inv_items) {
+  constexpr int LPR = TileStage::LPR, CPL = TileStage::CPL, UNROLL = TileStage::UNROLL, G = TileStage::G;
+  constexpr int RT = G * UNROLL;
+  constexpr int64_t ld = kStgLd;
+  __shared__ __attribute__((aligned(256))) unsigned char slots[kWavesPerBlock * kStgWaveBytes];
+  __shared__ __attribute__((aligned(256))) unsigned char frags[kStgFragBytes];
+  const int lane = threadIdx.x & (kWave - 1);
+  const int wid = __builtin_amdgcn_readfirstlane(threadIdx.x / kWave);
+  const int g = lane / LPR, c = lane % LPR;
+  const float intercept = *bptr;
+  const uint32_t skey = SMP ? sample_key(sseed, (uint32_t)((t_dev ? t_dev[0] : 0) + 1)) : 0u;
+  const RowSampler smp_res{skey, sthr, res_row0}, smp_lin{skey, sthr, row0};
+
+  float w[CPL][8], acc[CPL][8];
+  float wshift = 0.f;
+#pragma unroll
+  for (int k = 0; k < CPL; ++k)
+#pragma unroll
+    for (int j = 0; j < 8; ++j) {
+      w[k][j] = coef[8 * (c + k * LPR) + j];
+      wshift += w[k][j];
+      acc[k][j] = 0.f;
+    }
+  wshift *= kSynthShift;
+  float rs = 0.f;
+  float acc_r = 0.f, acc_loss = 0.f, acc_w = 0.f;
+
+  const uint32_t Tr = (uint32_t)(n_res / RT), Tl = (uint32_t)(n_lin / RT);
+  using lds_byte = __attribute__((address_space(3))) unsigned char;
+  build_coef_frags(frags, coef);
+  __syncthreads();
+  TileStage st{slots + wid * kStgWaveBytes,
+               (uint32_t)(uintptr_t)(lds_byte*)slots + wid * kStgWaveBytes,
+               (uint32_t)(uintptr_t)(lds_byte*)frags,
+               nullptr,
+               nullptr,
+               nullptr,
+               (int64_t)RT,
+               0u,
+               0u,
+               false,
+               reinterpret_cast<const unsigned char*>(X),
+               y,
+               y_lin,
+               0u,
+               0u,
+               0u,
+               0u,
+               false,
+               false};
+  uint32_t cur = claim_item(ticket, lane);
+  if (cur >= items) return;
+  GlmItem it = uniform_item(cur, Tr, Tl, items, inv_items);
+  for (;;) {
+    const uint32_t nr = it.nr, nl = it.nl, S = nr + nl;
+    int64_t br = (int64_t)it.r0 * RT, bl = (int64_t)it.l0 * RT;
+    if (nl > 0 && !st.l_pre) {
+      st.yls = y_lin + bl;
+      st.l_ahead = nl;
+      st.issue_label(g, c);
+    }
+    if (nr > 0 && !st.r_pre) {
+      st.xs = st.x0 + br * (ld * 2);
+      st.yrs = y + br;
+      st.r_ahead = nr;
+      st.issue_tile(lane);
+    }
+    st.r_pre = st.l_pre = false;
+    st.nx_nr = st.nx_nl = 0u;
+    uint32_t nxt = items;
+    GlmItem nx{0u, 0u, 0u, 0u};
+    bool claimed = false;
+    const auto claim_next = [&]() {
+      claimed = true;
+      nxt = claim_item(ticket, lane);
+      if (nxt < items) {
+        nx = uniform_item(nxt, Tr, Tl, items, inv_items);
+        st.nx_r0 = nx.r0;
+        st.nx_nr = nx.nr;
+        st.nx_l0 = nx.l0;
+        st.nx_nl = nx.nl;
+      }
+    };
+    uint32_t rem = 0, r_left = nr;
+    for (uint32_t s = 0; s < S; ++s) {
+      rem += nl;
+      if (rem >= S) {
+        rem -= S;
+        grad_tile<RowsLineage, LPR, CPL, UNROLL, LOSS, SMP, true, true, true>(bl, n_lin, X, ld, CPL * LPR, y_lin, nullptr,
+                                                                              seed, row0, w, wshift, intercept, g, c,
+                                                                              smp_lin, acc, rs, acc_r, acc_loss, acc_w, &st);
+        bl += RT;
+      } else {
+        if (r_left == 1) claim_next();
+        --r_left;
+        staged_resident_tile<LOSS, SMP, true>(br, intercept, lane, smp_res, acc, acc_r, acc_loss, acc_w, &st);
+        br += RT;
+      }
+    }
+    if (!claimed) claim_next();
+    item_flush<LPR, CPL>(acc, rs, acc_r, acc_loss, acc_w, islab + (int64_t)cur * pstride, lane);
+    if (nxt >= items) break;
+    cur = nxt;
+    it = nx;
+  }
+}
+
+constexpr int kItemChunk = 256, kItemSumBlock = 320;
+__global__ __launch_bounds__(kItemSumBlock) void glm_item_sum_kernel(const float* __restrict__ slab, int64_t nrows,
+                                                                    int pstride, int ncols,
+                                                                    double* __restrict__ mid) {
+  const int64_t lo = (int64_t)blockIdx.x * kItemChunk;
+  const int64_t hi = lo + kItemChunk < nrows ? lo + kItemChunk : nrows;
+  for (int i = threadIdx.x; i < ncols; i += kItemSumBlock) {
+    double s = 0.0;
+#pragma unroll 8
+    for (int64_t r = lo; r < hi; ++r) s += (double)__builtin_nontemporal_load(slab + r * pstride + i);
+    mid[(int64_t)blockIdx.x * pstride + i] = s;
+  }
 }
 
 template <class SRC, int LPR, int CPL, int U, bool UNW, bool FULL = false>
@@ -1241,6 +1444,24 @@
   }
 }
 
+__global__ __launch_bounds__(1024) void glm_finish_f64_kernel(const double* __restrict__ mid, int nrows, int pstride,
+                                                              int ncols, double* __restrict__ out) {
+  __shared__ double red[32][33];
+  const int cx = threadIdx.x & 31, gy = threadIdx.x >> 5;
+  const int i = blockIdx.x * 32 + cx;
+  double s = 0.0;
+  if (i < ncols)
+    for (int b = gy; b < nrows; b += 32) s += mid[(int64_t)b * pstride + i];
+  red[gy][cx] = s;
+  __syncthreads();
+  if (gy == 0 && i < ncols) {
+    double t = 0.0;
+#pragma unroll 8
+    for (int q = 0; q < 32; ++q) t += red[q][cx];
+    out[i] = t;
+  }
+}
+
 __global__ __launch_bounds__(256) void glm_sgd_update_kernel(
     const double* __restrict__ out, int dpad, double* __restrict__ bt, double* __restrict__ b,
     const double* __restrict__ inv_std, const double* __restrict__ l2v, double l2, double eta,
@@ -1380,6 +1601,78 @@
   return 0;
 }
 
+struct PersistPlan { int64_t items, slab_floats, mid_doubles; };
+constexpr int kPersistBlocksPerCu = 3;
+constexpr int kMaxDevices = 64;
+int current_device() {
+  int dev = 0;
+  return hipGetDevice(&dev) == hipSuccess && dev >= 0 && dev < kMaxDevices ? dev : -1;
+}
+int device_cus() {
+  static int cus[kMaxDevices] = {};
+  const int dev = current_device();
+  if (dev < 0) return 256;
+  if (cus[dev] == 0) {
+    int n = 0;
+    if (hipDeviceGetAttribute(&n, hipDeviceAttributeMultiprocessorCount, dev) != hipSuccess || n < 1) n = 256;
+    cus[dev] = n;
+  }
+  return cus[dev];
+}
+PersistPlan persist_plan(int64_t ld, int64_t n_res, int64_t n_lin, bool weighted, int full_tiles, int staged,
+                         int persist, int item_tiles, int pstride) {
+  constexpr int64_t RT = TileStage::G * TileStage::UNROLL;
+  const PersistPlan none{0, 0, 0};
+  if (persist <= 0 || item_tiles <= 0 || !full_tiles || ld != kStgLd || weighted || n_res < 0 || n_lin < 0) return none;
+  const uint64_t Tr = (uint64_t)(n_res / RT), Tl = (uint64_t)(n_lin / RT);
+  if (Tr + Tl == 0 || Tr >= kGlmItemMaxTiles || Tl >= kGlmItemMaxTiles) return none;
+  if (!(staged >= 2 || (staged == 1 && Tr > 0 && Tl > 0))) return none;
+  const uint64_t items = glm_item_count(Tr, Tl, (uint64_t)item_tiles);
+  if (items > kGlmItemMaxTiles) return none;
+  if (persist == 1) {
+    const uint64_t waves = (uint64_t)kPersistBlocksPerCu * device_cus() * kWavesPerBlock;
+    if (Tr == 0 || Tl == 0 || items < 64 * waves) return none;
+  }
+  const int64_t rows = (int64_t)items + 1;
+  return PersistPlan{(int64_t)items, rows * pstride, (rows + kItemChunk - 1) / kItemChunk * pstride};
+}
+template <int LOSS, bool SMP>
+int persist_blocks_per_cu() {
+  static int occ[kMaxDevices] = {};
+  const int dev = current_device();
+  if (dev < 0) return 1;
+  if (occ[dev] == 0) {
+    int o = 0;
+    if (hipOccupancyMaxActiveBlocksPerMultiprocessor(&o, glm_grad_persist_kernel<LOSS, SMP>, kBlock, 0) != hipSuccess ||
+        o < 1)
+      o = 1;
+    occ[dev] = o;
+  }
+  return occ[dev];
+}
+int launch_item_finish(const float* islab, int64_t nrows, int pstride, int ncols, double* imid, double* out,
+                       hipStream_t st) {
+  const int chunks = (int)((nrows + kItemChunk - 1) / kItemChunk);
+  hipLaunchKernelGGL(glm_item_sum_kernel, dim3(chunks), dim3(kItemSumBlock), 0, st, islab, nrows, pstride, ncols, imid);
+  O3S_CHECK_LAUNCH();
+  hipLaunchKernelGGL(glm_finish_f64_kernel, dim3((ncols + 31) / 32), dim3(1024), 0, st, imid, chunks, pstride, ncols,
+                     out);
+  O3S_CHECK_LAUNCH();
+  return 0;
+}
+
+}
+
+O3S_API int o3s_glm_persist_plan(int64_t ld, int64_t n_res, int64_t n_lin, int weighted, int full_tiles, int staged,
+                                 int persist, int item_tiles, int64_t* items, int64_t* slab_floats,
+                                 int64_t* mid_doubles) {
+  Layout l;
+  if (!resolve_layout(ld, &l)) return -1;
+  const PersistPlan p = persist_plan(ld, n_res, n_lin, weighted != 0, full_tiles, staged, persist, item_tiles, l.dpad + 4);
+  *items = p.items;
+  *slab_floats = p.slab_floats;
+  *mid_doubles = p.mid_doubles;
+  return 0;
 }
 
 O3S_API int o3s_glm_layout(int64_t ld, int* dpad, int* pstride) {
@@ -1426,16 +1719,24 @@
                                const float* sw, const float* coef, uint32_t seed, int64_t row0,
                                int64_t n_lin, float* partial, int grid, double* out, int waves,
                                int64_t res_row0, const int64_t* t_dev, uint32_t sseed,
-                               uint32_t sthr, int splits, int full_tiles, int staged, hipStream_t st) {
+                               uint32_t sthr, int splits, int full_tiles, int staged, int persist, int item_tiles,
+                               float* islab, int64_t islab_floats, double* imid, int64_t imid_doubles,
+                               uint32_t* ticket, int persist_blocks, hipStream_t st) {
   Layout l;
   if (!resolve_layout(ld, &l) || grid <= 0 || n_res < 0 || n_lin < 0) return -1;
   const int pstride = l.dpad + 4;
+  const PersistPlan plan = persist_plan(ld, n_res, n_lin, sw != nullptr, full_tiles, staged, persist, item_tiles, pstride);
+  if (plan.items > 0 && (!islab || !imid || !ticket || islab_floats < plan.slab_floats ||
+                         imid_doubles < plan.mid_doubles))
+    return -2;
+  bool persisted = false;
   const uint16_t* Xh = (const uint16_t*)X;
   const bool smp = sthr < (1u << 24);
   const int rc = with_remapped_layout_and_loss(l, loss, [&](auto L, auto C, auto LOSS) {
     constexpr int U = C >= 8 ? 1 : 8 / C;
     constexpr int64_t RT = (kWave / L) * U;
-    auto slice = [&](auto FULL, int g, int64_t r_lo, int64_t r_n, int64_t l_lo, int64_t l_n, int pacc) {
+    auto slice = [&](auto FULL, int g, int64_t r_lo, int64_t r_n, int64_t l_lo, int64_t l_n, int pacc,
+                     float* partial) {
       if (FULL && (r_n % RT != 0 || l_n % RT != 0 || ld != 8 * L * C)) return -1;
       const float* y_lin = y + n_res + l_lo;
       const float* sw_lin = sw ? sw + n_res + l_lo : nullptr;
@@ -1465,25 +1766,51 @@
     };
     constexpr bool kHasFull = !(L >= 32 && C == 4);
     const int64_t r_full = n_res / RT * RT, l_full = n_lin / RT * RT;
+    if constexpr (L == TileStage::LPR && C == TileStage::CPL) {
+      if (plan.items > 0) {
+        persisted = true;
+        if (hipMemsetAsync(ticket, 0, sizeof(uint32_t), st) != hipSuccess) return -3;
+        auto go_persist = [&](auto SMP) {
+          int64_t fit = (int64_t)persist_blocks_per_cu<LOSS, SMP>() * device_cus();
+          if (persist_blocks > 0 && persist_blocks < fit) fit = persist_blocks;
+          const int64_t need = (plan.items + kWavesPerBlock - 1) / kWavesPerBlock;
+          launch(glm_grad_persist_kernel<LOSS, SMP>, (int)(fit < need ? fit : need), st, Xh, r_full, y, y + n_res, coef,
+                 coef + l.dpad, seed, row0, l_full, islab, pstride, res_row0, t_dev, sseed, sthr, ticket,
+                 (uint32_t)plan.items, glm_item_inv((uint64_t)plan.items));
+        };
+        if (smp) go_persist(std::true_type{});
+        else go_persist(std::false_type{});
+        O3S_CHECK_LAUNCH();
+        int64_t rows = plan.items;
+        if (r_full != n_res || l_full != n_lin) {
+          const int rc2 = slice(std::false_type{}, 1, r_full, n_res - r_full, l_full, n_lin - l_full, 0,
+                                islab + plan.items * pstride);
+          O3S_CHECK_LAUNCH();
+          if (rc2 != 0) return rc2;
+          ++rows;
+        }
+        return launch_item_finish(islab, rows, pstride, l.dpad + 3, imid, out, st);
+      }
+    }
     if constexpr (kHasFull) {
       if (full_tiles && ld == 8 * L * C && r_full + l_full > 0) {
         const int rc = for_row_slices(
             splits, n_res, n_lin,
             [&](int64_t r_lo, int64_t r_n, int64_t l_lo, int64_t l_n, int pacc) {
-              return slice(std::true_type{}, grid, r_lo, r_n, l_lo, l_n, pacc);
+              return slice(std::true_type{}, grid, r_lo, r_n, l_lo, l_n, pacc, partial);
             },
             RT);
         if (rc != 0 || (r_full == n_res && l_full == n_lin)) return rc;
-        const int rc2 = slice(std::false_type{}, 1, r_full, n_res - r_full, l_full, n_lin - l_full, 1);
+        const int rc2 = slice(std::false_type{}, 1, r_full, n_res - r_full, l_full, n_lin - l_full, 1, partial);
         O3S_CHECK_LAUNCH();
         return rc2;
       }
     }
     return for_row_slices(splits, n_res, n_lin, [&](int64_t r_lo, int64_t r_n, int64_t l_lo, int64_t l_n, int pacc) {
-      return slice(std::false_type{}, grid, r_lo, r_n, l_lo, l_n, pacc);
+      return slice(std::false_type{}, grid, r_lo, r_n, l_lo, l_n, pacc, partial);
     });
   });
-  if (rc != 0) return rc;
+  if (rc != 0 || persisted) return rc;
   return launch_finish(partial, grid, pstride, l.dpad + 3, out, 0, st);
 }
 
diff --git a/orange3_spark_amd/ops/csrc/glm_items.h b/orange3_spark_amd/ops/csrc/glm_items.h
--- /dev/null
+++ b/orange3_spark_amd/ops/csrc/glm_items.h
@@ -0,0 +1,38 @@
+#pragma once
+#include <stdint.h>
+
+#if defined(__HIPCC__)
+#define O3S_HD __host__ __device__
+#else
+#define O3S_HD
+#endif
+
+namespace o3s {
+
+struct GlmItem {
+  uint32_t r0, nr;
+  uint32_t l0, nl;
+};
+
+constexpr uint64_t kGlmItemMaxTiles = uint64_t(1) << 31;
+
+O3S_HD inline uint64_t glm_item_count(uint64_t Tr, uint64_t Tl, uint64_t T) {
+  return T == 0 ? 0 : (Tr + Tl + T - 1) / T;
+}
+O3S_HD inline double glm_item_inv(uint64_t I) { return 1.0 / (double)I; }
+
+O3S_HD inline uint64_t glm_item_cut(uint64_t i, uint64_t n, uint64_t I, double inv) {
+  const uint64_t x = i * n;
+  uint64_t q = (uint64_t)((double)x * inv);
+  while (q * I > x) --q;
+  while (x - q * I >= I) ++q;
+  return q;
+}
+
+O3S_HD inline GlmItem glm_item(uint64_t i, uint64_t Tr, uint64_t Tl, uint64_t I, double inv) {
+  const uint64_t r0 = glm_item_cut(i, Tr, I, inv), r1 = glm_item_cut(i + 1, Tr, I, inv);
+  const uint64_t l0 = glm_item_cut(i, Tl, I, inv), l1 = glm_item_cut(i + 1, Tl, I, inv);
+  return GlmItem{(uint32_t)r0, (uint32_t)(r1 - r0), (uint32_t)l0, (uint32_t)(l1 - l0)};
+}
+
+}
diff --git a/orange3_spark_amd/ops/glm.py b/orange3_spark_amd/ops/glm.py
--- a/orange3_spark_amd/ops/glm.py
+++ b/orange3_spark_amd/ops/glm.py
@@ -1,5 +1,7 @@
 from __future__ import annotations
 
+import ctypes
+import logging
 import os
 
 import numpy as np
@@ -8,6 +10,7 @@
 from . import _native as N
 
 LOSS_LOGISTIC, LOSS_HINGE, LOSS_SQUARED = 0, 1, 2
+log = logging.getLogger(__name__)
 _MASK = 0xFFFFFFFF
 
 
@@ -157,6 +160,36 @@
         self.grid = grid or (N.num_cus(self.device) * 8 if self.device.type == "cuda" else 1)
         self.partial = torch.empty(self.grid * self.pstride, dtype=torch.float32, device=self.device)
         self.out = torch.empty(self.dpad + 3, dtype=torch.float64, device=self.device)
+        self.islab = self.imid = self.ticket = None
+        self.persist_failed = False
+
+    def item_slab(self, slab_floats: int, mid_doubles: int) -> None:
+        if self.ticket is None:
+            self.ticket = torch.zeros(1, dtype=torch.int32, device=self.device)
+        if self.islab is None or self.islab.numel() < slab_floats:
+            self.islab = None
+            self.islab = torch.empty(slab_floats, dtype=torch.float32, device=self.device)
+        if self.imid is None or self.imid.numel() < mid_doubles:
+            self.imid = None
+            self.imid = torch.empty(mid_doubles, dtype=torch.float64, device=self.device)
+
+    def reserve_items(self, n_res: int, n_lin: int, weighted: bool) -> int:
+        if MIX_PERSIST <= 0 or self.persist_failed or self.device.type != "cuda":
+            return 0
+        items, slab, mid = ctypes.c_int64(), ctypes.c_int64(), ctypes.c_int64()
+        N.check(N.kernels().o3s_glm_persist_plan(self.ld, n_res, n_lin, int(weighted), MIX_FULL_TILES, MIX_STAGED,
+                                                 MIX_PERSIST, MIX_ITEM_TILES, ctypes.byref(items), ctypes.byref(slab),
+                                                 ctypes.byref(mid)), "glm_persist_plan")
+        if items.value > 0:
+            try:
+                self.item_slab(slab.value, mid.value)
+            except torch.cuda.OutOfMemoryError:
+                self.islab = self.imid = None
+                self.persist_failed = True
+                log.warning("GLM item slab of %.0f MB (O3S_GLM_MIX_ITEM_TILES=%d) does not fit; "
+                            "the pass keeps its sliced launches", slab.value * 4 / 2 ** 20, MIX_ITEM_TILES)
+                return 0
+        return MIX_PERSIST
 
 
 _ROWS_MSG = ("GPU GLM pass expects a contiguous bf16 feature matrix (or a contiguous fp32 one whose row "
@@ -218,6 +251,9 @@
 MIX_SLICE_ROWS = int(os.environ.get("O3S_GLM_MIX_SLICE_ROWS", str(64 << 20)))
 MIX_FULL_TILES = int(os.environ.get("O3S_GLM_MIX_FULL", "1"))
 MIX_STAGED = int(os.environ.get("O3S_GLM_MIX_STAGED", "1"))
+MIX_PERSIST = int(os.environ.get("O3S_GLM_MIX_PERSIST", "1"))
+MIX_ITEM_TILES = int(os.environ.get("O3S_GLM_MIX_ITEM_TILES", "256"))
+MIX_PERSIST_BLOCKS = int(os.environ.get("O3S_GLM_MIX_PERSIST_BLOCKS", "0"))
 
 
 def mix_splits(n_rows: int) -> int:
@@ -273,11 +309,17 @@
                                              mix_splits(nr), N.stream_of(X)), "glm_grad_f32")
         return ws.out
     cf = _coef_buf(coef, ws.dpad, ws.device, intercept=intercept)
-    N.check(N.kernels().o3s_glm_grad_mixed(loss, X.data_ptr(), ld, nr, y.data_ptr(), N.ptr(sw),
-                                           cf.data_ptr(), seed & _MASK, row0, n_lin, ws.partial.data_ptr(),
-                                           ws.grid, ws.out.data_ptr(), MIX_WAVES, int(res_row0),
-                                           N.ptr(t_dev), int(sample_seed) & _MASK, thr, mix_splits(nr + n_lin),
-                                           MIX_FULL_TILES, MIX_STAGED, N.stream_of(X)),
+    lib = N.kernels()
+    persist = ws.reserve_items(nr, n_lin, sw is not None)
+    has = ws.islab is not None
+    N.check(lib.o3s_glm_grad_mixed(loss, X.data_ptr(), ld, nr, y.data_ptr(), N.ptr(sw),
+                                   cf.data_ptr(), seed & _MASK, row0, n_lin, ws.partial.data_ptr(),
+                                   ws.grid, ws.out.data_ptr(), MIX_WAVES, int(res_row0),
+                                   N.ptr(t_dev), int(sample_seed) & _MASK, thr, mix_splits(nr + n_lin),
+                                   MIX_FULL_TILES, MIX_STAGED, persist, MIX_ITEM_TILES,
+                                   N.ptr(ws.islab), ws.islab.numel() if has else 0,
+                                   N.ptr(ws.imid), ws.imid.numel() if has else 0, N.ptr(ws.ticket),
+                                   MIX_PERSIST_BLOCKS, N.stream_of(X)),
             "glm_grad_mixed")
     return ws.out
 
```
